# OpenNLPLab/ACR_WSSS

Hardware: AMD Instinct MI355X
Metric: img/s ACR-ViT-hybrid-base 448x448 train step (higher is better)
Workload: dtype f32_split; 1 GPU; BASELINE configs[1]: ViT-hybrid-base (DPT) 448x448, batch 16 per GPU, ACR train step (2 views, fwd+bwd+SGD); global_batch=16, classes=20, alpha=125, parallelism=dp1

## Files before the change

### acr_wsss_amd/csrc/attn_f32.h

```cpp
#pragma once
#include <hip/hip_runtime.h>
#include <stdint.h>

struct AttnGeom {
    int B, H, T;
    float scale;
    int64_t sb, st, sh;
    int64_t osb, ost, osh;
};

void acr_attn_fwd_f32_dma(const AttnGeom& g, const float* q, const float* k, const float* v, float* o, float* lse2, float* pmean,
                          int64_t pmean_sb, int64_t pmean_st, hipStream_t st);
void acr_attn_bwd_f32_dma(const AttnGeom& g, const float* q, const float* k, const float* v, const float* o, const float* d_o,
                          const float* lse2, const float* gm, int64_t gm_sb, int64_t gm_st, float* dq, float* dk, float* dv,
                          float* delta, hipStream_t st);

void acr_attn_fwd_f32_sres(const AttnGeom& g, const float* q, const float* k, const float* v, float* o, float* lse2, float* scores,
                           float* pmean, int64_t pmean_sb, int64_t pmean_st, hipStream_t st);
void acr_attn_bwd_f32_sres(const AttnGeom& g, const float* q, const float* k, const float* v, const float* o, const float* d_o,
                           const float* lse2, const float* scores, const float* gm, int64_t gm_sb, int64_t gm_st, float* dq,
                           float* dk, float* dv, float* delta, hipStream_t st);
void acr_attn_pmean_sres(const AttnGeom& g, const float* scores, const float* lse2, float* pmean, int64_t pmean_sb, int64_t pmean_st,
                         hipStream_t st);
void acr_attn_delta_sres(const AttnGeom& g, const float* scores, const float* o, const float* d_o, const float* lse2, const float* gm,
                         int64_t gm_sb, int64_t gm_st, float* delta, hipStream_t st);

int64_t acr_attn_x3_scores_floats(const AttnGeom& g);
int64_t acr_attn_x3_bwd_ws_floats(const AttnGeom& g);
bool acr_attn_x3_fwd_uses_split_tail(int T);
void acr_attn_fwd_f32_x3(const AttnGeom& g, const float* q, const float* k, const float* v, float* o, float* lse2, float* scores,
                         float* pmean, int64_t pmean_sb, int64_t pmean_st, hipStream_t st, char* oimg = nullptr);
void acr_attn_bwd_f32_x3(const AttnGeom& g, const float* q, const float* k, const float* v, const float* o, const float* d_o,
                         const float* lse2, const float* scores, const float* gm, int64_t gm_sb, int64_t gm_st, float* dq, float* dk,
                         float* dv, float* delta_ws, hipStream_t st);
```

### acr_wsss_amd/csrc/attn_f32.hip

```cpp
#include "acr_common.h"
#include "attn_f32.h"
#include "attn_f32_scores.h"

#define LDP 68
#define TILE_FLOATS (32 * LDP)

template <typename T, int NTHREADS>
__device__ __forceinline__ void stage_tile(float* lds, const T* g, int64_t st, int row0, int Tn, int tid, float mul) {
#pragma unroll
    for (int i = 0; i < 512 / NTHREADS; ++i) {
        const int slot = tid + i * NTHREADS;
        const int row = slot >> 4, c4 = slot & 15;
        f32x4 v = acr_load4<T>(g + (int64_t)min(row0 + row, Tn - 1) * st + c4 * 4) * mul;
        const f32x4 z = {0.f, 0.f, 0.f, 0.f};
        *reinterpret_cast<f32x4*>(lds + row * LDP + c4 * 4) = (row0 + row < Tn) ? v : z;
    }
}

template <typename T>
__device__ __forceinline__ void load_rows(float (&reg)[32], const T* g, int64_t st, int row0, int Tn, int lane, float mul) {
    const int r = lane & 31, h = lane >> 5;
    const float okm = (row0 + r < Tn) ? mul : 0.f;
    const T* p = g + (int64_t)min(row0 + r, Tn - 1) * st + 32 * h;
#pragma unroll
// ... 323 lines not shown
    const int r = lane & 31, hh = lane >> 5;
    const int key0 = ktile * 64 + wave * 32;
    const int64_t base = (int64_t)b * g.sb + (int64_t)h * g.sh;
    const int64_t obase = (int64_t)b * g.osb + (int64_t)h * g.osh;
    float kreg[32], vreg[32];
    load_rows<T>(kreg, k + base, g.st, key0, g.T, lane, g.scale * ACR_LOG2E);
    load_rows<T>(vreg, v + base, g.st, key0, g.T, lane, 1.f);
    const int key = key0 + r;
    const bool kok = key < g.T;
    const float invH = 1.f / (float)g.H;
    const float* lrow = lse2 + ((int64_t)b * g.H + h) * g.T;
    const float* drow = delta + ((int64_t)b * g.H + h) * g.T;
    const float* gbase = gm ? gm + (int64_t)b * gm_sb + min(key, g.T - 1) : nullptr;
    f32x16 dk0 = {0}, dk1 = {0}, dv0 = {0}, dv1 = {0};
    for (int q0 = 0; q0 < g.T; q0 += 32) {
        __syncthreads();
        stage_tile<T, 128>(qtile, q + base, g.st, q0, g.T, tid, 1.f);
        stage_tile<T, 128>(dotile, d_o + obase, g.ost, q0, g.T, tid, 1.f);
        if (tid < 32) {
            const bool ok = q0 + tid < g.T;
            const int qc = min(q0 + tid, g.T - 1);
            const float lv = lrow[qc], dvv = drow[qc];
            l2s[tid] = ok ? lv : INFINITY;
            dls[tid] = ok ? dvv : 0.f;
        }
        __syncthreads();
        f32x16 s = {0}, dp = {0};
        mma_rowop(s, qtile, kreg, lane);
        mma_rowop(dp, dotile, vreg, lane);
        float gv[16];
#pragma unroll
        for (int reg = 0; reg < 16; ++reg) gv[reg] = 0.f;
        if (gbase) {
#pragma unroll
            for (int reg = 0; reg < 16; ++reg) gv[reg] = gbase[min(q0 + acr_krow(reg, hh), g.T - 1) * (int)gm_st] * invH;
        }
        f32x16 p, ds;
        const float kmask = kok ? 1.f : 0.f;
#pragma unroll
        for (int reg = 0; reg < 16; ++reg) {
            const int kr = acr_krow(reg, hh);
            const float pv = exp2f(s[reg] - l2s[kr]) * kmask;
            p[reg] = pv;
            ds[reg] = pv * (dp[reg] + gv[reg] - dls[kr]);
        }
        mma_accop_a(dv0, p, dotile, 0, lane);
        mma_accop_a(dv1, p, dotile, 1, lane);
        mma_accop_a(dk0, ds, qtile, 0, lane);
        mma_accop_a(dk1, ds, qtile, 1, lane);
    }
#pragma unroll
    for (int reg = 0; reg < 16; ++reg) {
        const int kk = key0 + acr_krow(reg, hh);
        if (kk < g.T) {
            T* pk = dk + base + (int64_t)kk * g.st;
            T* pv = dv + base + (int64_t)kk * g.st;
            acr_store1<T>(pk + r, dk0[reg] * g.scale);
            acr_store1<T>(pk + 32 + r, dk1[reg] * g.scale);
            acr_store1<T>(pv + r, dv0[reg]);
            acr_store1<T>(pv + 32 + r, dv1[reg]);
        }
    }
}

template <typename T>
__global__ __launch_bounds__(64) void getam_row_kernel(AttnGeom g, const T* __restrict__ q, const T* __restrict__ k,
                                                       const T* __restrict__ v, const T* __restrict__ d_o,
                                                       const float* __restrict__ lse2, int batch, int func,
                                                       float* __restrict__ cam_row, int64_t row_stride) {
    __shared__ float q0s[64], do0s[64];
    const int j = blockIdx.x * 64 + threadIdx.x;
    batch += blockIdx.y;
    cam_row += (int64_t)blockIdx.y * row_stride;
    float sum_g = 0.f, sum_cg = 0.f;
    for (int h = 0; h < g.H; ++h) {
        const int64_t base = (int64_t)batch * g.sb + (int64_t)h * g.sh;
        __syncthreads();
        q0s[threadIdx.x] = acr_load1<T>(q + base + threadIdx.x) * (g.scale * ACR_LOG2E);
        do0s[threadIdx.x] = acr_load1<T>(d_o + (int64_t)batch * g.osb + (int64_t)h * g.osh + threadIdx.x);
        __syncthreads();
        if (j < g.T) {
            const T* kr = k + base + (int64_t)j * g.st;
            const T* vr = v + base + (int64_t)j * g.st;
            float s = 0.f, dp = 0.f;
#pragma unroll
            for (int d4 = 0; d4 < 16; ++d4) {
                f32x4 kv = acr_load4<T>(kr + 4 * d4), vv = acr_load4<T>(vr + 4 * d4);
#pragma unroll
                for (int e = 0; e < 4; ++e) {
                    s = fmaf(kv[e], q0s[4 * d4 + e], s);
                    dp = fmaf(vv[e], do0s[4 * d4 + e], dp);
                }
            }
            const float p = exp2f(s - lse2[((int64_t)batch * g.H + h) * g.T]);
            sum_g += fmaxf(dp, 0.f);
            sum_cg += fmaxf(dp * p, 0.f);
        }
    }
    if (j < g.T) {
        const float invH = 1.f / (float)g.H;
        const float mg = sum_g * invH, mcg = sum_cg * invH;
        float val;
        switch (func) {
            case ACR_GETAM_GRAD: val = mg; break;
            case ACR_GETAM_CAM_GRAD: val = mcg; break;
            case ACR_GETAM_GRAD_S: val = mg * mg; break;
            default: val = mcg * mg; break;
        }
        cam_row[j] += val;
    }
}

bool acr_bf16_mfma_ok(const acr_attn_desc* d, const void* const* ptrs, int n);
void acr_attn_fwd_bf16(const acr_attn_desc* d, const void* q, const void* k, const void* v, void* o, float* lse2,
                       float* pmean, int64_t pmean_sb, int64_t pmean_st, hipStream_t st);
void acr_attn_bwd_bf16(const acr_attn_desc* d, const void* q, const void* k, const void* v, const void* o,
                       const void* d_o, const float* lse2, const float* gm, int64_t gm_sb, int64_t gm_st, void* dq, void* dk,
                       void* dv, float* delta, hipStream_t st);
void acr_attn_probs_bf16(const acr_attn_desc* d, const void* q, const void* k, const float* lse2, float* probs,
                         hipStream_t st);
void acr_attn_dprobs_bf16(const acr_attn_desc* d, const void* d_o, const void* v, float* dprobs, hipStream_t st);

static int check_desc(const acr_attn_desc* d, const char* who) {
    ACR_CHECK_ARG(d != nullptr, "%s: null desc", who);
    ACR_CHECK_ARG(d->B > 0 && d->H > 0 && d->T > 0, "%s: bad geometry B=%d H=%d T=%d", who, d->B, d->H, d->T);
    ACR_CHECK_ARG(d->head_dim == 64, "%s: head_dim %d unsupported (library is built for 64)", who, d->head_dim);
    ACR_CHECK_ARG(d->dtype == ACR_F32 || d->dtype == ACR_BF16 || d->dtype == ACR_BF16_F32MATH || d->dtype == ACR_F32_BF16X3,
                  "%s: unknown dtype %d", who, d->dtype);
    ACR_CHECK_ARG((d->qkv_sb % 4) == 0 && (d->qkv_st % 4) == 0 && (d->qkv_sh % 4) == 0 && (d->o_sb % 4) == 0 &&
                      (d->o_st % 4) == 0 && (d->o_sh % 4) == 0,
                  "%s: strides must be multiples of 4 elements (vector loads)", who);
    ACR_CHECK_ARG((int64_t)d->B * d->H * ((d->T + 63) / 64) < (1ll << 31), "%s: grid too large", who);
    return ACR_OK;
}
static AttnGeom geom(const acr_attn_desc* d) {
    AttnGeom g;
    g.B = d->B; g.H = d->H; g.T = d->T; g.scale = d->scale;
    g.sb = d->qkv_sb; g.st = d->qkv_st; g.sh = d->qkv_sh;
    g.osb = d->o_sb; g.ost = d->o_st; g.osh = d->o_sh;
    return g;
}
static bool aligned16(const void* p) { return (reinterpret_cast<uintptr_t>(p) & 15) == 0; }
static bool aligned8(const void* p) { return (reinterpret_cast<uintptr_t>(p) & 7) == 0; }

template <typename T>
static int attn_fwd_t(const acr_attn_desc* d, const void* q, const void* k, const void* v, void* o, float* lse2,
                      float* pmean, int64_t pmean_sb, int64_t pmean_st, hipStream_t st) {
    AttnGeom g = geom(d);
    const int nqt = (d->T + 63) / 64;
    hipLaunchKernelGGL((attn_fwd_kernel<T>), dim3(d->B * d->H * nqt), dim3(128), 0, st, g, (const T*)q, (const T*)k,
                       (const T*)v, (T*)o, lse2);
    if (pmean)
        hipLaunchKernelGGL((attn_tile_qk_kernel<T, TQK_PMEAN>), dim3(d->B * nqt * nqt), dim3(256), 0, st, g,
                           (const T*)q, (const T*)k, (const float*)lse2, pmean, pmean_sb, pmean_st);
    return acr_check_launch("acr_attn_fwd");
}

extern "C" int acr_attn_fwd(const acr_attn_desc* d, const void* q, const void* k, const void* v, void* o,
                            float* lse2, float* pmean, int64_t pmean_sb, int64_t pmean_st, void* stream) {
    int rc = check_desc(d, "acr_attn_fwd");
    if (rc) return rc;
    ACR_CHECK_ARG(q && k && v && o && lse2, "acr_attn_fwd: null pointer");
    const bool f32 = d->dtype == ACR_F32;
    ACR_CHECK_ARG(f32 ? (aligned16(q) && aligned16(k) && aligned16(v) && aligned16(o))
                      : (aligned8(q) && aligned8(k) && aligned8(v) && aligned8(o)),
                  "acr_attn_fwd: q/k/v/o must be 16-byte (fp32) / 8-byte (bf16) aligned");
    ACR_CHECK_ARG(!pmean || (pmean_st >= d->T && pmean_sb >= (int64_t)d->T * pmean_st),
                  "acr_attn_fwd: pmean row pitch < T or batch stride < T*pitch");
    if (f32) {
        acr_attn_fwd_f32_dma(geom(d), (const float*)q, (const float*)k, (const float*)v, (float*)o, lse2, pmean, pmean_sb, pmean_st,
                             (hipStream_t)stream);
        return acr_check_launch("acr_attn_fwd");
    }
    const void* ptrs[4] = {q, k, v, o};
    if (d->dtype == ACR_BF16 && acr_bf16_mfma_ok(d, ptrs, 4)) {
        acr_attn_fwd_bf16(d, q, k, v, o, lse2, pmean, pmean_sb, pmean_st, (hipStream_t)stream);
        return acr_check_launch("acr_attn_fwd");
    }
    return attn_fwd_t<__bf16>(d, q, k, v, o, lse2, pmean, pmean_sb, pmean_st, (hipStream_t)stream);
}

static int check_gmean(const acr_attn_desc* d, const char* who, const float* gmean, int64_t gmean_sb, int64_t gmean_st) {
    ACR_CHECK_ARG(!gmean || (gmean_st >= d->T && gmean_sb >= (int64_t)d->T * gmean_st), "%s: gmean row pitch < T or batch stride < T*pitch", who);
    return ACR_OK;
}

template <typename T>
static int attn_bwd_t(const acr_attn_desc* d, const void* q, const void* k, const void* v, const void* o,
                      const void* d_o, const float* lse2, const float* gm, int64_t gm_sb, int64_t gm_st, void* dq,
                      void* dk, void* dv, float* delta, hipStream_t st) {
    AttnGeom g = geom(d);
    const int nqt = (d->T + 63) / 64;
    const dim3 grid(d->B * d->H * nqt);
    hipLaunchKernelGGL((attn_delta_kernel<T>), grid, dim3(128), 0, st, g, (const T*)q, (const T*)k, (const T*)o,
                       (const T*)d_o, lse2, gm, gm_sb, gm_st, delta);
    hipLaunchKernelGGL((attn_dkdv_kernel<T>), grid, dim3(128), 0, st, g, (const T*)q, (const T*)k, (const T*)v,
                       (const T*)d_o, lse2, (const float*)delta, gm, gm_sb, gm_st, (T*)dk, (T*)dv);
    hipLaunchKernelGGL((attn_dq_kernel<T>), grid, dim3(128), 0, st, g, (const T*)q, (const T*)k, (const T*)v,
                       (const T*)d_o, lse2, (const float*)delta, gm, gm_sb, gm_st, (T*)dq);
    return acr_check_launch("acr_attn_bwd");
}

extern "C" int acr_attn_bwd(const acr_attn_desc* d, const void* q, const void* k, const void* v, const void* o,
                            const void* d_o, const float* lse2, const float* gmean, int64_t gmean_sb, int64_t gmean_st,
                            void* dq, void* dk, void* dv, float* delta_ws, void* stream) {
    int rc = check_desc(d, "acr_attn_bwd");
    if (rc) return rc;
    ACR_CHECK_ARG(q && k && v && o && d_o && lse2 && dq && dk && dv && delta_ws, "acr_attn_bwd: null pointer");
    rc = check_gmean(d, "acr_attn_bwd", gmean, gmean_sb, gmean_st);
    if (rc) return rc;
    const bool f32 = d->dtype == ACR_F32;
    ACR_CHECK_ARG(f32 ? (aligned16(q) && aligned16(k) && aligned16(v) && aligned16(o) && aligned16(d_o))
                      : (aligned8(q) && aligned8(k) && aligned8(v) && aligned8(o) && aligned8(d_o)),
                  "acr_attn_bwd: inputs must be 16-byte (fp32) / 8-byte (bf16) aligned");
    if (f32) {
        acr_attn_bwd_f32_dma(geom(d), (const float*)q, (const float*)k, (const float*)v, (const float*)o, (const float*)d_o, lse2,
                             gmean, gmean_sb, gmean_st, (float*)dq, (float*)dk, (float*)dv, delta_ws, (hipStream_t)stream);
        return acr_check_launch("acr_attn_bwd");
    }
    const void* ptrs[8] = {q, k, v, o, d_o, dq, dk, dv};
    const bool g_ok = !gmean || ((gmean_st & 3) == 0 && gmean_st >= ((d->T + 3) & ~3) && (gmean_sb & 3) == 0 &&
                                 (reinterpret_cast<uintptr_t>(gmean) & 15) == 0);
    if (d->dtype == ACR_BF16 && g_ok && acr_bf16_mfma_ok(d, ptrs, 8)) {
        acr_attn_bwd_bf16(d, q, k, v, o, d_o, lse2, gmean, gmean_sb, gmean_st, dq, dk, dv, delta_ws, (hipStream_t)stream);
        return acr_check_launch("acr_attn_bwd");
    }
    return attn_bwd_t<__bf16>(d, q, k, v, o, d_o, lse2, gmean, gmean_sb, gmean_st, dq, dk, dv, delta_ws, (hipStream_t)stream);
}

extern "C" int64_t acr_attn_scores_floats(const acr_attn_desc* d) {
    if (d == nullptr || d->B <= 0 || d->H <= 0 || d->T <= 0) return 0;
    if (d->dtype == ACR_F32_BF16X3) return acr_attn_x3_scores_floats(geom(d));
    return attn_score_floats(d->B, d->H, d->T);
}

extern "C" int64_t acr_attn_bwd_ws_floats(const acr_attn_desc* d) {
    if (d == nullptr || d->B <= 0 || d->H <= 0 || d->T <= 0) return 0;
    if (d->dtype == ACR_F32_BF16X3) return acr_attn_x3_bwd_ws_floats(geom(d));
    return (int64_t)d->B * d->H * d->T;
}

static int check_x3(const acr_attn_desc* d, const char* who) {
    ACR_CHECK_ARG(d->qkv_sh >= 64 && d->o_sh >= 64, "%s: ACR_F32_BF16X3 needs head strides >= 64", who);
    ACR_CHECK_ARG((int64_t)32 * d->H * 64 < (1ll << 30), "%s: too many heads", who);
    return ACR_OK;
}

static int check_fwd_scores(const acr_attn_desc* d, const char* who, const void* q, const void* k, const void* v, const void* o,
                            const float* lse2, const float* scores, const float* pmean, int64_t pmean_sb, int64_t pmean_st,
                            bool has_image, const float* o_image) {
    ACR_CHECK_ARG(q && k && v && o && lse2 && scores && (!has_image || o_image), "%s: null pointer", who);
    ACR_CHECK_ARG(aligned16(q) && aligned16(k) && aligned16(v) && aligned16(o) && aligned16(scores) && aligned16(o_image),
                  "%s: q/k/v/o/scores%s must be 16-byte aligned", who, has_image ? "/o_image" : "");
    ACR_CHECK_ARG(!pmean || (pmean_st >= d->T && pmean_sb >= (int64_t)d->T * pmean_st), "%s: pmean row pitch < T or batch stride < T*pitch", who);
    return ACR_OK;
}

extern "C" int acr_attn_fwd_scores(const acr_attn_desc* d, const void* q, const void* k, const void* v, void* o, float* lse2,
                                   float* scores, float* pmean, int64_t pmean_sb, int64_t pmean_st, void* stream) {
    int rc = check_desc(d, "acr_attn_fwd_scores");
    if (rc) return rc;
    if (d->dtype != ACR_F32 && d->dtype != ACR_F32_BF16X3) {
        acr_set_error("acr_attn_fwd_scores: fp32 tensors only (the bf16 kernels recompute the logits)");
        return ACR_ERR_UNSUPPORTED;
    }
    rc = check_fwd_scores(d, "acr_attn_fwd_scores", q, k, v, o, lse2, scores, pmean, pmean_sb, pmean_st, false, nullptr);
    if (rc) return rc;
    if (d->dtype == ACR_F32_BF16X3) {
        rc = check_x3(d, "acr_attn_fwd_scores");
        if (rc) return rc;
        acr_attn_fwd_f32_x3(geom(d), (const float*)q, (const float*)k, (const float*)v, (float*)o, lse2, scores, pmean, pmean_sb, pmean_st,
                            (hipStream_t)stream);
        return acr_check_launch("acr_attn_fwd_scores");
    }
    acr_attn_fwd_f32_sres(geom(d), (const float*)q, (const float*)k, (const float*)v, (float*)o, lse2, scores, pmean, pmean_sb,
                          pmean_st, (hipStream_t)stream);
    return acr_check_launch("acr_attn_fwd_scores");
}

extern "C" int acr_attn_fwd_scores_oimg(const acr_attn_desc* d, const void* q, const void* k, const void* v, void* o, float* lse2,
                                        float* scores, float* pmean, int64_t pmean_sb, int64_t pmean_st, float* o_image, void* stream) {
    int rc = check_desc(d, "acr_attn_fwd_scores_oimg");
    if (rc) return rc;
    if (d->dtype != ACR_F32_BF16X3) {
        acr_set_error("acr_attn_fwd_scores_oimg: ACR_F32_BF16X3 only (the image is the split-product operand form)");
        return ACR_ERR_UNSUPPORTED;
    }
    rc = check_fwd_scores(d, "acr_attn_fwd_scores_oimg", q, k, v, o, lse2, scores, pmean, pmean_sb, pmean_st, true, o_image);
    if (rc) return rc;
    ACR_CHECK_ARG(d->o_sh == 64 && d->o_st == (int64_t)d->H * 64 && d->o_sb == (int64_t)d->T * d->o_st,
                  "acr_attn_fwd_scores_oimg: o must be the dense (B, T, H*64) activation (its image is that of the (B*T) x (H*64) matrix)");
    rc = check_x3(d, "acr_attn_fwd_scores_oimg");
    if (rc) return rc;
    acr_attn_fwd_f32_x3(geom(d), (const float*)q, (const float*)k, (const float*)v, (float*)o, lse2, scores, pmean, pmean_sb, pmean_st,
                        (hipStream_t)stream, reinterpret_cast<char*>(o_image));
    return acr_check_launch("acr_attn_fwd_scores_oimg");
}

extern "C" int acr_attn_fwd_oimg_offered(const acr_attn_desc* d) {
    if (!d || d->dtype != ACR_F32_BF16X3 || d->T <= 0) return 0;
    return acr_attn_x3_fwd_uses_split_tail(d->T) ? 0 : 1;
}

extern "C" int acr_attn_bwd_scores(const acr_attn_desc* d, const void* q, const void* k, const void* v, const void* o,
                                   const void* d_o, const float* lse2, const float* scores, const float* gmean, int64_t gmean_sb,
                                   int64_t gmean_st, void* dq, void* dk, void* dv, float* delta_ws, void* stream) {
    int rc = check_desc(d, "acr_attn_bwd_scores");
    if (rc) return rc;
    if (d->dtype != ACR_F32 && d->dtype != ACR_F32_BF16X3) {
        acr_set_error("acr_attn_bwd_scores: fp32 tensors only (the bf16 kernels recompute the logits)");
        return ACR_ERR_UNSUPPORTED;
    }
    ACR_CHECK_ARG(q && k && v && o && d_o && lse2 && scores && dq && dk && dv && delta_ws, "acr_attn_bwd_scores: null pointer");
    ACR_CHECK_ARG(aligned16(q) && aligned16(k) && aligned16(v) && aligned16(o) && aligned16(d_o) && aligned16(scores),
                  "acr_attn_bwd_scores: inputs must be 16-byte aligned");
    rc = check_gmean(d, "acr_attn_bwd_scores", gmean, gmean_sb, gmean_st);
    if (rc) return rc;
    ACR_CHECK_ARG(!gmean || ((gmean_st & 3) == 0 && (gmean_sb & 3) == 0 && aligned16(gmean)),
                  "acr_attn_bwd_scores: gmean must be 16-byte aligned with pitch and batch stride multiples of 4 floats");
    if (d->dtype == ACR_F32_BF16X3) {
        rc = check_x3(d, "acr_attn_bwd_scores");
        if (rc) return rc;
        ACR_CHECK_ARG(aligned16(delta_ws) && aligned16(dq) && aligned16(dk) && aligned16(dv), "acr_attn_bwd_scores: delta_ws / dq / dk / dv must be 16-byte aligned");
        acr_attn_bwd_f32_x3(geom(d), (const float*)q, (const float*)k, (const float*)v, (const float*)o, (const float*)d_o, lse2, scores,
                            gmean, gmean_sb, gmean_st, (float*)dq, (float*)dk, (float*)dv, delta_ws, (hipStream_t)stream);
        return acr_check_launch("acr_attn_bwd_scores");
    }
    acr_attn_bwd_f32_sres(geom(d), (const float*)q, (const float*)k, (const float*)v, (const float*)o, (const float*)d_o, lse2,
                          scores, gmean, gmean_sb, gmean_st, (float*)dq, (float*)dk, (float*)dv, delta_ws, (hipStream_t)stream);
    return acr_check_launch("acr_attn_bwd_scores");
}

extern "C" int acr_attn_probs(const acr_attn_desc* d, const void* q, const void* k, const float* lse2, float* probs,
                              void* stream) {
    int rc = check_desc(d, "acr_attn_probs");
    if (rc) return rc;
    ACR_CHECK_ARG(q && k && lse2 && probs, "acr_attn_probs: null pointer");
    AttnGeom g = geom(d);
    const int nt = (d->T + 63) / 64;
    ACR_CHECK_ARG((int64_t)d->B * d->H * nt * nt < (1ll << 31), "acr_attn_probs: grid too large");
    const dim3 grid(d->B * d->H * nt * nt);
    const void* pp[2] = {q, k};
    if (d->dtype == ACR_F32)
        hipLaunchKernelGGL((attn_tile_qk_kernel<float, TQK_PROBS>), grid, dim3(256), 0, (hipStream_t)stream, g,
                           (const float*)q, (const float*)k, lse2, probs, (int64_t)0, (int64_t)0);
    else if (d->dtype == ACR_BF16 && acr_bf16_mfma_ok(d, pp, 2))
        acr_attn_probs_bf16(d, q, k, lse2, probs, (hipStream_t)stream);
    else
        hipLaunchKernelGGL((attn_tile_qk_kernel<__bf16, TQK_PROBS>), grid, dim3(256), 0, (hipStream_t)stream, g,
                           (const __bf16*)q, (const __bf16*)k, lse2, probs, (int64_t)0, (int64_t)0);
    return acr_check_launch("acr_attn_probs");
}

extern "C" int acr_attn_dprobs(const acr_attn_desc* d, const void* d_o, const void* v, float* dprobs, void* stream) {
    int rc = check_desc(d, "acr_attn_dprobs");
    if (rc) return rc;
    ACR_CHECK_ARG(d_o && v && dprobs, "acr_attn_dprobs: null pointer");
    AttnGeom g = geom(d);
    const int nt = (d->T + 63) / 64;
    ACR_CHECK_ARG((int64_t)d->B * d->H * nt * nt < (1ll << 31), "acr_attn_dprobs: grid too large");
    const dim3 grid(d->B * d->H * nt * nt);
    const void* pp[2] = {d_o, v};
    if (d->dtype == ACR_F32)
        hipLaunchKernelGGL((attn_tile_qk_kernel<float, TQK_DPROBS>), grid, dim3(256), 0, (hipStream_t)stream, g,
                           (const float*)d_o, (const float*)v, (const float*)nullptr, dprobs, (int64_t)0, (int64_t)0);
    else if (d->dtype == ACR_BF16 && acr_bf16_mfma_ok(d, pp, 2))
        acr_attn_dprobs_bf16(d, d_o, v, dprobs, (hipStream_t)stream);
    else
        hipLaunchKernelGGL((attn_tile_qk_kernel<__bf16, TQK_DPROBS>), grid, dim3(256), 0, (hipStream_t)stream, g,
                           (const __bf16*)d_o, (const __bf16*)v, (const float*)nullptr, dprobs, (int64_t)0, (int64_t)0);
    return acr_check_launch("acr_attn_dprobs");
}

extern "C" int acr_getam_row_accum(const acr_attn_desc* d, const void* q, const void* k, const void* v,
                                   const void* d_o, const float* lse2, int32_t batch, int32_t func, float* cam_row,
                                   void* stream) {
    int rc = check_desc(d, "acr_getam_row_accum");
    if (rc) return rc;
    ACR_CHECK_ARG(q && k && v && d_o && lse2 && cam_row, "acr_getam_row_accum: null pointer");
    ACR_CHECK_ARG(batch >= 0 && batch < d->B, "acr_getam_row_accum: batch %d out of range", batch);
    ACR_CHECK_ARG(func >= 0 && func <= 3, "acr_getam_row_accum: unknown func %d", func);
    AttnGeom g = geom(d);
    const dim3 grid((d->T + 63) / 64);
    if (d->dtype == ACR_F32)
        hipLaunchKernelGGL((getam_row_kernel<float>), grid, dim3(64), 0, (hipStream_t)stream, g, (const float*)q,
                           (const float*)k, (const float*)v, (const float*)d_o, lse2, batch, func, cam_row, (int64_t)0);
    else
        hipLaunchKernelGGL((getam_row_kernel<__bf16>), grid, dim3(64), 0, (hipStream_t)stream, g, (const __bf16*)q,
                           (const __bf16*)k, (const __bf16*)v, (const __bf16*)d_o, lse2, batch, func, cam_row, (int64_t)0);
    return acr_check_launch("acr_getam_row_accum");
}

extern "C" int acr_getam_rows_accum(const acr_attn_desc* d, const void* q, const void* k, const void* v, const void* d_o,
                                    const float* lse2, int32_t func, float* cam_rows, int64_t row_stride, void* stream) {
    int rc = check_desc(d, "acr_getam_rows_accum");
    if (rc) return rc;
    ACR_CHECK_ARG(q && k && v && d_o && lse2 && cam_rows, "acr_getam_rows_accum: null pointer");
    ACR_CHECK_ARG(func >= 0 && func <= 3, "acr_getam_rows_accum: unknown func %d", func);
    ACR_CHECK_ARG(row_stride >= d->T && d->B < 65536, "acr_getam_rows_accum: row pitch < T or batch too large");
    ACR_CHECK_ARG(d->dtype != ACR_F32_BF16X3, "acr_getam_rows_accum: exact kernels only (pass ACR_F32)");
    AttnGeom g = geom(d);
    const dim3 grid((d->T + 63) / 64, d->B);
    if (d->dtype == ACR_F32)
        hipLaunchKernelGGL((getam_row_kernel<float>), grid, dim3(64), 0, (hipStream_t)stream, g, (const float*)q,
                           (const float*)k, (const float*)v, (const float*)d_o, lse2, 0, func, cam_rows, row_stride);
    else
        hipLaunchKernelGGL((getam_row_kernel<__bf16>), grid, dim3(64), 0, (hipStream_t)stream, g, (const __bf16*)q,
                           (const __bf16*)k, (const __bf16*)v, (const __bf16*)d_o, lse2, 0, func, cam_rows, row_stride);
    return acr_check_launch("acr_getam_rows_accum");
}
```

### acr_wsss_amd/csrc/attn_f32_scores.h

```cpp
#pragma once
#include "acr_common.h"
#include "attn_f32.h"
#include "attn_f32_tiles.h"

#define SB_FLOATS 1024
__device__ __forceinline__ int64_t attn_score_block(int H, int NB, int b, int hd, int qb, int kb) {
    return ((((int64_t)b * H + hd) * NB + qb) * NB + kb) * SB_FLOATS;
}
static inline int64_t attn_score_floats(int B, int H, int T) {
    const int64_t nb = (T + 31) / 32;
    return (int64_t)B * H * nb * nb * SB_FLOATS;
}
static inline bool attn_split_tail(int NB, int nw) { return (NB % nw) == 1 && NB > nw; }

#define SRES_LOAD_NT(p) __builtin_nontemporal_load(reinterpret_cast<const f32x4*>(p))
#define SRES_LOAD(p) (*reinterpret_cast<const f32x4*>(p))
#define SRES_STORE(p, v) __builtin_nontemporal_store(v, reinterpret_cast<f32x4*>(p))
#define SRES_LOAD_DQ(p) SRES_LOAD_NT(p)
#define SRES_DMA_AUX 0

template <bool TEXT, int N>
__device__ __forceinline__ void attn_vmcnt() {
    if constexpr (!TEXT) asm volatile("s_waitcnt vmcnt(%0)" ::"n"(N) : "memory");
    else if constexpr (N == 8) asm volatile("s_waitcnt vmcnt(8)" ::: "memory");
    else if constexpr (N == 4) asm volatile("s_waitcnt vmcnt(4)" ::: "memory");
    else { static_assert(N == 0, "add the count's text"); asm volatile("s_waitcnt vmcnt(0)" ::: "memory"); }
}
template <bool TEXT, int... Ns>
__device__ __forceinline__ void attn_wait_vm(int n) {
    if (!((n >= Ns ? (attn_vmcnt<TEXT, Ns>(), true) : false) || ...)) attn_vmcnt<TEXT, 0>();
}
#define ATTN_FENCE() asm volatile("" ::: "memory")

#define ATTN_MASK_ROWS(s, row0, T, h)                                   \
    if ((row0) + 32 > (T)) {  \
        _Pragma("unroll") for (int reg = 0; reg < 16; ++reg)            \
            if ((row0) + acr_krow(reg, h) >= (T)) s[reg] = -INFINITY;   \
    }

#define ATTN_QLANE_STREAMS(sres, H, NB, T, b, hd, q0, wave, lane, ssm, gsm, gm, gm_sb, gm_st)                                       \
    const float* srow = sres + attn_score_block(H, NB, b, hd, min(q0 >> 5, NB - 1), 0) + lane * 4;                                  \
    float* sw = ssm + wave * 2 * SB_FLOATS;                                                                                         \
    auto dma_scores = [&](int kblk, int slot) {                                                                                     \
        const float* src = srow + (int64_t)kblk * SB_FLOATS;                                                                        \
        _Pragma("unroll") for (int gq = 0; gq < 4; ++gq)                                                                            \
            __builtin_amdgcn_global_load_lds((glb_vp)(src + gq * 256), (lds_vp)(sw + slot * SB_FLOATS + gq * 256), 16, 0, SRES_DMA_AUX); \
    };                                                                                                                              \
    const float* gb0 = gm ? gm + (int64_t)b * gm_sb : nullptr;                                                                      \
    float* gw = gsm + wave * SB_FLOATS;                                                                                             \
    const float* grow[4];                                                                                                           \
    int gchunk[4];                                                                                                                  \
    _Pragma("unroll") for (int p = 0; p < 4; ++p) {                                                                                 \
        const int row = 8 * p + (lane >> 3);                                                                                        \
        grow[p] = gb0 ? gb0 + (int64_t)min(q0 + row, T - 1) * gm_st : nullptr;                                                      \
        gchunk[p] = 4 * ((lane & 7) ^ ((row >> 1) & 7));                                                                            \
    }                                                                                                                               \
    auto dma_g = [&](int k0) {                                                                                                      \
        if (gb0 == nullptr) return;                                                                                                 \
        _Pragma("unroll") for (int p = 0; p < 4; ++p)                                                                               \
            __builtin_amdgcn_global_load_lds((glb_vp)(grow[p] + min(k0 + gchunk[p], (int)gm_st - 4)), (lds_vp)(gw + p * 256), 16, 0, 0); \
    }
#define ATTN_QLANE_ADDRS(lane, r, h)                                                                                                \
    const uint32_t saddr = lds_addr_of(sw) + lane * 16;                                                                             \
    uint32_t gaddr[4];                                                                                                              \
    _Pragma("unroll") for (int gq = 0; gq < 4; ++gq) gaddr[gq] = lds_addr_of(gw) + r * 128 + (((2 * gq + h) ^ ((r >> 1) & 7)) << 4)
#define ATTN_QLANE_READ(SLOT, s4, g4, k0, T, h)                                                                                     \
    ACR_LDS_RD128(s4[0], saddr, SLOT * 4096); ACR_LDS_RD128(s4[1], saddr, SLOT * 4096 + 1024);                                      \
    ACR_LDS_RD128(s4[2], saddr, SLOT * 4096 + 2048); ACR_LDS_RD128(s4[3], saddr, SLOT * 4096 + 3072);                               \
    if (gb0 != nullptr) {                                                                                                           \
        ACR_LDS_RD128(g4[0], gaddr[0], 0); ACR_LDS_RD128(g4[1], gaddr[1], 0);                                                       \
        ACR_LDS_RD128(g4[2], gaddr[2], 0); ACR_LDS_RD128(g4[3], gaddr[3], 0);                                                       \
        ACR_LDS_WAIT4(0, g4[0], g4[1], g4[2], g4[3]);                                                                               \
        if (k0 + 32 > T) {                                                                                                          \
            _Pragma("unroll") for (int gq = 0; gq < 4; ++gq)                                                                        \
                _Pragma("unroll") for (int e = 0; e < 4; ++e)                                                                       \
                    if (k0 + 8 * gq + 4 * h + e >= T) g4[gq][e] = 0.f;                                                              \
        }                                                                                                                           \
    } else {                                                                                                                        \
        _Pragma("unroll") for (int gq = 0; gq < 4; ++gq) g4[gq] = f32x4{0.f, 0.f, 0.f, 0.f};                                        \
    }                                                                                                                               \
    ACR_LDS_WAIT4(0, s4[0], s4[1], s4[2], s4[3])
__device__ __forceinline__ void attn_ds_qlane(f32x16& ds, const f32x4 (&s4)[4], const f32x4 (&g4)[4], const f32x16& dp, float l2q, float dl,
                                              float invH) {
#pragma unroll
    for (int reg = 0; reg < 16; ++reg)
        ds[reg] = __builtin_amdgcn_exp2f(s4[reg >> 2][reg & 3] - l2q) * (dp[reg] + g4[reg >> 2][reg & 3] * invH - dl);
}

#define ATTN_KLANE_STREAMS(sres, H, NB, T, b, hd, key0, wave, lane, ssm, gsm, gm, gm_sb, gm_st)                                     \
    const float* scol = sres + attn_score_block(H, NB, b, hd, 0, min(key0 >> 5, NB - 1));                                           \
    const int64_t sstep = (int64_t)NB * SB_FLOATS;                                                                                  \
    int soff[4];                                                                                                                    \
    _Pragma("unroll") for (int gq = 0; gq < 4; ++gq) soff[gq] = gq * 256 + 4 * (lane ^ (2 * gq + (lane >> 5)));                     \
    float* sw = ssm + wave * 2 * SB_FLOATS;                                                                                         \
    auto dma_scores = [&](int qblk, int slot) {                                                                                     \
        const float* src = scol + (int64_t)qblk * sstep;                                                                            \
        _Pragma("unroll") for (int gq = 0; gq < 4; ++gq)                                                                            \
            __builtin_amdgcn_global_load_lds((glb_vp)(src + soff[gq]), (lds_vp)(sw + slot * SB_FLOATS + gq * 256), 16, 0, SRES_DMA_AUX); \
    };                                                                                                                              \
    const float* gb0 = gm ? gm + (int64_t)b * gm_sb : nullptr;                                                                      \
    float* gw = gsm + wave * SB_FLOATS;                                                                                             \
    const int gcol = min(key0 + 4 * (lane & 7), (int)gm_st - 4);                                                                    \
    auto dma_g = [&](int qrow0) {                                                                                                   \
        if (gb0 == nullptr) return;                                                                                                 \
        _Pragma("unroll") for (int p = 0; p < 4; ++p) {                                                                             \
            const float* src = gb0 + (int64_t)min(qrow0 + 8 * p + (lane >> 3), T - 1) * gm_st + gcol;                               \
            __builtin_amdgcn_global_load_lds((glb_vp)src, (lds_vp)(gw + p * 256), 16, 0, 0);                                        \
        }                                                                                                                           \
    }
#define ATTN_KLANE_ADDRS(ssm, gsm, wave, r, h)                                                                                      \
    uint32_t stb[4];                                                                                                                \
    {                                                                                                                               \
        const int gk = r >> 3, hk = (r >> 2) & 1, ek = r & 3, mm = 2 * gk + hk;                                                     \
        _Pragma("unroll") for (int j = 0; j < 4; ++j)                                                                               \
            stb[j] = lds_addr_of(ssm) + ((wave * 2 * SB_FLOATS) + gk * 256 + 128 * hk + ek + 4 * ((j + 4 * h) ^ mm)) * 4;           \
    }                                                                                                                               \
    const uint32_t gaddr = lds_addr_of(gsm) + (wave * SB_FLOATS + 4 * h * 32 + r) * 4
#define ATTN_16(M, ...) \
    M(0, __VA_ARGS__); M(1, __VA_ARGS__); M(2, __VA_ARGS__); M(3, __VA_ARGS__); M(4, __VA_ARGS__); M(5, __VA_ARGS__); M(6, __VA_ARGS__); M(7, __VA_ARGS__); \
    M(8, __VA_ARGS__); M(9, __VA_ARGS__); M(10, __VA_ARGS__); M(11, __VA_ARGS__); M(12, __VA_ARGS__); M(13, __VA_ARGS__); M(14, __VA_ARGS__); M(15, __VA_ARGS__)
#define ATTN_RDS(REG, s, SLOT) ACR_LDS_RD32(s[REG], stb[(REG) & 3], SLOT * SB_FLOATS * 4 + 128 * ((REG) >> 2))
#define ATTN_RDG(REG, gv) ACR_LDS_RD32(gv[REG], gaddr, 128 * (((REG) & 3) + 8 * ((REG) >> 2)))
#define ATTN_V16(x) \
    "+v"(x[0]), "+v"(x[1]), "+v"(x[2]), "+v"(x[3]), "+v"(x[4]), "+v"(x[5]), "+v"(x[6]), "+v"(x[7]), "+v"(x[8]), "+v"(x[9]), "+v"(x[10]), \
        "+v"(x[11]), "+v"(x[12]), "+v"(x[13]), "+v"(x[14]), "+v"(x[15])
#define ATTN_READ_G(gv)                                                     \
    if (gb0 != nullptr) {                                                   \
        ATTN_16(ATTN_RDG, gv);                                              \
        asm volatile("s_waitcnt lgkmcnt(0)" : ATTN_V16(gv));                \
    } else {                                                                \
        _Pragma("unroll") for (int reg = 0; reg < 16; ++reg) gv[reg] = 0.f; \
    }

__device__ __forceinline__ void attn_store_scores(float* sp, const f32x16& s) {
#pragma unroll
    for (int gq = 0; gq < 4; ++gq) {
        const f32x4 t = {s[4 * gq], s[4 * gq + 1], s[4 * gq + 2], s[4 * gq + 3]};
        SRES_STORE(sp + gq * 256, t);
    }
}
#define ATTN_SOFTMAX_STEP(s, m, l, o0, o1, p)                                                             \
    {                                                                                                     \
        float mx_ = s[0];                                                                                 \
        _Pragma("unroll") for (int reg = 1; reg < 16; ++reg) mx_ = fmaxf(mx_, s[reg]);                    \
        mx_ = fmaxf(mx_, __shfl_xor(mx_, 32));                                                            \
        if (__any(mx_ > m + 8.f)) {                                                                       \
            const float mn_ = fmaxf(m, mx_);                                                              \
            const float alpha_ = __builtin_amdgcn_exp2f(m - mn_);                                         \
            l *= alpha_;                                                                                  \
            o0 *= alpha_; o1 *= alpha_;                                                                   \
            m = mn_;                                                                                      \
        }                                                                                                 \
        float rs_ = 0.f;                                                                                  \
        _Pragma("unroll") for (int reg = 0; reg < 16; ++reg) { p[reg] = __builtin_amdgcn_exp2f(s[reg] - m); rs_ += p[reg]; } \
        rs_ += __shfl_xor(rs_, 32);                                                                       \
        l += rs_;                                                                                         \
    }
#define ATTN_FWD_FINISH(g, o, lse2, b, hd, q0, r, h, o0, o1, m, l, inv)                                                   \
    {                                                                                                                     \
        float* ob_ = o + (int64_t)b * g.osb + (int64_t)(q0 + r) * g.ost + (int64_t)hd * g.osh;                            \
        _Pragma("unroll") for (int grp = 0; grp < 4; ++grp) {                                                             \
            f32x4 a_ = {o0[4 * grp] * inv, o0[4 * grp + 1] * inv, o0[4 * grp + 2] * inv, o0[4 * grp + 3] * inv};          \
            f32x4 c_ = {o1[4 * grp] * inv, o1[4 * grp + 1] * inv, o1[4 * grp + 2] * inv, o1[4 * grp + 3] * inv};          \
            *reinterpret_cast<f32x4*>(ob_ + 8 * grp + 4 * h) = a_;                                                        \
            *reinterpret_cast<f32x4*>(ob_ + 32 + 8 * grp + 4 * h) = c_;                                                   \
        }                                                                                                                 \
        if (h == 0) lse2[((int64_t)b * g.H + hd) * g.T + q0 + r] = m + log2f(l);                                          \
    }
```

### acr_wsss_amd/csrc/attn_f32_sres.hip

```cpp
#include <type_traits>

#include "acr_common.h"
#include "attn_f32.h"
#include "attn_f32_tiles.h"
#include "attn_f32_scores.h"
#include "attn_f32_sres_tails.h"


template <int NW>
__global__ __launch_bounds__(64 * NW, NW == 4 ? 2 : 1) void attn_fwd_sres_kernel(AttnGeom g, const float* __restrict__ q, const float* __restrict__ k,
                                                               const float* __restrict__ v, float* __restrict__ o,
                                                               float* __restrict__ lse2, float* __restrict__ sres, int ntail) {
    __shared__ __attribute__((aligned(1024))) float smem[4 * DT_FLOATS];
    __shared__ float mlsh[4 * 64];
    const int nmain = (int)gridDim.x - ntail;
    if (NW == 4 && (int)blockIdx.x >= nmain) {
        attn_fwd_tail_body<4>(smem, mlsh, g, q, k, v, o, lse2, sres, acr_xcd_remap((int)blockIdx.x - nmain, ntail));
        return;
    }
    const int NB = (g.T + 31) >> 5, nqt = ntail ? NB / NW : (NB + NW - 1) / NW;
    int id = acr_xcd_remap(blockIdx.x, nmain);
    const int qt = id % nqt; id /= nqt;
    const int hd = id % g.H;
    const int b = id / g.H;
// ... 156 lines not shown
    f32x16 pm = {0};
    for (int h0 = 0; h0 < g.H; h0 += 4) {
        f32x4 sv[4][4];
        float lv[4];
#pragma unroll
        for (int hi = 0; hi < 4; ++hi) {
            const int hd = min(h0 + hi, g.H - 1);
#pragma unroll
            for (int gq = 0; gq < 4; ++gq) sv[hi][gq] = SRES_LOAD_NT(sp + hd * hstride + gq * 256);
            lv[hi] = lp[(int64_t)hd * g.T];
        }
#pragma unroll
        for (int hi = 0; hi < 4; ++hi) {
            if (h0 + hi < g.H) {
                const float l2 = qrow < g.T ? lv[hi] : INFINITY;
#pragma unroll
                for (int reg = 0; reg < 16; ++reg) pm[reg] += __builtin_amdgcn_exp2f(sv[hi][reg >> 2][reg & 3] - l2);
            }
        }
    }
    const float mul = 1.f / (float)g.H;
    float* tl = tile[wave];
#pragma unroll
    for (int reg = 0; reg < 16; ++reg) tl[theta * 33 + acr_krow(reg, hh)] = pm[reg] * mul;
    __syncthreads();
    if (act) {
        const int key = kb * 32 + theta;
        float* ob = out + (int64_t)b * out_sb;
        if (key < g.T) {
#pragma unroll
            for (int i = 0; i < 16; ++i) {
                const int row = 2 * i + hh;
                const int qq = qb * 32 + row;
                if (qq < g.T) ob[(int64_t)qq * out_st + key] = tl[row * 33 + theta];
            }
        }
    }
}

__global__ __launch_bounds__(256) void attn_delta_sres_kernel(AttnGeom g, int NB, const float* __restrict__ sres,
                                                              const float* __restrict__ o, const float* __restrict__ d_o,
                                                              const float* __restrict__ lse2, const float* __restrict__ gm,
                                                              int64_t gm_sb, int64_t gm_st, float* __restrict__ delta) {
    const int tid = threadIdx.x, lane = tid & 63, wave = tid >> 6;
    const int theta = lane & 31, hh = lane >> 5;
    int id = blockIdx.x * 4 + wave;
    if (id >= g.B * NB * g.H) return;
    const int hd = id % g.H;
    const int t = id / g.H;
    const int qb = t % NB, b = t / NB;
    const int qrow = qb * 32 + theta;
    const bool qok = qrow < g.T;
    const int qc = min(qrow, g.T - 1);
    float part = 0.f;
    {
        const int64_t off = (int64_t)b * g.osb + (int64_t)hd * g.osh + (int64_t)qc * g.ost + 32 * hh;
        const float* op = o + off;
        const float* dp = d_o + off;
#pragma unroll
        for (int i = 0; i < 8; ++i) {
            const f32x4 a = *reinterpret_cast<const f32x4*>(op + 4 * i), c = *reinterpret_cast<const f32x4*>(dp + 4 * i);
            part += a[0] * c[0] + a[1] * c[1] + a[2] * c[2] + a[3] * c[3];
        }
    }
    part += __shfl_xor(part, 32);
    float rho = 0.f;
    if (gm != nullptr) {
        const float l2q = qok ? lse2[((int64_t)b * g.H + hd) * g.T + qrow] : INFINITY;
        const float* sp = sres + attn_score_block(g.H, NB, b, hd, qb, 0) + lane * 4;
        const float* gr = gm + (int64_t)b * gm_sb + (int64_t)qc * gm_st;
        const int nfull = g.T >> 5;
#pragma unroll 4
        for (int kb = 0; kb < nfull; ++kb) {
            f32x4 sv[4], gv[4];
#pragma unroll
            for (int gq = 0; gq < 4; ++gq) {
                sv[gq] = SRES_LOAD(sp + (int64_t)kb * SB_FLOATS + gq * 256);
                gv[gq] = *reinterpret_cast<const f32x4*>(gr + kb * 32 + 8 * gq + 4 * hh);
            }
#pragma unroll
            for (int reg = 0; reg < 16; ++reg)
                rho = fmaf(__builtin_amdgcn_exp2f(sv[reg >> 2][reg & 3] - l2q), gv[reg >> 2][reg & 3], rho);
        }
        if (nfull < NB) {
            const int k0 = nfull * 32;
#pragma unroll
            for (int gq = 0; gq < 4; ++gq) {
                const f32x4 sv = *reinterpret_cast<const f32x4*>(sp + (int64_t)nfull * SB_FLOATS + gq * 256);
#pragma unroll
                for (int e = 0; e < 4; ++e) {
                    const float gv = gr[min(k0 + 8 * gq + 4 * hh + e, g.T - 1)];
                    rho = fmaf(__builtin_amdgcn_exp2f(sv[e] - l2q), gv, rho);
                }
            }
        }
        rho += __shfl_xor(rho, 32);
    }
    if (hh == 0 && qok) delta[((int64_t)b * g.H + hd) * g.T + qrow] = part + rho * (1.f / (float)g.H);
}

__device__ __forceinline__ void sres_wait_vm(int n) { attn_wait_vm<true, 8, 4>(n); }

__device__ __forceinline__ void attn_dq_sres_body(float* smem, float* ssm, float* gsm, int bid, int nblk, bool tails, const AttnGeom& g,
                                                  const float* __restrict__ k, const float* __restrict__ v,
                                                  const float* __restrict__ d_o, const float* __restrict__ lse2,
                                                  const float* __restrict__ delta, const float* __restrict__ sres,
                                                  const float* __restrict__ gm, int64_t gm_sb, int64_t gm_st, float* __restrict__ dq) {
    const int NB = (g.T + 31) >> 5, nqt = tails ? NB >> 2 : (NB + 3) >> 2;
    int id = acr_xcd_remap(bid, nblk);
    const int qt = id % nqt; id /= nqt;
    const int hd = id % g.H;
    const int b = id / g.H;
    const int tid = threadIdx.x, lane = tid & 63;
    const int wave = __builtin_amdgcn_readfirstlane(tid >> 6);
    const int r = lane & 31, h = lane >> 5;
    const int q0 = qt * 128 + wave * 32;
    const bool live = q0 < g.T;
    const int64_t base = (int64_t)b * g.sb + (int64_t)hd * g.sh;
    const int64_t obase = (int64_t)b * g.osb + (int64_t)hd * g.osh;
    const float* kb = k + base;
    const float* vb = v + base;
    ATTN_QLANE_STREAMS(sres, g.H, NB, g.T, b, hd, q0, wave, lane, ssm, gsm, gm, gm_sb, gm_st);
    dma_tile32(smem, kb, g.st, 0, g.T, wave, lane);
    dma_tile32(smem + DT_FLOATS, vb, g.st, 0, g.T, wave, lane);
    if (live) {
        dma_g(0);
        dma_scores(0, 0);
        if (32 < g.T) dma_scores(1, 1);
    }
    float doreg[32];
    rows_from_global(doreg, d_o + obase, g.ost, q0, g.T, r, h, 1.f);
    const bool qok = q0 + r < g.T;
    const float l2q = qok ? lse2[((int64_t)b * g.H + hd) * g.T + q0 + r] : INFINITY;
    const float dl = qok ? delta[((int64_t)b * g.H + hd) * g.T + q0 + r] : 0.f;
    const float invH = gb0 ? 1.f / (float)g.H : 0.f;
    f32x16 dq0 = {0}, dq1 = {0};
    const LaneBasesA lb = lane_bases_a(r, h, smem);
    int doff[2];
    dma_offsets32(doff, g.st, wave, lane);
    ATTN_QLANE_ADDRS(lane, r, h);
    auto step = [&](int k0, auto slot_tag) {
        constexpr int SLOT = decltype(slot_tag)::value;
        constexpr int KOFF = SLOT * 2 * DT_FLOATS * 4, VOFF = KOFF + DT_FLOATS * 4;
        sres_wait_vm((k0 > 0 && live) ? (gb0 ? 4 : 0) + (k0 + 32 < g.T ? 4 : 0) : 0);
        acr_barrier_nofence();
        if (k0 + 64 <= g.T) {
            dma_tile32_i(smem + (SLOT ^ 1) * 2 * DT_FLOATS, kb + (int64_t)(k0 + 32) * g.st, doff, wave);
            dma_tile32_i(smem + (SLOT ^ 1) * 2 * DT_FLOATS + DT_FLOATS, vb + (int64_t)(k0 + 32) * g.st, doff, wave);
        } else if (k0 + 32 < g.T) {
            dma_tile32(smem + (SLOT ^ 1) * 2 * DT_FLOATS, kb, g.st, k0 + 32, g.T, wave, lane);
            dma_tile32(smem + (SLOT ^ 1) * 2 * DT_FLOATS + DT_FLOATS, vb, g.st, k0 + 32, g.T, wave, lane);
        }
        ATTN_FENCE();
        if (!live) return;
        f32x16 dp = {0};
        rowop_x<VOFF>(dp, lb, doreg);
        if (k0 > 0) sres_wait_vm(k0 + 32 < g.T ? 8 : 0);
        f32x4 s4[4], g4[4];
        ATTN_QLANE_READ(SLOT, s4, g4, k0, g.T, h);
        f32x16 ds;
        __builtin_amdgcn_s_setprio(2);
        attn_ds_qlane(ds, s4, g4, dp, l2q, dl, invH);
        __builtin_amdgcn_s_setprio(0);
        if (k0 + 32 < g.T) dma_g(k0 + 32);
        if (k0 + 64 < g.T) dma_scores((k0 >> 5) + 2, SLOT);
        ATTN_FENCE();
        accop_x<KOFF, 0, true>(dq0, ds, lb);
        accop_x<KOFF, 1, true>(dq1, ds, lb);
    };
    for (int k0 = 0; k0 < g.T; k0 += 64) {
        step(k0, std::integral_constant<int, 0>{});
        if (k0 + 32 < g.T) step(k0 + 32, std::integral_constant<int, 1>{});
    }
    if (!live) return;
#pragma unroll
    for (int reg = 0; reg < 16; ++reg) {
        const int qq = q0 + acr_krow(reg, h);
        if (qq < g.T) {
            float* p = dq + base + (int64_t)qq * g.st;
            p[r] = dq0[reg] * g.scale;
            p[32 + r] = dq1[reg] * g.scale;
        }
    }
}

__device__ __forceinline__ void attn_dkdv_sres_body(float* smem, float* ssm, float* gsm, int bid, int nblk, bool tails, const AttnGeom& g,
                                                    const float* __restrict__ q, const float* __restrict__ v,
                                                    const float* __restrict__ d_o, const float* __restrict__ lse2,
                                                    const float* __restrict__ delta, const float* __restrict__ sres,
                                                    const float* __restrict__ gm, int64_t gm_sb, int64_t gm_st,
                                                    float* __restrict__ dk, float* __restrict__ dv) {
    const int NB = (g.T + 31) >> 5, nkt = tails ? NB >> 2 : (NB + 3) >> 2;
    int id = acr_xcd_remap(bid, nblk);
    const int ktile = id % nkt; id /= nkt;
    const int hd = id % g.H;
    const int b = id / g.H;
    const int tid = threadIdx.x, lane = tid & 63;
    const int wave = __builtin_amdgcn_readfirstlane(tid >> 6);
    const int r = lane & 31, h = lane >> 5;
    const int key0 = ktile * 128 + wave * 32;
    const bool live = key0 < g.T;
    const int64_t base = (int64_t)b * g.sb + (int64_t)hd * g.sh;
    const int64_t obase = (int64_t)b * g.osb + (int64_t)hd * g.osh;
    const float* qb = q + base;
    const float* dob = d_o + obase;
    const float* lrow = lse2 + ((int64_t)b * g.H + hd) * g.T;
    const float* drow = delta + ((int64_t)b * g.H + hd) * g.T;
    ATTN_KLANE_STREAMS(sres, g.H, NB, g.T, b, hd, key0, wave, lane, ssm, gsm, gm, gm_sb, gm_st);
    dma_tile32(smem, qb, g.st, 0, g.T, wave, lane);
    dma_tile32(smem + DT_FLOATS, dob, g.ost, 0, g.T, wave, lane);
    if (live) {
        dma_g(0);
        dma_scores(0, 0);
        if (32 < g.T) dma_scores(1, 1);
    }
    float vreg[32];
    rows_from_global(vreg, v + base, g.st, key0, g.T, r, h, 1.f);
    const float invH = gb0 ? 1.f / (float)g.H : 0.f;
    f32x16 dk0 = {0}, dk1 = {0}, dv0 = {0}, dv1 = {0};
    const LaneBasesA lb = lane_bases_a(r, h, smem);
    int qoff[2], dooff[2];
    dma_offsets32(qoff, g.st, wave, lane);
    dma_offsets32(dooff, g.ost, wave, lane);
    ATTN_KLANE_ADDRS(ssm, gsm, wave, r, h);
    auto step = [&](int q0, auto slot_tag) {
        constexpr int SLOT = decltype(slot_tag)::value;
        constexpr int QOFF = SLOT * 2 * DT_FLOATS * 4, DOOFF = QOFF + DT_FLOATS * 4;
        sres_wait_vm((q0 > 0 && live) ? (gb0 ? 4 : 0) + (q0 + 32 < g.T ? 4 : 0) : 0);
        acr_barrier_nofence();
        if (q0 + 64 <= g.T) {
            dma_tile32_i(smem + (SLOT ^ 1) * 2 * DT_FLOATS, qb + (int64_t)(q0 + 32) * g.st, qoff, wave);
            dma_tile32_i(smem + (SLOT ^ 1) * 2 * DT_FLOATS + DT_FLOATS, dob + (int64_t)(q0 + 32) * g.ost, dooff, wave);
        } else if (q0 + 32 < g.T) {
            dma_tile32(smem + (SLOT ^ 1) * 2 * DT_FLOATS, qb, g.st, q0 + 32, g.T, wave, lane);
            dma_tile32(smem + (SLOT ^ 1) * 2 * DT_FLOATS + DT_FLOATS, dob, g.ost, q0 + 32, g.T, wave, lane);
        }
        ATTN_FENCE();
        if (!live) return;
        const int qi = min(q0 + r, g.T - 1);
        const float lq_lane = lrow[qi], dq_lane = drow[qi];
        f32x16 dp = {0};
        rowop_x<DOOFF>(dp, lb, vreg);
        if (q0 > 0) sres_wait_vm(q0 + 32 < g.T ? 8 : 0);
        float s[16], gv[16];
        ATTN_16(ATTN_RDS, s, SLOT);
        ATTN_READ_G(gv)
        asm volatile("s_waitcnt lgkmcnt(0)" : ATTN_V16(s));
        ATTN_MASK_ROWS(s, q0, g.T, h);
        f32x16 p, ds;
        __builtin_amdgcn_s_setprio(2);
#pragma unroll
        for (int reg = 0; reg < 16; ++reg) {
            const int src = acr_krow(reg, h);
            const float lq = __shfl(lq_lane, src), dq_ = __shfl(dq_lane, src);
            const float pv = __builtin_amdgcn_exp2f(s[reg] - lq);
            p[reg] = pv;
            ds[reg] = pv * (dp[reg] + gv[reg] * invH - dq_);
        }
        __builtin_amdgcn_s_setprio(0);
        asm volatile("s_waitcnt lgkmcnt(0)" ::: "memory");
        if (q0 + 32 < g.T) dma_g(q0 + 32);
        if (q0 + 64 < g.T) dma_scores((q0 >> 5) + 2, SLOT);
        ATTN_FENCE();
        accop_x<DOOFF, 0, true>(dv0, p, lb);
        accop_x<DOOFF, 1, true>(dv1, p, lb);
        accop_x<QOFF, 0, true>(dk0, ds, lb);
        accop_x<QOFF, 1, true>(dk1, ds, lb);
    };
    for (int q0 = 0; q0 < g.T; q0 += 64) {
        step(q0, std::integral_constant<int, 0>{});
        if (q0 + 32 < g.T) step(q0 + 32, std::integral_constant<int, 1>{});
    }
    if (!live) return;
#pragma unroll
    for (int reg = 0; reg < 16; ++reg) {
        const int kk = key0 + acr_krow(reg, h);
        if (kk < g.T) {
            float* pk = dk + base + (int64_t)kk * g.st;
            float* pv = dv + base + (int64_t)kk * g.st;
            pk[r] = dk0[reg] * g.scale;
            pk[32 + r] = dk1[reg] * g.scale;
            pv[r] = dv0[reg];
            pv[32 + r] = dv1[reg];
        }
    }
}

__global__ __launch_bounds__(256, 2) void attn_bwd_sres_kernel(AttnGeom g, const float* __restrict__ q, const float* __restrict__ k,
                                                               const float* __restrict__ v, const float* __restrict__ d_o,
                                                               const float* __restrict__ lse2, const float* __restrict__ delta,
                                                               const float* __restrict__ sres, const float* __restrict__ gm,
                                                               int64_t gm_sb, int64_t gm_st, float* __restrict__ dq,
                                                               float* __restrict__ dk, float* __restrict__ dv, int ntail) {
    __shared__ __attribute__((aligned(1024))) float smem[4 * DT_FLOATS];
    __shared__ __attribute__((aligned(1024))) float ssm[4 * 2 * SB_FLOATS];
    __shared__ __attribute__((aligned(1024))) float gsm[4 * SB_FLOATS];
    const int half = ((int)gridDim.x - 2 * ntail) >> 1;
    const int bid = (int)blockIdx.x;
    if (bid < half)
        attn_dkdv_sres_body(smem, ssm, gsm, bid, half, ntail != 0, g, q, v, d_o, lse2, delta, sres, gm, gm_sb, gm_st, dk, dv);
    else if (bid < 2 * half)
        attn_dq_sres_body(smem, ssm, gsm, bid - half, half, ntail != 0, g, k, v, d_o, lse2, delta, sres, gm, gm_sb, gm_st, dq);
    else if (bid < 2 * half + ntail)
        attn_dkdv_tail_body<4>(smem, ssm, g, q, v, d_o, lse2, delta, sres, gm, gm_sb, gm_st, dk, dv, acr_xcd_remap(bid - 2 * half, ntail));
    else
        attn_dq_tail_body<4>(smem, g, k, v, d_o, lse2, delta, sres, gm, gm_sb, gm_st, dq, acr_xcd_remap(bid - 2 * half - ntail, ntail));
}

void acr_attn_fwd_f32_sres(const AttnGeom& g, const float* q, const float* k, const float* v, float* o, float* lse2, float* scores,
                           float* pmean, int64_t pmean_sb, int64_t pmean_st, hipStream_t st) {
    const int NB = (g.T + 31) / 32;
    const int ntail = attn_split_tail(NB, 4) ? g.B * g.H : 0;
    const int nmain = g.B * g.H * (ntail ? NB / 4 : (NB + 3) / 4);
    hipLaunchKernelGGL(attn_fwd_sres_kernel<4>, dim3(nmain + ntail), dim3(256), 0, st, g, q, k, v, o, lse2, scores, ntail);
    if (pmean) acr_attn_pmean_sres(g, scores, lse2, pmean, pmean_sb, pmean_st, st);
}

void acr_attn_pmean_sres(const AttnGeom& g, const float* scores, const float* lse2, float* pmean, int64_t pmean_sb, int64_t pmean_st,
                         hipStream_t st) {
    const int NB = (g.T + 31) / 32;
    hipLaunchKernelGGL(attn_pmean_sres_kernel, dim3((g.B * NB * NB + 3) / 4), dim3(256), 0, st, g, NB, scores, lse2, pmean, pmean_sb,
                       pmean_st);
}

void acr_attn_delta_sres(const AttnGeom& g, const float* scores, const float* o, const float* d_o, const float* lse2, const float* gm,
                         int64_t gm_sb, int64_t gm_st, float* delta, hipStream_t st) {
    const int NB = (g.T + 31) / 32;
#ifndef DELTA4_NW
#define DELTA4_NW 4
#endif
    if (gm != nullptr && (g.H % DELTA4_NW) == 0 && acr_opt(ACR_OPT_ATTN_DELTA_1HEAD) == 0)
        hipLaunchKernelGGL(attn_delta_sres4_kernel<DELTA4_NW>, dim3(g.B * NB * (g.H / DELTA4_NW)), dim3(64 * DELTA4_NW), 0, st, g, NB, scores, o, d_o,
                           lse2, gm, gm_sb, gm_st, delta);
    else
        hipLaunchKernelGGL(attn_delta_sres_kernel, dim3((g.B * NB * g.H + 3) / 4), dim3(256), 0, st, g, NB, scores, o, d_o, lse2, gm, gm_sb,
                           gm_st, delta);
}

void acr_attn_bwd_f32_sres(const AttnGeom& g, const float* q, const float* k, const float* v, const float* o, const float* d_o,
                           const float* lse2, const float* scores, const float* gm, int64_t gm_sb, int64_t gm_st, float* dq,
                           float* dk, float* dv, float* delta, hipStream_t st) {
    const int nt = (g.T + 127) / 128, NB = (g.T + 31) / 32;
    acr_attn_delta_sres(g, scores, o, d_o, lse2, gm, gm_sb, gm_st, delta, st);
    const int ntail = attn_split_tail(NB, 4) ? g.B * g.H : 0;
    const int nmain = g.B * g.H * (ntail ? NB / 4 : nt);
    hipLaunchKernelGGL(attn_bwd_sres_kernel, dim3(2 * nmain + 2 * ntail), dim3(256), 0, st, g, q, k, v, d_o, lse2, (const float*)delta,
                       scores, gm, gm_sb, gm_st, dq, dk, dv, ntail);
}
```

### acr_wsss_amd/csrc/attn_f32_sres_tails.h

```cpp
#pragma once
#include "acr_common.h"
#include "attn_f32.h"
#include "attn_f32_tiles.h"
#include "attn_f32_scores.h"


__device__ __forceinline__ void wave_wait_dma() { asm volatile("s_waitcnt vmcnt(0)" ::: "memory"); }
__device__ __forceinline__ void wave_wait_lds() { asm volatile("s_waitcnt lgkmcnt(0)" ::: "memory"); }

template <int NW>
__device__ __forceinline__ void attn_fwd_tail_body(float* smem, float* mlsh, const AttnGeom& g, const float* __restrict__ q,
                                                   const float* __restrict__ k, const float* __restrict__ v, float* __restrict__ o,
                                                   float* __restrict__ lse2, float* __restrict__ sres, int id) {
    const int NB = (g.T + 31) >> 5;
    const int hd = id % g.H, b = id / g.H;
    const int tid = threadIdx.x, lane = tid & 63;
    const int wave = __builtin_amdgcn_readfirstlane(tid >> 6);
    const int r = lane & 31, h = lane >> 5;
    const int q0 = (NB - 1) * 32;
    const int64_t base = (int64_t)b * g.sb + (int64_t)hd * g.sh;
    const float* kb = k + base;
    const float* vb = v + base;
    float* tl = smem + wave * DT_FLOATS;
    float qreg[32];
    rows_from_global(qreg, q + base, g.st, q0, g.T, r, h, g.scale * ACR_LOG2E);
    float m = -INFINITY, l = 0.f;
    f32x16 o0 = {0}, o1 = {0};
    const LaneBases lb = lane_bases_at(r, h, wave * DT_FLOATS * 4);
    const char* sm = reinterpret_cast<const char*>(smem);
    float* sblk = sres + attn_score_block(g.H, NB, b, hd, NB - 1, 0) + lane * 4;
    for (int kt = wave; kt < NB; kt += NW) {
        const int k0 = kt * 32;
        dma_tile32_one(tl, kb, g.st, k0, g.T, lane);
        wave_wait_dma();
        f32x16 s = {0};
        rowop_i<0>(s, sm, lb, qreg);
        ATTN_MASK_ROWS(s, k0, g.T, h);
        wave_wait_lds();
        dma_tile32_one(tl, vb, g.st, k0, g.T, lane);
        attn_store_scores(sblk + (int64_t)kt * SB_FLOATS, s);
        f32x16 p;
        ATTN_SOFTMAX_STEP(s, m, l, o0, o1, p);
        wave_wait_dma();
        accop_b_i<0, 0>(o0, p, sm, lb);
        accop_b_i<0, 1>(o1, p, sm, lb);
        wave_wait_lds();
    }
    __syncthreads();
#pragma unroll
    for (int e = 0; e < 16; ++e) { tl[e * 64 + lane] = o0[e]; tl[(16 + e) * 64 + lane] = o1[e]; }
    if (h == 0) { mlsh[wave * 64 + r] = m; mlsh[wave * 64 + 32 + r] = l; }
    __syncthreads();
    if (wave != 0) return;
    float M = m;
#pragma unroll
    for (int w = 1; w < NW; ++w) M = fmaxf(M, mlsh[w * 64 + r]);
    float L = 0.f;
    f32x16 a0 = {0}, a1 = {0};
#pragma unroll
    for (int w = 0; w < NW; ++w) {
        const float f = __builtin_amdgcn_exp2f(mlsh[w * 64 + r] - M);
        L += mlsh[w * 64 + 32 + r] * f;
        const float* pw = smem + w * DT_FLOATS;
#pragma unroll
        for (int e = 0; e < 16; ++e) { a0[e] += pw[e * 64 + lane] * f; a1[e] += pw[(16 + e) * 64 + lane] * f; }
    }
    if (q0 + r < g.T) {
        const float inv = 1.f / L;
        ATTN_FWD_FINISH(g, o, lse2, b, hd, q0, r, h, a0, a1, M, L, inv);
    }
}

template <int NW>
__device__ __forceinline__ void attn_dq_tail_body(float* smem, const AttnGeom& g, const float* __restrict__ k,
                                                  const float* __restrict__ v, const float* __restrict__ d_o,
                                                  const float* __restrict__ lse2, const float* __restrict__ delta,
                                                  const float* __restrict__ sres, const float* __restrict__ gm, int64_t gm_sb,
                                                  int64_t gm_st, float* __restrict__ dq, int id) {
    const int NB = (g.T + 31) >> 5;
    const int hd = id % g.H, b = id / g.H;
    const int tid = threadIdx.x, lane = tid & 63;
    const int wave = __builtin_amdgcn_readfirstlane(tid >> 6);
    const int r = lane & 31, h = lane >> 5;
    const int q0 = (NB - 1) * 32;
    const int64_t base = (int64_t)b * g.sb + (int64_t)hd * g.sh;
    const int64_t obase = (int64_t)b * g.osb + (int64_t)hd * g.osh;
    const float* kb = k + base;
    const float* vb = v + base;
    float* tl = smem + wave * DT_FLOATS;
    float doreg[32];
    rows_from_global(doreg, d_o + obase, g.ost, q0, g.T, r, h, 1.f);
    const bool qok = q0 + r < g.T;
    const float l2q = qok ? lse2[((int64_t)b * g.H + hd) * g.T + q0 + r] : INFINITY;
    const float dl = qok ? delta[((int64_t)b * g.H + hd) * g.T + q0 + r] : 0.f;
    const float invH = 1.f / (float)g.H;
    const float* grow = gm ? gm + (int64_t)b * gm_sb + (int64_t)min(q0 + r, g.T - 1) * gm_st : nullptr;
    const float* sblk = sres + attn_score_block(g.H, NB, b, hd, NB - 1, 0) + lane * 4;
    f32x16 dq0 = {0}, dq1 = {0};
    const LaneBases lb = lane_bases_at(r, h, wave * DT_FLOATS * 4);
    const char* sm = reinterpret_cast<const char*>(smem);
    for (int kt = wave; kt < NB; kt += NW) {
        const int k0 = kt * 32;
        dma_tile32_one(tl, vb, g.st, k0, g.T, lane);
        f32x4 s4[4], g4[4];
        const float* sp = sblk + (int64_t)kt * SB_FLOATS;
#pragma unroll
        for (int gq = 0; gq < 4; ++gq) s4[gq] = SRES_LOAD_DQ(sp + gq * 256);
        if (grow == nullptr) {
#pragma unroll
            for (int gq = 0; gq < 4; ++gq) g4[gq] = f32x4{0.f, 0.f, 0.f, 0.f};
        } else if (k0 + 32 <= g.T) {
#pragma unroll
            for (int gq = 0; gq < 4; ++gq) g4[gq] = *reinterpret_cast<const f32x4*>(grow + k0 + 8 * gq + 4 * h);
        } else {
#pragma unroll
            for (int gq = 0; gq < 4; ++gq)
#pragma unroll
                for (int e = 0; e < 4; ++e) g4[gq][e] = grow[min(k0 + 8 * gq + 4 * h + e, g.T - 1)];
        }
        wave_wait_dma();
        f32x16 dp = {0};
        rowop_i<0>(dp, sm, lb, doreg);
        wave_wait_lds();
        dma_tile32_one(tl, kb, g.st, k0, g.T, lane);
        f32x16 ds;
#pragma unroll
        for (int reg = 0; reg < 16; ++reg) {
            const float gv = g4[reg >> 2][reg & 3] * invH;
            ds[reg] = __builtin_amdgcn_exp2f(s4[reg >> 2][reg & 3] - l2q) * (dp[reg] + gv - dl);
        }
        wave_wait_dma();
        accop_a_i<0, 0>(dq0, ds, sm, lb);
        accop_a_i<0, 1>(dq1, ds, sm, lb);
        wave_wait_lds();
    }
    __syncthreads();
#pragma unroll
    for (int e = 0; e < 16; ++e) { tl[e * 64 + lane] = dq0[e]; tl[(16 + e) * 64 + lane] = dq1[e]; }
    __syncthreads();
    if (wave != 0) return;
#pragma unroll 1
    for (int w = 1; w < NW; ++w) {
        const float* pw = smem + w * DT_FLOATS;
#pragma unroll
        for (int e = 0; e < 16; ++e) { dq0[e] += pw[e * 64 + lane]; dq1[e] += pw[(16 + e) * 64 + lane]; }
    }
#pragma unroll
    for (int reg = 0; reg < 16; ++reg) {
        const int qq = q0 + acr_krow(reg, h);
        if (qq < g.T) {
            float* p = dq + base + (int64_t)qq * g.st;
            p[r] = dq0[reg] * g.scale;
            p[32 + r] = dq1[reg] * g.scale;
        }
    }
}

template <int NW>
__device__ __forceinline__ void attn_dkdv_tail_body(float* smem, float* ssm, const AttnGeom& g, const float* __restrict__ q,
                                                    const float* __restrict__ v, const float* __restrict__ d_o,
                                                    const float* __restrict__ lse2, const float* __restrict__ delta,
                                                    const float* __restrict__ sres, const float* __restrict__ gm, int64_t gm_sb,
                                                    int64_t gm_st, float* __restrict__ dk, float* __restrict__ dv, int id) {
    const int NB = (g.T + 31) >> 5;
    const int hd = id % g.H, b = id / g.H;
    const int tid = threadIdx.x, lane = tid & 63;
    const int wave = __builtin_amdgcn_readfirstlane(tid >> 6);
    const int r = lane & 31, h = lane >> 5;
    const int key0 = (NB - 1) * 32;
    const int64_t base = (int64_t)b * g.sb + (int64_t)hd * g.sh;
    const int64_t obase = (int64_t)b * g.osb + (int64_t)hd * g.osh;
    const float* qb = q + base;
    const float* dob = d_o + obase;
    const float* lrow = lse2 + ((int64_t)b * g.H + hd) * g.T;
    const float* drow = delta + ((int64_t)b * g.H + hd) * g.T;
    const float* scol = sres + attn_score_block(g.H, NB, b, hd, 0, NB - 1);
    const int64_t sstep = (int64_t)NB * SB_FLOATS;
    float* tl = smem + wave * DT_FLOATS;
    float* sw = ssm + wave * 2 * SB_FLOATS;
    float* rcw = sw + SB_FLOATS;
    float vreg[32];
    rows_from_global(vreg, v + base, g.st, key0, g.T, r, h, 1.f);
    const int key = key0 + r;
    const int gcl = min(key, g.T - 1);
    const float invH = 1.f / (float)g.H;
    const float* gb0 = gm ? gm + (int64_t)b * gm_sb : nullptr;
    f32x16 dk0 = {0}, dk1 = {0}, dv0 = {0}, dv1 = {0};
    const LaneBases lb = lane_bases_at(r, h, wave * DT_FLOATS * 4);
    const char* sm = reinterpret_cast<const char*>(smem);
    const char* ssb = reinterpret_cast<const char*>(ssm);
    int tb[4];
    {
        const int gk = r >> 3, hk = (r >> 2) & 1, ek = r & 3, mm = 2 * gk + hk;
#pragma unroll
        for (int j = 0; j < 4; ++j) tb[j] = ((wave * 2 * SB_FLOATS) + gk * 256 + 128 * hk + ek + 4 * ((j + 4 * h) ^ mm)) * 4;
    }
    for (int qt = wave; qt < NB; qt += NW) {
        const int q0 = qt * 32;
        dma_tile32_one(tl, dob, g.ost, q0, g.T, lane);
        {
            const float* src = scol + (int64_t)qt * sstep;
#pragma unroll
            for (int gq = 0; gq < 4; ++gq)
                __builtin_amdgcn_global_load_lds((glb_vp)(src + gq * 256 + 4 * (lane ^ (2 * gq + (lane >> 5)))),
                                                 (lds_vp)(sw + gq * 256), 16, 0, 0);
        }
        dma_rowconst(rcw, lrow, drow, q0, g.T, lane);
        float gv[16];
#pragma unroll
        for (int reg = 0; reg < 16; ++reg)
            gv[reg] = gb0 ? gb0[(int64_t)min(q0 + acr_krow(reg, h), g.T - 1) * gm_st + gcl] * invH : 0.f;
        wave_wait_dma();
        f32x16 dp = {0};
        rowop_i<0>(dp, sm, lb, vreg);
        f32x16 s;
#pragma unroll
        for (int reg = 0; reg < 16; ++reg) s[reg] = *reinterpret_cast<const float*>(ssb + tb[reg & 3] + 128 * (reg >> 2));
        ATTN_MASK_ROWS(s, q0, g.T, h);
        f32x16 p, ds;
#pragma unroll
        for (int gq = 0; gq < 4; ++gq) {
            const f32x4 l4 = *reinterpret_cast<const f32x4*>(rcw + 8 * gq + 4 * h);
            const f32x4 d4 = *reinterpret_cast<const f32x4*>(rcw + 32 + 8 * gq + 4 * h);
#pragma unroll
            for (int e = 0; e < 4; ++e) {
                const int reg = 4 * gq + e;
                const float pv = __builtin_amdgcn_exp2f(s[reg] - l4[e]);
                p[reg] = pv;
                ds[reg] = pv * (dp[reg] + gv[reg] - d4[e]);
            }
        }
        accop_a_i<0, 0>(dv0, p, sm, lb);
        accop_a_i<0, 1>(dv1, p, sm, lb);
        wave_wait_lds();
        dma_tile32_one(tl, qb, g.st, q0, g.T, lane);
        wave_wait_dma();
        accop_a_i<0, 0>(dk0, ds, sm, lb);
        accop_a_i<0, 1>(dk1, ds, sm, lb);
        wave_wait_lds();
    }
    __syncthreads();
#pragma unroll
    for (int e = 0; e < 16; ++e) {
        tl[e * 64 + lane] = dk0[e]; tl[(16 + e) * 64 + lane] = dk1[e];
        sw[e * 64 + lane] = dv0[e]; sw[(16 + e) * 64 + lane] = dv1[e];
    }
    __syncthreads();
    if (wave != 0) return;
#pragma unroll 1
    for (int w = 1; w < NW; ++w) {
        const float* pk = smem + w * DT_FLOATS;
        const float* pv = ssm + w * 2 * SB_FLOATS;
#pragma unroll
        for (int e = 0; e < 16; ++e) {
            dk0[e] += pk[e * 64 + lane]; dk1[e] += pk[(16 + e) * 64 + lane];
            dv0[e] += pv[e * 64 + lane]; dv1[e] += pv[(16 + e) * 64 + lane];
        }
    }
#pragma unroll
    for (int reg = 0; reg < 16; ++reg) {
        const int kk = key0 + acr_krow(reg, h);
        if (kk < g.T) {
            float* pk = dk + base + (int64_t)kk * g.st;
            float* pv = dv + base + (int64_t)kk * g.st;
            pk[r] = dk0[reg] * g.scale;
            pk[32 + r] = dk1[reg] * g.scale;
            pv[r] = dv0[reg];
            pv[32 + r] = dv1[reg];
        }
    }
}
```

### acr_wsss_amd/csrc/attn_f32_x3.hip

```cpp
#include <type_traits>

#include "acr_split.h"
#include "attn_f32.h"
#include "attn_f32_scores.h"
#include "attn_f32_sres_tails.h"

typedef __bf16 bf16_t;

#define X3_PLANE_B (32 * 64 * 2)
#define X3_TILE_B (3 * X3_PLANE_B)
#define X3_SLOT_B (2 * X3_TILE_B)


__device__ __forceinline__ void x3_wait_vm(int n) { attn_wait_vm<false, 9, 8, 7, 5, 4, 1>(n); }
__device__ __forceinline__ void x3_barrier(int n_younger) {
    x3_wait_vm(n_younger);
    acr_barrier_nofence();
}

struct X3Geom {
    int B, H, T, D;
    float scale;
    int64_t plane;
    int64_t osb, ost, osh;
    int64_t sb, st, sh;
};

__device__ __forceinline__ int x3_swz(int row) {
    const int x = (row >> 1) & 7;
    return x ^ ((x & 1) << 2);
}

struct X3SplitArgs {
    const float* src[3];
    int64_t sb, st, sh;
    bf16_t* dst;
    int64_t plane;
    int B, T, H;
};
__global__ __launch_bounds__(256) void x3_split_kernel(const X3SplitArgs a) {
    const int64_t n8 = (int64_t)a.B * a.T * a.H * 8;
    const int64_t i = (int64_t)blockIdx.x * 256 + threadIdx.x;
    if (i >= n8) return;
    const int w = blockIdx.y;
    const int c8 = (int)(i & 7);
    int64_t t = i >> 3;
    const int h = (int)(t % a.H); t /= a.H;
    const int tok = (int)(t % a.T);
    const int b = (int)(t / a.T);
    const float* s = a.src[w] + (int64_t)b * a.sb + (int64_t)tok * a.st + (int64_t)h * a.sh + c8 * 8;
    const f32x4 lo = *reinterpret_cast<const f32x4*>(s), hi = *reinterpret_cast<const f32x4*>(s + 4);
    bf16x8 p0, p1, p2;
    split3_bf16(lo, hi, p0, p1, p2);
    bf16_t* d = a.dst + (int64_t)(3 * w) * a.plane + i * 8;
    *reinterpret_cast<bf16x8*>(d) = p0;
    *reinterpret_cast<bf16x8*>(d + a.plane) = p1;
    *reinterpret_cast<bf16x8*>(d + 2 * a.plane) = p2;
}

__global__ __launch_bounds__(256) void x3_split2d_kernel(const float* __restrict__ x, int64_t rows, int64_t cols, int64_t ld,
                                                        bf16_t* __restrict__ dst, int64_t plane) {
    const int64_t c8n = cols >> 3;
    const int64_t i = (int64_t)blockIdx.x * 256 + threadIdx.x;
    if (i >= rows * c8n) return;
    const int64_t row = i / c8n, c8 = i - row * c8n;
    const float* s = x + row * ld + c8 * 8;
    const f32x4 lo = *reinterpret_cast<const f32x4*>(s), hi = *reinterpret_cast<const f32x4*>(s + 4);
    bf16x8 p0, p1, p2;
    split3_bf16(lo, hi, p0, p1, p2);
    bf16_t* d = dst + row * cols + c8 * 8;
    *reinterpret_cast<bf16x8*>(d) = p0;
    *reinterpret_cast<bf16x8*>(d + plane) = p1;
    *reinterpret_cast<bf16x8*>(d + 2 * plane) = p2;
}

__device__ __forceinline__ int x3_dma_off(int D, int wave, int lane) {
    const int row = 8 * wave + (lane >> 3);
    return row * D + (((lane & 7) ^ x3_swz(row)) << 3);
}
__device__ __forceinline__ void x3_dma_tile_i(char* lds, const bf16_t* __restrict__ row0ptr, int64_t plane, int off, int wave) {
#pragma unroll
    for (int p = 0; p < 3; ++p)
        __builtin_amdgcn_global_load_lds((glb_vp)(row0ptr + p * plane + off), (lds_vp)(lds + p * X3_PLANE_B + wave * 1024), 16, 0, 0);
}
__device__ __forceinline__ void x3_dma_tile(char* lds, const bf16_t* __restrict__ base, int64_t plane, int D, int row0, int Tn, int wave,
                                            int lane) {
    const int row = 8 * wave + (lane >> 3);
    const bf16_t* src = base + (int64_t)min(row0 + row, Tn - 1) * D + (((lane & 7) ^ x3_swz(row)) << 3);
#pragma unroll
    for (int p = 0; p < 3; ++p)
        __builtin_amdgcn_global_load_lds((glb_vp)(src + p * plane), (lds_vp)(lds + p * X3_PLANE_B + wave * 1024), 16, 0, 0);
}

struct X3Lane { uint32_t rowb[4]; uint32_t trb[2][2]; };
__device__ __forceinline__ X3Lane x3_lane(int lane, const char* smem) {
    X3Lane lb;
    const uint32_t lds0 = lds_addr_of(smem);
    const int r = lane & 31, h = lane >> 5;
    const int fr = x3_swz(r);
#pragma unroll
    for (int s = 0; s < 4; ++s) lb.rowb[s] = lds0 + r * 128 + (((2 * s + h) ^ fr) << 4);
    const int i = lane & 15, g1 = (lane >> 4) & 1, q = i >> 2, p = i & 3;
#pragma unroll
    for (int hi = 0; hi < 2; ++hi) {
        const int row = 8 * hi + 4 * h + q;
        const int f = x3_swz(row);
#pragma unroll
        for (int blk = 0; blk < 2; ++blk) lb.trb[hi][blk] = lds0 + row * 128 + (((4 * blk + 2 * g1 + (p >> 1)) ^ f) << 4) + 8 * (p & 1);
    }
    return lb;
}
#define X3_RDTR(lo, hi, alo, ahi, OFF)                                                                  \
    asm volatile("ds_read_b64_tr_b16 %0, %2 offset:%4\n\tds_read_b64_tr_b16 %1, %3 offset:%4"          \
                 : "=&v"(lo), "=&v"(hi) : "v"(alo), "v"(ahi), "i"(OFF))
#define X3_WAIT3(cnt, x) asm volatile("s_waitcnt lgkmcnt(" #cnt ")" : "+v"(x[0]), "+v"(x[1]), "+v"(x[2]))
#define X3_WAIT6(cnt, l, h_) \
    asm volatile("s_waitcnt lgkmcnt(" #cnt ")" : "+v"(l[0]), "+v"(l[1]), "+v"(l[2]), "+v"(h_[0]), "+v"(h_[1]), "+v"(h_[2]))
#define X3_ROWFRAG(a, lb, TOFF, S) \
    { ACR_LDS_RD128(a[0], lb.rowb[S], TOFF); ACR_LDS_RD128(a[1], lb.rowb[S], (TOFF) + X3_PLANE_B); ACR_LDS_RD128(a[2], lb.rowb[S], (TOFF) + 2 * X3_PLANE_B); }
#define X3_TRFRAG(l, h_, lb, TOFF, S, BLK)                                                      \
    { X3_RDTR(l[0], h_[0], lb.trb[0][BLK], lb.trb[1][BLK], (TOFF) + (S) * 2048);                 \
      X3_RDTR(l[1], h_[1], lb.trb[0][BLK], lb.trb[1][BLK], (TOFF) + X3_PLANE_B + (S) * 2048);    \
      X3_RDTR(l[2], h_[2], lb.trb[0][BLK], lb.trb[1][BLK], (TOFF) + 2 * X3_PLANE_B + (S) * 2048); }
#define X3_JOIN(a, l, h_)                                                                       \
    const bf16x8 a[3] = {__builtin_shufflevector(l[0], h_[0], 0, 1, 2, 3, 4, 5, 6, 7),           \
                         __builtin_shufflevector(l[1], h_[1], 0, 1, 2, 3, 4, 5, 6, 7),           \
                         __builtin_shufflevector(l[2], h_[2], 0, 1, 2, 3, 4, 5, 6, 7)}

struct X3Nop { __device__ __forceinline__ void operator()() const {} };

template <int TILE_OFF, class F0 = X3Nop, class F1 = X3Nop, class F2 = X3Nop>
__device__ __forceinline__ void x3_rowop(f32x16& acc, const X3Lane& lb, const bf16x8 (&y)[3][4], F0&& f0 = F0(), F1&& f1 = F1(),
                                         F2&& f2 = F2()) {
    bf16x8 a0[3], a1[3];
    X3_ROWFRAG(a0, lb, TILE_OFF, 0);
    X3_ROWFRAG(a1, lb, TILE_OFF, 1);
    X3_WAIT3(3, a0);
    { const bf16x8 b_[3] = {y[0][0], y[1][0], y[2][0]}; ACR_MFMA6(acc, a0, b_); }
    f0();
    X3_ROWFRAG(a0, lb, TILE_OFF, 2);
    X3_WAIT3(3, a1);
    { const bf16x8 b_[3] = {y[0][1], y[1][1], y[2][1]}; ACR_MFMA6(acc, a1, b_); }
    f1();
    X3_ROWFRAG(a1, lb, TILE_OFF, 3);
    X3_WAIT3(3, a0);
    { const bf16x8 b_[3] = {y[0][2], y[1][2], y[2][2]}; ACR_MFMA6(acc, a0, b_); }
    f2();
    X3_WAIT3(0, a1);
    { const bf16x8 b_[3] = {y[0][3], y[1][3], y[2][3]}; ACR_MFMA6(acc, a1, b_); }
}
template <int TILE_OFF, bool ZA, class F0 = X3Nop, class F1 = X3Nop, class F2 = X3Nop>
__device__ __forceinline__ void x3_accop(f32x16& acc0, f32x16& acc1, const bf16x8 (&z0)[3], const bf16x8 (&z1)[3], const X3Lane& lb,
                                         F0&& f0 = F0(), F1&& f1 = F1(), F2&& f2 = F2()) {
    bf16x4 l0[3], h0[3], l1[3], h1[3];
    X3_TRFRAG(l0, h0, lb, TILE_OFF, 0, 0);
    X3_TRFRAG(l1, h1, lb, TILE_OFF, 0, 1);
    X3_WAIT6(6, l0, h0);
    { X3_JOIN(t, l0, h0); if (ZA) { ACR_MFMA6(acc0, z0, t); } else { ACR_MFMA6(acc0, t, z0); } }
    f0();
    X3_TRFRAG(l0, h0, lb, TILE_OFF, 1, 0);
    X3_WAIT6(6, l1, h1);
    { X3_JOIN(t, l1, h1); if (ZA) { ACR_MFMA6(acc1, z0, t); } else { ACR_MFMA6(acc1, t, z0); } }
    f1();
    X3_TRFRAG(l1, h1, lb, TILE_OFF, 1, 1);
    X3_WAIT6(6, l0, h0);
    { X3_JOIN(t, l0, h0); if (ZA) { ACR_MFMA6(acc0, z1, t); } else { ACR_MFMA6(acc0, t, z1); } }
    f2();
    X3_WAIT6(0, l1, h1);
    { X3_JOIN(t, l1, h1); if (ZA) { ACR_MFMA6(acc1, z1, t); } else { ACR_MFMA6(acc1, t, z1); } }
}
template <int TILE_OFF, bool ZA, class F0 = X3Nop, class F1 = X3Nop, class F2 = X3Nop>
__device__ __forceinline__ void x3_accop1(f32x16& acc0, f32x16& acc1, const bf16x8 (&z0)[3], const bf16x8 (&z1)[3], const X3Lane& lb,
                                          F0&& f0 = F0(), F1&& f1 = F1(), F2&& f2 = F2()) {
    bf16x4 l0[3], h0[3];
    X3_TRFRAG(l0, h0, lb, TILE_OFF, 0, 0);
    X3_WAIT6(0, l0, h0);
    { X3_JOIN(t, l0, h0); if (ZA) { ACR_MFMA6(acc0, z0, t); } else { ACR_MFMA6(acc0, t, z0); } }
    X3_TRFRAG(l0, h0, lb, TILE_OFF, 0, 1);
    f0();
    X3_WAIT6(0, l0, h0);
    { X3_JOIN(t, l0, h0); if (ZA) { ACR_MFMA6(acc1, z0, t); } else { ACR_MFMA6(acc1, t, z0); } }
    X3_TRFRAG(l0, h0, lb, TILE_OFF, 1, 0);
    f1();
    X3_WAIT6(0, l0, h0);
    { X3_JOIN(t, l0, h0); if (ZA) { ACR_MFMA6(acc0, z1, t); } else { ACR_MFMA6(acc0, t, z1); } }
    X3_TRFRAG(l0, h0, lb, TILE_OFF, 1, 1);
    f2();
    X3_WAIT6(0, l0, h0);
    { X3_JOIN(t, l0, h0); if (ZA) { ACR_MFMA6(acc1, z1, t); } else { ACR_MFMA6(acc1, t, z1); } }
}
__device__ __forceinline__ void x3_rows_from_global(bf16x8 (&y)[3][4], const bf16_t* __restrict__ base, int64_t plane, int D, int row0,
                                                    int Tn, int r, int h) {
    const bf16_t* p0 = base + (int64_t)min(row0 + r, Tn - 1) * D + 8 * h;
#pragma unroll
    for (int p = 0; p < 3; ++p)
#pragma unroll
        for (int s = 0; s < 4; ++s) y[p][s] = *reinterpret_cast<const bf16x8*>(p0 + p * plane + 16 * s);
}

__global__ __launch_bounds__(256, 2) void attn_fwd_x3_kernel(X3Geom g, const bf16_t* __restrict__ qp, const bf16_t* __restrict__ kp,
                                                             const bf16_t* __restrict__ vp, float* __restrict__ o, float* __restrict__ lse2,
                                                             float* __restrict__ sres, const float* __restrict__ q32,
                                                             const float* __restrict__ k32, const float* __restrict__ v32,
                                                             AttnGeom g32, int ntail, char* __restrict__ oimg) {
    __shared__ __attribute__((aligned(1024))) char smem[2 * X3_SLOT_B];
    __shared__ float mlsh[4 * 64];
    const int nmain = (int)gridDim.x - ntail;
    if ((int)blockIdx.x >= nmain) {
        attn_fwd_tail_body<4>(reinterpret_cast<float*>(smem), mlsh, g32, q32, k32, v32, o, lse2, sres, acr_xcd_remap((int)blockIdx.x - nmain, ntail));
        return;
    }
    const int NB = (g.T + 31) >> 5, nqt = ntail ? NB >> 2 : (NB + 3) >> 2;
    int id = acr_xcd_remap(blockIdx.x, nmain);
    const int qt = id % nqt; id /= nqt;
    const int hd = id % g.H;
    const int b = id / g.H;
    const int tid = threadIdx.x, lane = tid & 63;
    const int wave = __builtin_amdgcn_readfirstlane(tid >> 6);
    const int r = lane & 31, h = lane >> 5;
    const int q0 = (qt * 4 + wave) * 32;
    const bool live = q0 < g.T;
    const int64_t pbase = (int64_t)b * g.T * g.D + (int64_t)hd * 64;
    const bf16_t* kb = kp + pbase;
    const bf16_t* vb = vp + pbase;
    x3_dma_tile(smem, kb, g.plane, g.D, 0, g.T, wave, lane);
    x3_dma_tile(smem + X3_TILE_B, vb, g.plane, g.D, 0, g.T, wave, lane);
    bf16x8 qf[3][4];
    x3_rows_from_global(qf, qp + pbase, g.plane, g.D, q0, g.T, r, h);
    float m = -INFINITY, l = 0.f;
    f32x16 o0 = {0}, o1 = {0};
    const X3Lane lb = x3_lane(lane, smem);
    const int doff = x3_dma_off(g.D, wave, lane);
    const float c2 = g.scale * ACR_LOG2E;
    float* sblk = sres + attn_score_block(g.H, NB, b, hd, min(q0 >> 5, NB - 1), 0) + lane * 4;
    auto step = [&](int k0, auto slot_tag) {
        constexpr int SLOT = decltype(slot_tag)::value;
        constexpr int KOFF = SLOT * X3_SLOT_B, VOFF = KOFF + X3_TILE_B;
        x3_barrier((k0 > 0 && live) ? 4 : 0);
        auto dma_next = [&](const bf16_t* base, int toff) {
            if (k0 + 64 <= g.T) x3_dma_tile_i(smem + (SLOT ^ 1) * X3_SLOT_B + toff, base + (int64_t)(k0 + 32) * g.D, g.plane, doff, wave);
            else if (k0 + 32 < g.T) x3_dma_tile(smem + (SLOT ^ 1) * X3_SLOT_B + toff, base, g.plane, g.D, k0 + 32, g.T, wave, lane);
            ATTN_FENCE();
        };
        if (!live) {
            dma_next(kb, 0);
            dma_next(vb, X3_TILE_B);
            return;
        }
        f32x16 s = {0};
        x3_rowop<KOFF>(s, lb, qf, [&] { dma_next(kb, 0); }, [&] { dma_next(vb, X3_TILE_B); });
#pragma unroll
        for (int reg = 0; reg < 16; ++reg) s[reg] *= c2;
        ATTN_MASK_ROWS(s, k0, g.T, h);
        attn_store_scores(sblk + (int64_t)(k0 >> 5) * SB_FLOATS, s);
        f32x16 p;
        ATTN_SOFTMAX_STEP(s, m, l, o0, o1, p);
        bf16x8 p0[3], p1[3];
        split3_bf16_acc<0>(p, p0);
        x3_accop<VOFF, false>(o0, o1, p0, p1, lb, [&] { split3_bf16_acc<1>(p, p1); });
    };
    for (int k0 = 0; k0 < g.T; k0 += 64) {
        step(k0, std::integral_constant<int, 0>{});
        if (k0 + 32 < g.T) step(k0 + 32, std::integral_constant<int, 1>{});
    }
    if (live && q0 + r < g.T) {
        const float inv = 1.f / l;
        ATTN_FWD_FINISH(g, o, lse2, b, hd, q0, r, h, o0, o1, m, l, inv);
        if (oimg != nullptr) {
            const int64_t row = (int64_t)b * g.T + q0 + r;
            const int nkb = g.D >> 4;
            char* ib = oimg + IMG_STAGE_OFF(row >> 7, nkb, hd * 4, 3) + (int)(row & 127) * IMG_ROW_B;
            const int sw = (int)IMG_ROW_SWZ(row);
#pragma unroll
            for (int half = 0; half < 2; ++half)
#pragma unroll
                for (int j = 0; j < 2; ++j) {
                    float own[4], snd[4], rcv[4];
#pragma unroll
                    for (int e = 0; e < 4; ++e) {
                        const float lo = (half ? o1 : o0)[4 * (2 * j) + e] * inv, hi = (half ? o1 : o0)[4 * (2 * j + 1) + e] * inv;
                        own[e] = h ? hi : lo;
                        snd[e] = h ? lo : hi;
                    }
#pragma unroll
                    for (int e = 0; e < 4; ++e) rcv[e] = __shfl_xor(snd[e], 32);
                    const float v8[8] = {h ? rcv[0] : own[0], h ? rcv[1] : own[1], h ? rcv[2] : own[2], h ? rcv[3] : own[3],
                                         h ? own[0] : rcv[0], h ? own[1] : rcv[1], h ? own[2] : rcv[2], h ? own[3] : rcv[3]};
                    bf16x8 p0, p1, p2;
                    split3_bf16(v8, p0, p1, p2);
                    const int c8 = half * 4 + 2 * j + h;
                    char* dst = ib + (c8 >> 1) * (3 * IMG_PLANE_B) + (((c8 & 1) ^ sw) << 4);
                    *reinterpret_cast<bf16x8*>(dst) = p0;
                    *reinterpret_cast<bf16x8*>(dst + IMG_PLANE_B) = p1;
                    *reinterpret_cast<bf16x8*>(dst + 2 * IMG_PLANE_B) = p2;
                }
        }
    }
    if (oimg != nullptr && live && b == g.B - 1 && q0 + 32 >= g.T) {
        const int64_t rows = (int64_t)g.B * g.T, rend = (rows + 127) & ~(int64_t)127;
        const int nkb = g.D >> 4;
        const bf16x8 z = {0};
        for (int i = lane; i < (int)(rend - rows) * 24; i += 64) {
            const int64_t row = rows + i / 24;
            const int rem = i % 24, stage = rem / 6, pl = (rem % 6) >> 1, half = rem & 1;
            char* dst = oimg + IMG_STAGE_OFF(row >> 7, nkb, (int64_t)(hd * 4) + stage, 3) + pl * IMG_PLANE_B + (int)(row & 127) * IMG_ROW_B + half * 16;
            *reinterpret_cast<bf16x8*>(dst) = z;
        }
    }
}

#define X3_BW 8

__device__ __forceinline__ void attn_dq_x3_body(char* smem, float* ssm, float* gsm, int bid, int nblk, bool tails, const X3Geom& g,
                                                const bf16_t* __restrict__ kp, const bf16_t* __restrict__ vp,
                                                const bf16_t* __restrict__ dop, const float* __restrict__ lse2,
                                                const float* __restrict__ delta, const float* __restrict__ sres,
                                                const float* __restrict__ gm, int64_t gm_sb, int64_t gm_st, float* __restrict__ dq) {
    const int NB = (g.T + 31) >> 5, nqt = tails ? NB / X3_BW : (NB + X3_BW - 1) / X3_BW;
    int id = acr_xcd_remap(bid, nblk);
    const int qt = id % nqt; id /= nqt;
    const int hd = id % g.H;
    const int b = id / g.H;
    const int tid = threadIdx.x, lane = tid & 63;
    const int wave = __builtin_amdgcn_readfirstlane(tid >> 6);
    const int r = lane & 31, h = lane >> 5;
    const int q0 = (qt * X3_BW + wave) * 32;
    const bool live = q0 < g.T;
    const int64_t pbase = (int64_t)b * g.T * g.D + (int64_t)hd * 64;
    const int op = wave >> 2, pc = wave & 3;
    const bf16_t* tb = (op ? vp : kp) + pbase;
    char* tdst = smem + op * X3_TILE_B;
    ATTN_QLANE_STREAMS(sres, g.H, NB, g.T, b, hd, q0, wave, lane, ssm, gsm, gm, gm_sb, gm_st);
    x3_dma_tile(tdst, tb, g.plane, g.D, 0, g.T, pc, lane);
    if (live) {
        dma_g(0);
        dma_scores(0, 0);
        if (32 < g.T) dma_scores(1, 1);
    }
    bf16x8 dof[3][4];
    x3_rows_from_global(dof, dop + pbase, g.plane, g.D, q0, g.T, r, h);
    const bool qok = q0 + r < g.T;
    const float l2q = qok ? lse2[((int64_t)b * g.H + hd) * g.T + q0 + r] : INFINITY;
    const float dl = qok ? delta[((int64_t)b * g.H + hd) * g.T + q0 + r] : 0.f;
    const float invH = gb0 ? 1.f / (float)g.H : 0.f;
    f32x16 dq0 = {0}, dq1 = {0};
    const X3Lane lb = x3_lane(lane, smem);
    const int doff = x3_dma_off(g.D, pc, lane);
    ATTN_QLANE_ADDRS(lane, r, h);
    auto step = [&](int k0, auto slot_tag) {
        constexpr int SLOT = decltype(slot_tag)::value;
        constexpr int KOFF = SLOT * X3_SLOT_B, VOFF = KOFF + X3_TILE_B;
        x3_barrier((k0 > 0 && live) ? (gb0 ? 4 : 0) + (k0 + 32 < g.T ? 4 : 0) : 0);
        auto dma_next = [&] {
            if (k0 + 64 <= g.T) x3_dma_tile_i(tdst + (SLOT ^ 1) * X3_SLOT_B, tb + (int64_t)(k0 + 32) * g.D, g.plane, doff, pc);
            else if (k0 + 32 < g.T) x3_dma_tile(tdst + (SLOT ^ 1) * X3_SLOT_B, tb, g.plane, g.D, k0 + 32, g.T, pc, lane);
            ATTN_FENCE();
        };
        if (!live) { dma_next(); return; }
        f32x16 dp = {0};
        x3_rowop<VOFF>(dp, lb, dof, dma_next);
        if (k0 > 0) x3_wait_vm(k0 + 32 < g.T ? 7 : 0);
        f32x4 s4[4], g4[4];
        ATTN_QLANE_READ(SLOT, s4, g4, k0, g.T, h);
        f32x16 ds;
        attn_ds_qlane(ds, s4, g4, dp, l2q, dl, invH);
        bf16x8 z0[3], z1[3];
        split3_bf16_acc<0>(ds, z0);
        x3_accop<KOFF, true>(dq0, dq1, z0, z1, lb,
                             [&] { split3_bf16_acc<1>(ds, z1); },
                             [&] { if (k0 + 32 < g.T) dma_g(k0 + 32); ATTN_FENCE(); },
                             [&] { if (k0 + 64 < g.T) dma_scores((k0 >> 5) + 2, SLOT); ATTN_FENCE(); });
    };
    for (int k0 = 0; k0 < g.T; k0 += 64) {
        step(k0, std::integral_constant<int, 0>{});
        if (k0 + 32 < g.T) step(k0 + 32, std::integral_constant<int, 1>{});
    }
    if (!live) return;
    const int64_t base = (int64_t)b * g.sb + (int64_t)hd * g.sh;
#pragma unroll
    for (int reg = 0; reg < 16; ++reg) {
        const int qq = q0 + acr_krow(reg, h);
        if (qq < g.T) {
            float* p = dq + base + (int64_t)qq * g.st;
            p[r] = dq0[reg] * g.scale;
            p[32 + r] = dq1[reg] * g.scale;
        }
    }
}

__device__ __forceinline__ void attn_dkdv_x3_body(char* smem, float* ssm, float* gsm, float* rcm, int bid, int nblk, bool tails,
                                                  const X3Geom& g,
                                                  const bf16_t* __restrict__ qp, const bf16_t* __restrict__ vp,
                                                  const bf16_t* __restrict__ dop, const float* __restrict__ lse2,
                                                  const float* __restrict__ delta, const float* __restrict__ sres,
                                                  const float* __restrict__ gm, int64_t gm_sb, int64_t gm_st, float* __restrict__ dk,
                                                  float* __restrict__ dv) {
    const int NB = (g.T + 31) >> 5, nkt = tails ? NB / X3_BW : (NB + X3_BW - 1) / X3_BW;
    int id = acr_xcd_remap(bid, nblk);
    const int ktile = id % nkt; id /= nkt;
    const int hd = id % g.H;
    const int b = id / g.H;
    const int tid = threadIdx.x, lane = tid & 63;
    const int wave = __builtin_amdgcn_readfirstlane(tid >> 6);
    const int r = lane & 31, h = lane >> 5;
    const int key0 = (ktile * X3_BW + wave) * 32;
    const bool live = key0 < g.T;
    const int64_t pbase = (int64_t)b * g.T * g.D + (int64_t)hd * 64;
    const int op = wave >> 2, pc = wave & 3;
    const bf16_t* tb = (op ? dop : qp) + pbase;
    char* tdst = smem + op * X3_TILE_B;
    const float* lrow = lse2 + ((int64_t)b * g.H + hd) * g.T;
    const float* drow = delta + ((int64_t)b * g.H + hd) * g.T;
    ATTN_KLANE_STREAMS(sres, g.H, NB, g.T, b, hd, key0, wave, lane, ssm, gsm, gm, gm_sb, gm_st);
    float* rcw = rcm + wave * 64;
    auto dma_rc = [&](int q0) {
        const float* src = (lane < 32 ? lrow : drow) + min(q0 + (lane & 31), g.T - 1);
        __builtin_amdgcn_global_load_lds((glb_vp)src, (lds_vp)rcw, 4, 0, 0);
    };
    x3_dma_tile(tdst, tb, g.plane, g.D, 0, g.T, pc, lane);
    if (live) {
        dma_rc(0);
        dma_g(0);
        dma_scores(0, 0);
        if (32 < g.T) dma_scores(1, 1);
    }
    bf16x8 vf[3][4];
    x3_rows_from_global(vf, vp + pbase, g.plane, g.D, key0, g.T, r, h);
    const float invH = gb0 ? 1.f / (float)g.H : 0.f;
    f32x16 dk0 = {0}, dk1 = {0}, dv0 = {0}, dv1 = {0};
    const X3Lane lb = x3_lane(lane, smem);
    const int doff = x3_dma_off(g.D, pc, lane);
    ATTN_KLANE_ADDRS(ssm, gsm, wave, r, h);
    const uint32_t rcaddr = lds_addr_of(rcw) + 16 * h;
    auto step = [&](int q0, auto slot_tag) {
        constexpr int SLOT = decltype(slot_tag)::value;
        constexpr int QOFF = SLOT * X3_SLOT_B, DOOFF = QOFF + X3_TILE_B;
        x3_barrier((q0 > 0 && live) ? 1 + (gb0 ? 4 : 0) + (q0 + 32 < g.T ? 4 : 0) : 0);
        auto dma_next = [&] {
            if (q0 + 64 <= g.T) x3_dma_tile_i(tdst + (SLOT ^ 1) * X3_SLOT_B, tb + (int64_t)(q0 + 32) * g.D, g.plane, doff, pc);
            else if (q0 + 32 < g.T) x3_dma_tile(tdst + (SLOT ^ 1) * X3_SLOT_B, tb, g.plane, g.D, q0 + 32, g.T, pc, lane);
            ATTN_FENCE();
        };
        if (!live) { dma_next(); return; }
        f32x16 dp = {0};
        x3_rowop<DOOFF>(dp, lb, vf, dma_next);
        if (q0 > 0) x3_wait_vm(q0 + 32 < g.T ? 7 : 0);
        float s[16], gv[16];
        f32x4 l4[4], d4[4];
        ATTN_16(ATTN_RDS, s, SLOT);
        ACR_LDS_RD128(l4[0], rcaddr, 0); ACR_LDS_RD128(l4[1], rcaddr, 32); ACR_LDS_RD128(l4[2], rcaddr, 64); ACR_LDS_RD128(l4[3], rcaddr, 96);
        ACR_LDS_RD128(d4[0], rcaddr, 128); ACR_LDS_RD128(d4[1], rcaddr, 160); ACR_LDS_RD128(d4[2], rcaddr, 192); ACR_LDS_RD128(d4[3], rcaddr, 224);
        ATTN_READ_G(gv)
        asm volatile("s_waitcnt lgkmcnt(0)" : ATTN_V16(s), "+v"(l4[0]), "+v"(l4[1]), "+v"(l4[2]), "+v"(l4[3]), "+v"(d4[0]), "+v"(d4[1]), "+v"(d4[2]), "+v"(d4[3]));
        ATTN_MASK_ROWS(s, q0, g.T, h);
        f32x16 p, ds;
#pragma unroll
        for (int gq = 0; gq < 4; ++gq) {
#pragma unroll
            for (int e = 0; e < 4; ++e) {
                const int reg = 4 * gq + e;
                const float pv = __builtin_amdgcn_exp2f(s[reg] - l4[gq][e]);
                p[reg] = pv;
                ds[reg] = pv * (dp[reg] + gv[reg] * invH - d4[gq][e]);
            }
        }
        asm volatile("s_waitcnt lgkmcnt(0)" ::: "memory");
        bf16x8 z0[3], z1[3];
        split3_bf16_acc<0>(p, z0);
        x3_accop<DOOFF, true>(dv0, dv1, z0, z1, lb,
                              [&] { split3_bf16_acc<1>(p, z1); },
                              [&] { if (q0 + 32 < g.T) dma_rc(q0 + 32); ATTN_FENCE(); },
                              [&] { if (q0 + 32 < g.T) dma_g(q0 + 32); ATTN_FENCE(); });
        split3_bf16_acc<0>(ds, z0);
        x3_accop<QOFF, true>(dk0, dk1, z0, z1, lb,
                             [&] { split3_bf16_acc<1>(ds, z1); },
                             [&] { if (q0 + 64 < g.T) dma_scores((q0 >> 5) + 2, SLOT); ATTN_FENCE(); });
    };
    for (int q0 = 0; q0 < g.T; q0 += 64) {
        step(q0, std::integral_constant<int, 0>{});
        if (q0 + 32 < g.T) step(q0 + 32, std::integral_constant<int, 1>{});
    }
    if (!live) return;
    const int64_t base = (int64_t)b * g.sb + (int64_t)hd * g.sh;
#pragma unroll
    for (int reg = 0; reg < 16; ++reg) {
        const int kk = key0 + acr_krow(reg, h);
        if (kk < g.T) {
            float* pk = dk + base + (int64_t)kk * g.st;
            float* pv = dv + base + (int64_t)kk * g.st;
            pk[r] = dk0[reg] * g.scale;
            pk[32 + r] = dk1[reg] * g.scale;
            pv[r] = dv0[reg];
            pv[32 + r] = dv1[reg];
        }
    }
}

__global__ __launch_bounds__(64 * X3_BW, 2) void attn_bwd_x3_kernel(X3Geom g, const bf16_t* __restrict__ qp, const bf16_t* __restrict__ kp,
                                                                   const bf16_t* __restrict__ vp, const bf16_t* __restrict__ dop,
                                                                   const float* __restrict__ lse2, const float* __restrict__ delta,
                                                                   const float* __restrict__ sres, const float* __restrict__ gm,
                                                                   int64_t gm_sb, int64_t gm_st, float* __restrict__ dq,
                                                                   float* __restrict__ dk, float* __restrict__ dv,
                                                                   const float* __restrict__ q32, const float* __restrict__ k32,
                                                                   const float* __restrict__ v32, const float* __restrict__ do32,
                                                                   AttnGeom g32, int ntail) {
    __shared__ __attribute__((aligned(1024))) char lds[2 * X3_SLOT_B + X3_BW * 3 * SB_FLOATS * 4 + X3_BW * 256];
    char* smem = lds;
    float* ssm = reinterpret_cast<float*>(lds + 2 * X3_SLOT_B);
    float* gsm = ssm + X3_BW * 2 * SB_FLOATS;
    float* rcm = gsm + X3_BW * SB_FLOATS;
    const int half = ((int)gridDim.x - 2 * ntail) >> 1;
    const int bid = (int)blockIdx.x;
    if (bid < half)
        attn_dkdv_x3_body(smem, ssm, gsm, rcm, bid, half, ntail != 0, g, qp, vp, dop, lse2, delta, sres, gm, gm_sb, gm_st, dk, dv);
    else if (bid < 2 * half)
        attn_dq_x3_body(smem, ssm, gsm, bid - half, half, ntail != 0, g, kp, vp, dop, lse2, delta, sres, gm, gm_sb, gm_st, dq);
    else if (bid < 2 * half + ntail)
        attn_dkdv_tail_body<X3_BW>(reinterpret_cast<float*>(lds), reinterpret_cast<float*>(lds) + X3_BW * DT_FLOATS, g32, q32, v32, do32, lse2,
                                   delta, sres, gm, gm_sb, gm_st, dk, dv, acr_xcd_remap(bid - 2 * half, ntail));
    else
        attn_dq_tail_body<X3_BW>(reinterpret_cast<float*>(lds), g32, k32, v32, do32, lse2, delta, sres, gm, gm_sb, gm_st, dq,
                                 acr_xcd_remap(bid - 2 * half - ntail, ntail));
}

int64_t acr_attn_x3_scores_floats(const AttnGeom& g) {
    return attn_score_floats(g.B, g.H, g.T) + 9 * ((int64_t)g.B * g.T * g.H * 64) / 2;
}
int64_t acr_attn_x3_bwd_ws_floats(const AttnGeom& g) {
    return (((int64_t)g.B * g.H * g.T + 3) & ~(int64_t)3) + 3 * ((int64_t)g.B * g.T * g.H * 64) / 2;
}
static X3Geom x3_geom(const AttnGeom& g) {
    X3Geom x;
    x.B = g.B; x.H = g.H; x.T = g.T; x.D = g.H * 64; x.scale = g.scale;
    x.plane = (int64_t)g.B * g.T * x.D;
    x.osb = g.osb; x.ost = g.ost; x.osh = g.osh;
    x.sb = g.sb; x.st = g.st; x.sh = g.sh;
    return x;
}

bool acr_attn_x3_fwd_uses_split_tail(int T) {
    const int NB = (T + 31) / 32;
    return attn_split_tail(NB, 4) && NB >= 33;
}

void acr_attn_fwd_f32_x3(const AttnGeom& g, const float* q, const float* k, const float* v, float* o, float* lse2, float* scores,
                         float* pmean, int64_t pmean_sb, int64_t pmean_st, hipStream_t st, char* oimg) {
    const X3Geom x = x3_geom(g);
    bf16_t* planes = reinterpret_cast<bf16_t*>(scores + attn_score_floats(g.B, g.H, g.T));
    X3SplitArgs a;
    a.src[0] = q; a.src[1] = k; a.src[2] = v;
    a.sb = g.sb; a.st = g.st; a.sh = g.sh; a.dst = planes; a.plane = x.plane; a.B = g.B; a.T = g.T; a.H = g.H;
    const int64_t n8 = (int64_t)g.B * g.T * g.H * 8;
    hipLaunchKernelGGL(x3_split_kernel, dim3((unsigned)((n8 + 255) / 256), 3), dim3(256), 0, st, a);
    const int NB = (g.T + 31) / 32;
    const int ntail = (acr_attn_x3_fwd_uses_split_tail(g.T) && oimg == nullptr) ? g.B * g.H : 0;
    hipLaunchKernelGGL(attn_fwd_x3_kernel, dim3(g.B * g.H * (ntail ? NB / 4 : (NB + 3) / 4) + ntail), dim3(256), 0, st, x, (const bf16_t*)planes,
                       (const bf16_t*)(planes + 3 * x.plane), (const bf16_t*)(planes + 6 * x.plane), o, lse2, scores, q, k, v, g, ntail, oimg);
    if (pmean) acr_attn_pmean_sres(g, scores, lse2, pmean, pmean_sb, pmean_st, st);
}

void acr_attn_bwd_f32_x3(const AttnGeom& g, const float* q, const float* k, const float* v, const float* o, const float* d_o,
                         const float* lse2, const float* scores, const float* gm, int64_t gm_sb, int64_t gm_st, float* dq, float* dk,
                         float* dv, float* delta_ws, hipStream_t st) {
    const X3Geom x = x3_geom(g);
    const bf16_t* planes = reinterpret_cast<const bf16_t*>(scores + attn_score_floats(g.B, g.H, g.T));
    bf16_t* dop = reinterpret_cast<bf16_t*>(delta_ws + (((int64_t)g.B * g.H * g.T + 3) & ~(int64_t)3));
    X3SplitArgs a;
    a.src[0] = d_o; a.src[1] = a.src[2] = nullptr;
    a.sb = g.osb; a.st = g.ost; a.sh = g.osh; a.dst = dop; a.plane = x.plane; a.B = g.B; a.T = g.T; a.H = g.H;
    const int64_t n8 = (int64_t)g.B * g.T * g.H * 8;
    hipLaunchKernelGGL(x3_split_kernel, dim3((unsigned)((n8 + 255) / 256), 1), dim3(256), 0, st, a);
    acr_attn_delta_sres(g, scores, o, d_o, lse2, gm, gm_sb, gm_st, delta_ws, st);
    const int NB = (g.T + 31) / 32;
    const int ntail = attn_split_tail(NB, X3_BW) ? g.B * g.H : 0;
    const int nmain = g.B * g.H * (ntail ? NB / X3_BW : (NB + X3_BW - 1) / X3_BW);
    hipLaunchKernelGGL(attn_bwd_x3_kernel, dim3(2 * nmain + 2 * ntail), dim3(64 * X3_BW), 0, st, x, planes, planes + 3 * x.plane,
                       planes + 6 * x.plane, (const bf16_t*)dop, lse2, (const float*)delta_ws, scores, gm, gm_sb, gm_st, dq, dk, dv, q, k, v, d_o, g,
                       ntail);
}

extern "C" int acr_split3_bf16(const float* x, int64_t rows, int64_t cols, int64_t ld, void* planes, int64_t plane_stride, void* stream) {
    ACR_CHECK_ARG(x && planes, "acr_split3_bf16: null pointer");
    ACR_CHECK_ARG(rows > 0 && cols > 0 && (cols % 8) == 0 && (ld % 4) == 0 && ld >= cols, "acr_split3_bf16: need cols %% 8 == 0, ld %% 4 == 0, ld >= cols");
    ACR_CHECK_ARG(plane_stride >= rows * cols && (plane_stride % 8) == 0, "acr_split3_bf16: plane stride must cover rows * cols and be a multiple of 8");
    ACR_CHECK_ARG(((uintptr_t)x & 15) == 0 && ((uintptr_t)planes & 15) == 0, "acr_split3_bf16: 16-byte alignment");
    const int64_t n = rows * (cols >> 3);
    ACR_CHECK_ARG((n + 255) / 256 < (1ll << 31), "acr_split3_bf16: too large");
    hipLaunchKernelGGL(x3_split2d_kernel, dim3((unsigned)((n + 255) / 256)), dim3(256), 0, (hipStream_t)stream, x, rows, cols, ld,
                       (bf16_t*)planes, plane_stride);
    return acr_check_launch("acr_split3_bf16");
}
```

### acr_wsss_amd/ops.py

```python
import os
import numpy as np
import torch
from torch.autograd import Function

from . import _abi
from . import _derived
from . import _lib as L

HEAD_DIM = 64
ATTN_F32_SCORES = True


def pad4(n):
    return (n + 3) & ~3


def _desc(B, H, T, dtype, packed_qkv=True, math=0):
    D = H * HEAD_DIM
    d = L.AttnDesc()
    d.B, d.H, d.T, d.head_dim = B, H, T, HEAD_DIM
    d.dtype = L.ACR_F32_BF16X3 if (math == 1 and dtype == torch.float32) else L.dtype_code(dtype)
    d.scale = HEAD_DIM ** -0.5
    d.qkv_sb, d.qkv_st, d.qkv_sh = T * 3 * D, 3 * D, HEAD_DIM
    d.o_sb, d.o_st, d.o_sh = T * D, D, HEAD_DIM
    return d


def _qkv_ptrs(qkv, H):
    esz = qkv.element_size()
    base = qkv.data_ptr()
    D = H * HEAD_DIM
    return (L.c_void_p(base), L.c_void_p(base + D * esz), L.c_void_p(base + 2 * D * esz))


class MeanStack:

    def __init__(self, B, Lyr, T, device):
        self.buf = torch.empty((B, Lyr, T, T), dtype=torch.float32, device=device)
        self.n_layers = Lyr



class KernelTimer:

    def __init__(self):
        self.samples, self._seen, self._open = {}, set(), []

    def next_step(self):
        self._seen.clear()

    def begin(self, key):
        if key in self._seen:
            return None
        self._seen.add(key)
        e0, e1 = torch.cuda.Event(enable_timing=True), torch.cuda.Event(enable_timing=True)
        e0.record()
        return key, e0, e1

    def end(self, tok):
        tok[2].record()
        self._open.append(tok)

    def collect(self):
        torch.cuda.synchronize()
        for key, e0, e1 in self._open:
            self.samples.setdefault(key, []).append(e0.elapsed_time(e1))
        self._open = []
        return self.samples


KERNEL_TIMER = None


def _t0(name, *dims):
    return KERNEL_TIMER.begin("%s %s" % (name, "x".join(str(int(d)) for d in dims))) if KERNEL_TIMER is not None else None


def _t1(tok):
    if tok is not None:
        KERNEL_TIMER.end(tok)

class AttnCoreFn(Function):

    @staticmethod
    def forward(ctx, qkv, heads, stack, layer, owner, math=0, want_oimg=False):
        L.require_gpu(qkv)
        ctx.set_materialize_grads(False)
        if not qkv.is_contiguous():
            qkv = qkv.contiguous()
        B, T, D3 = qkv.shape
        D = heads * HEAD_DIM
        assert D3 == 3 * D, "qkv last dim %d != 3*heads*64" % D3
        lib = L.load()
        keep_scores = ctx.needs_input_grad[0]
        ctx.math = math = int(math == 1 and ATTN_F32_SCORES and qkv.dtype == torch.float32 and (keep_scores or stack is not None))
        d = _desc(B, heads, T, qkv.dtype, math=math)
        o = torch.empty((B, T, D), dtype=qkv.dtype, device=qkv.device)
        lse2 = torch.empty((B, heads, T), dtype=torch.float32, device=qkv.device)
        pm = None
        if stack is not None:
            pm = stack.buf[:, layer]
        qp, kp, vp = _qkv_ptrs(qkv, heads)
        scores = None
        if ATTN_F32_SCORES and qkv.dtype == torch.float32 and (keep_scores or pm is not None):
            scores = torch.empty(lib.acr_attn_scores_floats(d), dtype=torch.float32, device=qkv.device)
        tok = _t0("attn_fwd" if pm is not None else "attn_fwd_nomean", B, heads, T)
        pm_sb, pm_st = (pm.stride(0), pm.stride(1)) if pm is not None else (0, 0)
        oimg = None
        if want_oimg and scores is not None and math == 1 and lib.acr_attn_fwd_oimg_offered(d):
            oimg = x3_image_empty(B * T, D, qkv.device)
        if oimg is not None:
            L.check(lib.acr_attn_fwd_scores_oimg(d, qp, kp, vp, L.ptr(o), L.ptr(lse2), L.ptr(scores), L.ptr(pm), pm_sb, pm_st, L.ptr(oimg),
                                                 L.stream_ptr()), "acr_attn_fwd_scores_oimg")
        elif scores is not None:
            L.check(lib.acr_attn_fwd_scores(d, qp, kp, vp, L.ptr(o), L.ptr(lse2), L.ptr(scores), L.ptr(pm), pm_sb, pm_st,
                                            L.stream_ptr()), "acr_attn_fwd_scores")
        else:
            L.check(lib.acr_attn_fwd(d, qp, kp, vp, L.ptr(o), L.ptr(lse2), L.ptr(pm), pm_sb, pm_st, L.stream_ptr()),
                    "acr_attn_fwd")
        _t1(tok)
        if scores is not None and keep_scores:
            ctx.save_for_backward(qkv, o, lse2, scores)
        else:
            ctx.save_for_backward(qkv, o, lse2)
        ctx.heads = heads
        keep = owner is not None and (not owner.training or getattr(owner, "keep_state_in_training", False))
        ctx.owner = owner if keep else None
        if owner is not None:
            owner._saved = (qkv, lse2, heads) if keep else None
            owner._saved_do = None
            owner._saved_gpm = None
        if want_oimg:
            if oimg is not None:
                ctx.mark_non_differentiable(oimg)
            return o, pm, oimg
        if pm is None:
            return o, None
        return o, pm

    @staticmethod
    def backward(ctx, d_o, g_pm, *unused):
        saved = ctx.saved_tensors
        qkv, o, lse2 = saved[:3]
        scores = saved[3] if len(saved) > 3 else None
        heads = ctx.heads
        B, T, _ = qkv.shape
        lib = L.load()
        if d_o is None:
            d_o = torch.zeros_like(o)
        if not d_o.is_contiguous():
            d_o = d_o.contiguous()
        if d_o.dtype != qkv.dtype:
            d_o = d_o.to(qkv.dtype)
        gm_sb = gm_st = 0
        if g_pm is not None:
            ok = (g_pm.dtype == torch.float32 and g_pm.stride(2) == 1 and g_pm.stride(1) % 4 == 0
                  and g_pm.stride(1) >= pad4(T) and g_pm.stride(0) % 4 == 0 and g_pm.data_ptr() % 16 == 0)
            if not ok:
                buf = torch.zeros((B, T, pad4(T)), dtype=torch.float32, device=qkv.device)
                buf[:, :, :T].copy_(g_pm)
                g_pm = buf[:, :, :T]
            gm_sb, gm_st = g_pm.stride(0), g_pm.stride(1)
        d = _desc(B, heads, T, qkv.dtype, math=ctx.math if scores is not None else 0)
        dqkv = torch.empty_like(qkv)
        delta = torch.empty(lib.acr_attn_bwd_ws_floats(d) if scores is not None else B * heads * T, dtype=torch.float32, device=qkv.device)
        qp, kp, vp = _qkv_ptrs(qkv, heads)
        dqp, dkp, dvp = _qkv_ptrs(dqkv, heads)
        tok = _t0("attn_bwd" if g_pm is not None else "attn_bwd_nomean", B, heads, T)
        if scores is not None:
            L.check(lib.acr_attn_bwd_scores(d, qp, kp, vp, L.ptr(o), L.ptr(d_o), L.ptr(lse2), L.ptr(scores), L.ptr(g_pm), gm_sb,
                                            gm_st, dqp, dkp, dvp, L.ptr(delta), L.stream_ptr()), "acr_attn_bwd_scores")
        else:
            L.check(lib.acr_attn_bwd(d, qp, kp, vp, L.ptr(o), L.ptr(d_o), L.ptr(lse2), L.ptr(g_pm), gm_sb, gm_st,
                                     dqp, dkp, dvp, L.ptr(delta), L.stream_ptr()), "acr_attn_bwd")
        _t1(tok)
        if ctx.owner is not None:
            ctx.owner._saved_do = d_o
            ctx.owner._saved_gpm = g_pm
        return dqkv, None, None, None, None, None, None


class StackAliasFn(Function):

    @staticmethod
    def forward(ctx, stack, *pms):
        ctx.n = len(pms)
        return stack.buf

    @staticmethod
    def backward(ctx, g):
        return (None,) + tuple(g[:, l] for l in range(ctx.n))


def attention_core(qkv, heads, stack=None, layer=0, owner=None, math=0):
    return AttnCoreFn.apply(qkv, heads, stack, layer, owner, math)


def attention_core_oimg(qkv, heads, stack=None, layer=0, owner=None, math=0):
    return AttnCoreFn.apply(qkv, heads, stack, layer, owner, math, True)


def attn_probs(qkv, lse2, heads):
    B, T, _ = qkv.shape
    lib = L.load()
    out = torch.empty((B, heads, T, T), dtype=torch.float32, device=qkv.device)
    qp, kp, _ = _qkv_ptrs(qkv, heads)
    L.check(lib.acr_attn_probs(_desc(B, heads, T, qkv.dtype), qp, kp, L.ptr(lse2), L.ptr(out), L.stream_ptr()),
            "acr_attn_probs")
    return out


def attn_dprobs(qkv, d_o, heads):
    B, T, _ = qkv.shape
    lib = L.load()
    out = torch.empty((B, heads, T, T), dtype=torch.float32, device=qkv.device)
    _, _, vp = _qkv_ptrs(qkv, heads)
    L.check(lib.acr_attn_dprobs(_desc(B, heads, T, qkv.dtype), L.ptr(d_o), vp, L.ptr(out), L.stream_ptr()),
            "acr_attn_dprobs")
    return out


def getam_row_accum(qkv, d_o, lse2, heads, batch, func, cam_row):
    B, T, _ = qkv.shape
    lib = L.load()
    qp, kp, vp = _qkv_ptrs(qkv, heads)
    L.check(lib.acr_getam_row_accum(_desc(B, heads, T, qkv.dtype), qp, kp, vp, L.ptr(d_o), L.ptr(lse2), batch,
                                    L.GETAM_FUNCS[func], L.ptr(cam_row), L.stream_ptr()), "acr_getam_row_accum")


def getam_rows_accum(qkv, d_o, lse2, heads, func, cam_rows):
    B, T, _ = qkv.shape
    lib = L.load()
    qp, kp, vp = _qkv_ptrs(qkv, heads)
    assert cam_rows.shape == (B, T) and cam_rows.stride(1) == 1
    L.check(lib.acr_getam_rows_accum(_desc(B, heads, T, qkv.dtype), qp, kp, vp, L.ptr(d_o), L.ptr(lse2), L.GETAM_FUNCS[func],
                                     L.ptr(cam_rows), cam_rows.stride(0), L.stream_ptr()), "acr_getam_rows_accum")


def linear_bf16(x, weight, bias=None, resid=None, out=None):
    L.require_gpu(x, weight)
    M, K = x.shape
    N = weight.shape[0]
    assert x.dtype == torch.bfloat16 and weight.dtype == torch.bfloat16 and x.stride(1) == 1 and weight.stride(1) == 1
    if out is None:
        out = torch.empty((M, N), dtype=torch.bfloat16, device=x.device)
    tok = _t0("linear_bf16", M, N, K)
    L.check(L.load().acr_linear_bf16(L.ptr(x), x.stride(0), L.ptr(weight), weight.stride(0), L.ptr(bias),
                                     L.ptr(resid), resid.stride(0) if resid is not None else 0, L.ptr(out),
                                     out.stride(0), M, N, K, L.stream_ptr()), "acr_linear_bf16")
    _t1(tok)
    return out


def colsum_bf16(dy2):
    M, N = dy2.shape
    lib = L.load()
    if N % 8 or dy2.stride(1) != 1 or dy2.stride(0) % 8 or dy2.data_ptr() % 16:
        return dy2.sum(dim=0)
    ws = torch.empty(lib.acr_colsum_ws_floats(M, N), dtype=torch.float32, device=dy2.device)
    out = torch.empty(N, dtype=torch.bfloat16, device=dy2.device)
    L.check(lib.acr_colsum_bf16(L.ptr(dy2), dy2.stride(0), M, N, L.ptr(ws), L.ptr(out), L.stream_ptr()), "acr_colsum_bf16")
    return out


def wgrad_bf16(dy2, x2):
    M, N = dy2.shape
    K = x2.shape[1]
    lib = L.load()
    nws = lib.acr_wgrad_ws_floats(M, N, K)
    if (nws == 0 or dy2.stride(1) != 1 or x2.stride(1) != 1 or dy2.stride(0) % 8 or x2.stride(0) % 8
            or dy2.data_ptr() % 16 or x2.data_ptr() % 16):
        return torch.mm(dy2.t(), x2)
    ws = torch.empty(nws, dtype=torch.float32, device=dy2.device)
    dw = torch.empty((N, K), dtype=torch.bfloat16, device=dy2.device)
    tok = _t0("wgrad_bf16", M, N, K)
    L.check(lib.acr_wgrad_bf16(L.ptr(dy2), dy2.stride(0), L.ptr(x2), x2.stride(0), M, N, K, L.ptr(ws), L.ptr(dw),
                               L.stream_ptr()), "acr_wgrad_bf16")
    _t1(tok)
    return dw


def wgrad_bias_bf16(dy2, x2):
    M, N = dy2.shape
    K = x2.shape[1]
    lib = L.load()
    nws = lib.acr_wgrad_bias_ws_floats(M, N, K)
    if (nws == 0 or N % 8 or dy2.stride(1) != 1 or x2.stride(1) != 1 or dy2.stride(0) % 8 or x2.stride(0) % 8
            or dy2.data_ptr() % 16 or x2.data_ptr() % 16):
        return wgrad_bf16(dy2, x2), colsum_bf16(dy2)
    ws = torch.empty(nws, dtype=torch.float32, device=dy2.device)
    dw = torch.empty((N, K), dtype=torch.bfloat16, device=dy2.device)
    db = torch.empty(N, dtype=torch.bfloat16, device=dy2.device)
    tok = _t0("wgrad_bf16", M, N, K)
    L.check(lib.acr_wgrad_bias_bf16(L.ptr(dy2), dy2.stride(0), L.ptr(x2), x2.stride(0), M, N, K, L.ptr(ws), L.ptr(dw), L.ptr(db),
                                    L.stream_ptr()), "acr_wgrad_bias_bf16")
    _t1(tok)
    return dw, db


def transpose_records(srcs, dsts, shapes):
    rec = np.zeros(len(shapes), _abi.record_dtype("acr_tr_tensor"))
    bt, t0 = [], 0
    for i, (src, dst, (rows, cols)) in enumerate(zip(srcs, dsts, shapes)):
        tr, tc = (rows + 63) // 64, (cols + 63) // 64
        rec[i] = (src, dst, rows, cols, t0, tc)
        bt.append(np.full(tr * tc, i, dtype=np.int32))
        t0 += tr * tc
    return rec, np.concatenate(bt), t0


class WeightTransposes:

    def __init__(self, modules, dtype=torch.bfloat16):
        mult = 8 if dtype == torch.bfloat16 else 4
        self.dtype = dtype
        self.lins = [m for m in modules if isinstance(m, torch.nn.Linear) and m.weight.is_cuda and m.weight.dtype == dtype
                     and m.weight.is_contiguous() and m.weight.shape[0] % mult == 0 and m.weight.shape[1] % mult == 0
                     and m.weight.shape[0] >= 64 and m.weight.requires_grad]
        self.ok = bool(self.lins)
        if not self.ok:
            return
        dev = self.lins[0].weight.device
        self.bufs = [torch.empty(tuple(m.weight.shape)[::-1], dtype=dtype, device=dev) for m in self.lins]
        self._ptrs = [m.weight.data_ptr() for m in self.lins]
        rec, blk, self.nblocks = transpose_records(self._ptrs, [wt.data_ptr() for wt in self.bufs], [tuple(m.weight.shape) for m in self.lins])
        self.table = torch.from_numpy(rec.view(np.uint8).copy()).to(dev)
        self.blk = torch.from_numpy(blk).to(dev)

    @torch.no_grad()
    def refresh(self):
        if not self.ok:
            return
        if any(m.weight.data_ptr() != p for m, p in zip(self.lins, self._ptrs)):
            self.ok = False
            for m in self.lins:
                _derived.entries(m).pop("t", None)
            return
        fn = L.load().acr_transpose_many_bf16 if self.dtype == torch.bfloat16 else L.load().acr_transpose_many_f32
        L.check(fn(L.ptr(self.table), L.ptr(self.blk), self.nblocks, L.stream_ptr()), "acr_transpose_many")
        for m, wt in zip(self.lins, self.bufs):
            _derived.put(m, "t", m.weight, wt)


def weight_t(weight, owner=None, make=True):
    wt = _derived.get(owner, "t", weight)
    return weight.t().contiguous() if wt is None and make else wt


F32_WT = True


def _dx_f32(dy2, weight, owner, out, aux=None, act=0, math=0):
    wt = weight_t(weight, owner, make=False) if F32_WT else None
    if wt is not None:
        return gemm_f32_raw("nt", dy2, wt, out, aux=aux, act=act, math=math)
    return gemm_f32_raw("nn", dy2, weight, out, aux=aux, act=act, math=math)


class LinearBf16Fn(Function):

    @staticmethod
    def forward(ctx, x, weight, bias, resid, owner=None):
        ctx.owner = owner
        shp = x.shape
        x2 = x.reshape(-1, shp[-1])
        r2 = resid.reshape(-1, weight.shape[0]) if resid is not None else None
        y = linear_bf16(x2, weight, bias, r2)
        ctx.save_for_backward(x2, weight)
        ctx.has_bias, ctx.has_resid = bias is not None, resid is not None
        return y.reshape(*shp[:-1], weight.shape[0])

    @staticmethod
    def backward(ctx, dy):
        x2, weight = ctx.saved_tensors
        dy2 = dy.reshape(-1, dy.shape[-1])
        if not dy2.is_contiguous():
            dy2 = dy2.contiguous()
        dx = dw = db = None
        if ctx.needs_input_grad[0]:
            if weight.shape[0] % 64 == 0:
                dx = linear_bf16(dy2, weight_t(weight, ctx.owner))
            else:
                dx = torch.mm(dy2, weight)
            dx = dx.reshape(*dy.shape[:-1], weight.shape[1])
        want_db = ctx.has_bias and ctx.needs_input_grad[2]
        if ctx.needs_input_grad[1] and want_db:
            dw, db = wgrad_bias_bf16(dy2, x2)
        else:
            if ctx.needs_input_grad[1]:
                dw = wgrad_bf16(dy2, x2)
            if want_db:
                db = colsum_bf16(dy2)
        return dx, dw, db, (dy if ctx.has_resid else None), None


def _al16(*ts):
    return all(t is None or t.data_ptr() % 16 == 0 for t in ts)


def mlp_fusable(x, fc1, fc2):
    return (x.is_cuda and x.dtype == torch.bfloat16 and x.is_contiguous() and fc1.weight.dtype == torch.bfloat16
            and fc1.bias is not None and fc2.bias is not None and fc1.weight.shape[1] % 64 == 0
            and fc1.weight.shape[0] % 64 == 0 and fc2.weight.shape[0] % 64 == 0
            and _al16(x, fc1.weight, fc1.bias, fc2.weight, fc2.bias))


class MlpFn(Function):

    @staticmethod
    def forward(ctx, x, w1, b1, w2, b2, resid, fc1=None, fc2=None):
        ctx.fc1, ctx.fc2 = fc1, fc2
        shp = x.shape
        x2 = x.reshape(-1, shp[-1])
        M, K = x2.shape
        Hd = w1.shape[0]
        lib = L.load()
        h = torch.empty((M, Hd), dtype=torch.bfloat16, device=x.device)
        a = torch.empty((M, Hd), dtype=torch.bfloat16, device=x.device)
        tok = _t0("linear_bf16", M, Hd, K)
        L.check(lib.acr_linear_gelu_bf16(L.ptr(x2), x2.stride(0), L.ptr(w1), w1.stride(0), L.ptr(b1), L.ptr(h), L.ptr(a), Hd,
                                         M, Hd, K, L.stream_ptr()), "acr_linear_gelu_bf16")
        _t1(tok)
        r2 = resid.reshape(-1, w2.shape[0]) if resid is not None else None
        y = linear_bf16(a, w2, b2, r2)
        ctx.save_for_backward(x2, h, a, w1, w2)
        ctx.has_resid = resid is not None
        return y.reshape(*shp[:-1], w2.shape[0])

    @staticmethod
    def backward(ctx, dy):
        x2, h, a, w1, w2 = ctx.saved_tensors
        dy2 = dy.reshape(-1, dy.shape[-1])
        if not dy2.is_contiguous():
            dy2 = dy2.contiguous()
        M, Hd = h.shape
        lib = L.load()
        need = ctx.needs_input_grad
        dw1 = db1 = dw2 = db2 = None
        if need[3] and need[4]:
            dw2, db2 = wgrad_bias_bf16(dy2, a)
        elif need[3]:
            dw2 = wgrad_bf16(dy2, a)
        elif need[4]:
            db2 = colsum_bf16(dy2)
        w2t = weight_t(w2, ctx.fc2)
        dh = torch.empty_like(h)
        L.check(lib.acr_linear_dgelu_bf16(L.ptr(dy2), dy2.stride(0), L.ptr(w2t), w2t.stride(0), L.ptr(h), h.stride(0), L.ptr(dh),
                                          dh.stride(0), M, Hd, dy2.shape[1], L.stream_ptr()), "acr_linear_dgelu_bf16")
        if need[1] and need[2]:
            dw1, db1 = wgrad_bias_bf16(dh, x2)
        elif need[1]:
            dw1 = wgrad_bf16(dh, x2)
        elif need[2]:
            db1 = colsum_bf16(dh)
        dx = None
        if need[0]:
            dx = linear_bf16(dh, weight_t(w1, ctx.fc1)).reshape(*dy.shape[:-1], w1.shape[1])
        return dx, dw1, db1, dw2, db2, (dy if ctx.has_resid else None), None, None


def mlp(x, fc1, fc2, resid=None):
    return MlpFn.apply(x, fc1.weight, fc1.bias, fc2.weight, fc2.bias, resid, fc1, fc2)


GEMM_MODES = {m: _abi.constants["ACR_GEMM_" + m.upper()] for m in ("nt", "nn", "tn")}


def gemm_f32_raw(mode, a, b, c, bias=None, aux=None, act=0, c2=None, colsum=None, math=0):
    lib = L.load()
    md = GEMM_MODES[mode]
    M, N = c.shape
    K = a.shape[0] if md == 2 else a.shape[1]
# ... 1031 lines not shown
```

### include/acr_hip.h

```cpp
#ifndef ACR_HIP_H
#define ACR_HIP_H

#include <stddef.h>
#include <stdint.h>

#ifdef __cplusplus
extern "C" {
#endif

#define ACR_ABI_VERSION 2

typedef enum acr_status {
    ACR_OK = 0,
    ACR_ERR_INVALID = -1,
    ACR_ERR_LAUNCH = -2,
    ACR_ERR_UNSUPPORTED = -3
} acr_status;

typedef enum acr_dtype { ACR_F32 = 0, ACR_BF16 = 1, ACR_BF16_F32MATH = 2, ACR_F32_BF16X3 = 3 } acr_dtype;

typedef enum acr_math { ACR_MATH_F32 = 0, ACR_MATH_BF16X3 = 1, ACR_MATH_FP16X2 = 2 } acr_math;
#define ACR_FP16X2_REL 2.384185791015625e-07
#define ACR_FP16X2_FLOOR 1.8189894035458565e-12

typedef enum acr_getam_func {
    ACR_GETAM_GRAD = 0, ACR_GETAM_CAM_GRAD = 1, ACR_GETAM_GRAD_S = 2, ACR_GETAM_CAM_GRAD_S = 3
} acr_getam_func;

typedef struct acr_attn_desc {
    int32_t B, H, T, head_dim;
    int32_t dtype;
    float   scale;
    int64_t qkv_sb, qkv_st, qkv_sh;
    int64_t o_sb, o_st, o_sh;
} acr_attn_desc;

int         acr_version(void);
const char* acr_last_error(void);

typedef enum acr_option {
    ACR_OPT_ATTN_DELTA_1HEAD = 7,
} acr_option;
int     acr_set_option(int32_t option, int32_t value);
int32_t acr_get_option(int32_t option);

int acr_attn_fwd(const acr_attn_desc* desc, const void* q, const void* k, const void* v,
                 void* o, float* lse2, float* pmean, int64_t pmean_sb, int64_t pmean_st, void* stream);

int acr_attn_bwd(const acr_attn_desc* desc, const void* q, const void* k, const void* v,
                 const void* o, const void* d_o, const float* lse2,
                 const float* gmean, int64_t gmean_sb, int64_t gmean_st,
                 void* dq, void* dk, void* dv, float* delta_ws, void* stream);

int64_t acr_attn_scores_floats(const acr_attn_desc* desc);
int64_t acr_attn_bwd_ws_floats(const acr_attn_desc* desc);
int acr_split3_bf16(const float* x, int64_t rows, int64_t cols, int64_t ld, void* planes, int64_t plane_stride, void* stream);
int acr_attn_fwd_scores(const acr_attn_desc* desc, const void* q, const void* k, const void* v,
                        void* o, float* lse2, float* scores, float* pmean, int64_t pmean_sb, int64_t pmean_st, void* stream);
int acr_attn_fwd_scores_oimg(const acr_attn_desc* desc, const void* q, const void* k, const void* v,
                             void* o, float* lse2, float* scores, float* pmean, int64_t pmean_sb, int64_t pmean_st, float* o_image,
                             void* stream);
int acr_attn_fwd_oimg_offered(const acr_attn_desc* desc);
int acr_attn_bwd_scores(const acr_attn_desc* desc, const void* q, const void* k, const void* v,
                        const void* o, const void* d_o, const float* lse2, const float* scores,
                        const float* gmean, int64_t gmean_sb, int64_t gmean_st,
                        void* dq, void* dk, void* dv, float* delta_ws, void* stream);

int acr_attn_probs(const acr_attn_desc* desc, const void* q, const void* k, const float* lse2,
                   float* probs, void* stream);
int acr_attn_dprobs(const acr_attn_desc* desc, const void* d_o, const void* v,
                    float* dprobs, void* stream);

int acr_linear_bf16(const void* a, int64_t lda, const void* b, int64_t ldb, const void* bias,
                    const void* resid, int64_t ldr, void* y, int64_t ldy, int32_t M, int32_t N, int32_t K,
                    void* stream);
int acr_linear_gelu_bf16(const void* a, int64_t lda, const void* w, int64_t ldw, const void* bias, void* h, void* act,
                         int64_t ldy, int32_t M, int32_t N, int32_t K, void* stream);
int acr_linear_dgelu_bf16(const void* a, int64_t lda, const void* w, int64_t ldw, const void* h, int64_t ldh, void* y,
                          int64_t ldy, int32_t M, int32_t N, int32_t K, void* stream);


typedef enum acr_gemm_mode { ACR_GEMM_NT = 0, ACR_GEMM_NN = 1, ACR_GEMM_TN = 2 } acr_gemm_mode;
size_t acr_gemm_f32_ws_floats(int32_t mode, int32_t math, int32_t M, int32_t N, int32_t K);
int acr_gemm_f32(int32_t mode, int32_t math, int32_t act, const float* a, int64_t lda, const float* b, int64_t ldb, const float* bias,
                 const float* aux, int64_t ldaux, float* c, int64_t ldc, float* c2, float* colsum, int32_t M, int32_t N,
                 int32_t K, float* ws, void* stream);

size_t acr_wgrad_ws_floats(int32_t M, int32_t N, int32_t K);
int acr_wgrad_bf16(const void* dy, int64_t ldy, const void* x, int64_t ldx, int32_t M, int32_t N, int32_t K,
                   float* ws, void* dw, void* stream);
size_t acr_wgrad_bias_ws_floats(int32_t M, int32_t N, int32_t K);
int acr_wgrad_bias_bf16(const void* dy, int64_t ldy, const void* x, int64_t ldx, int32_t M, int32_t N, int32_t K, float* ws,
                        void* dw, void* dbias, void* stream);


size_t acr_colsum_ws_floats(int32_t M, int32_t N);
int acr_colsum_bf16(const void* dy, int64_t ld, int32_t M, int32_t N, float* ws, void* out, void* stream);

int acr_conv1x1_bf16(const void* w, int64_t ldw, const void* x, const void* addend, void* y, int32_t nsamp, int32_t cout,
                     int32_t cin, int32_t hw, void* stream);
size_t acr_conv1x1_wgrad_ws_floats(int32_t nsamp, int32_t cout, int32_t cin, int32_t hw);
int acr_conv1x1_wgrad_bf16(const void* dy, const void* x, int32_t nsamp, int32_t cout, int32_t cin, int32_t hw,
                           float* ws, void* dw, void* stream);

size_t acr_conv1x1_ws_floats(int32_t math, int32_t nsamp, int32_t cout, int32_t cin, int32_t hw);
int acr_conv1x1_f32(int32_t math, const float* w, int32_t w_transposed, const float* x, const float* addend, float* y, int32_t nsamp,
                    int32_t cout, int32_t cin, int32_t hw, float* ws, void* stream);
int acr_conv1x1_x3(const float* w_img, const float* x, const float* addend, float* y, int32_t nsamp, int32_t cout, int32_t cin, int32_t hw,
                   float* ws, void* stream);
size_t acr_conv1x1_wgrad_f32_ws_floats(int32_t nsamp, int32_t cout, int32_t cin, int32_t hw);
int acr_conv1x1_wgrad_f32(int32_t math, const float* dy, const float* x, int32_t nsamp, int32_t cout, int32_t cin, int32_t hw, float* ws,
                          float* dw, void* stream);

size_t acr_x3_image_floats(int32_t rows, int32_t cols);
size_t acr_x3_colsum_ws_floats(int32_t rows, int32_t cols);
int acr_x3_image(const float* x, int64_t ld, int32_t rows, int32_t cols, float* image, float* colsum, float* colsum_ws, void* stream);
int acr_x3_image_t(const float* x, int64_t ld, int32_t rows, int32_t cols, float* image, void* stream);
size_t acr_gemm_x3_ws_floats(int32_t mode, int32_t act, int32_t M, int32_t N, int32_t K);
typedef struct acr_x3_many_desc {
    const float* src;
    void* dst;
    int32_t rows, K, sr, kin, sko, ski, wg0, nkb;
} acr_x3_many_desc;
int acr_x3_image_many(const void* descs, const int32_t* blk, int32_t nwg, void* stream);
int acr_gemm_x3(int32_t mode, int32_t act, const float* a_img, const float* b_img, const float* bias, const float* aux, int64_t ldaux, float* c,
                int64_t ldc, float* c2, float* colsum, int32_t M, int32_t N, int32_t K, float* ws, void* stream);

typedef enum acr_h2_dir { ACR_H2_ROWS = 0, ACR_H2_COLS = 1 } acr_h2_dir;
size_t acr_h2_image_floats(int32_t rows, int32_t cols);
size_t acr_h2_ws_floats(int32_t rows, int32_t cols);
int acr_h2_image(const float* x, int64_t ld, int32_t rows, int32_t cols, float* image, float* colsum, float* ws, void* stream);
int acr_h2_image_cols(const float* x, int64_t ld, int32_t rows, int32_t cols, float* image, float* colsum, float* ws, void* stream);
int acr_h2_image_t(const float* x, int64_t ld, int32_t rows, int32_t cols, float* image, float* ws, void* stream);
size_t acr_gemm_h2_ws_floats(int32_t mode, int32_t act, int32_t M, int32_t N, int32_t K);
int acr_gemm_h2(int32_t mode, int32_t act, const float* a_img, const float* b_img, const float* bias, const float* aux, int64_t ldaux, float* c,
                int64_t ldc, float* c2, int32_t M, int32_t N, int32_t K, float* ws, void* stream);

size_t acr_conv3x3_ws_floats(int32_t nsamp, int32_t cout, int32_t cin, int32_t H, int32_t W);
int acr_conv3x3_f32(int32_t math, const float* w_packed, const float* x, float* y, int32_t nsamp, int32_t cout, int32_t cin,
                    int32_t H, int32_t W, float* ws, void* stream);
int acr_conv3x3_x3(const float* w_img, const float* x, float* y, int32_t nsamp, int32_t cout, int32_t cin, int32_t H, int32_t W, float* ws,
                   void* stream);
size_t acr_conv3x3_wgrad_ws_floats(int32_t nsamp, int32_t cout, int32_t cin, int32_t H, int32_t W);
int acr_conv3x3_wgrad_f32(int32_t math, const float* dy, const float* x, int32_t nsamp, int32_t cout, int32_t cin, int32_t H, int32_t W,
                          float* ws, float* dw_packed, void* stream);

int acr_space_to_depth2_f32(const float* x, float* xs, int32_t nsamp, int32_t C, int32_t H, int32_t W, int32_t xrows, void* stream);
int acr_depth_to_space2_f32(const float* xs, float* x, int32_t nsamp, int32_t C, int32_t H, int32_t W, void* stream);
size_t acr_conv_taps_ws_floats(int32_t nsamp, int32_t cout, int32_t cin, int32_t H, int32_t W, int32_t ntap);
int acr_conv_taps_x3(const float* w_img, const float* x, float* y, int32_t nsamp, int32_t cout, int32_t cin, int32_t H, int32_t W, int32_t ntap,
                     const int32_t* tdy, const int32_t* tdx, const int32_t* tcb, int32_t xrows, int32_t yrows, float* ws, void* stream);
size_t acr_conv_taps_wgrad_ws_floats(int32_t nsamp, int32_t cout, int32_t cin, int32_t H, int32_t W, int32_t ntap);
int acr_conv_taps_wgrad_f32(int32_t math, const float* dy, const float* x, int32_t nsamp, int32_t cout, int32_t cin, int32_t H, int32_t W,
                            int32_t ntap, const int32_t* tdy, const int32_t* tdx, const int32_t* tcb, int32_t xrows, float* ws, float* dw_packed,
                            void* stream);

int acr_maxpool3x3s2_fwd_bf16(const void* x, void* y, uint8_t* amax, int64_t nc, int32_t h, int32_t w, int32_t ho,
                              int32_t wo, int32_t pad_top, int32_t pad_left, void* stream);
int acr_maxpool3x3s2_bwd_bf16(const void* dy, const uint8_t* amax, void* dx, int64_t nc, int32_t h, int32_t w,
                              int32_t ho, int32_t wo, int32_t pad_top, int32_t pad_left, void* stream);
int acr_maxpool3x3s2_fwd_f32(const void* x, void* y, uint8_t* amax, int64_t nc, int32_t h, int32_t w, int32_t ho,
                             int32_t wo, int32_t pad_top, int32_t pad_left, void* stream);
int acr_maxpool3x3s2_bwd_f32(const void* dy, const uint8_t* amax, void* dx, int64_t nc, int32_t h, int32_t w,
                             int32_t ho, int32_t wo, int32_t pad_top, int32_t pad_left, void* stream);
int acr_subsample2_fwd_f32(const float* x, float* y, int64_t nc, int32_t h, int32_t w, void* stream);
int acr_subsample2_bwd_f32(const float* dy, float* dx, int64_t nc, int32_t h, int32_t w, void* stream);

typedef struct acr_sgd_tensor {
    const void* grad;
    float* master;
    float* mom;
    void* param;
    int64_t n;
} acr_sgd_tensor;
int32_t acr_sgd_chunk_elems(void);
int acr_sgd_step_bf16(const void* table, const int32_t* blk_tensor, const int32_t* blk_chunk, int32_t nblocks, float lr,
                      float momentum, void* stream);
int acr_sgd_step_f32(const void* table, const int32_t* blk_tensor, const int32_t* blk_chunk, int32_t nblocks, float lr,
                     float momentum, void* stream);

typedef struct acr_tr_tensor {
    const void* src;
    void* dst;
    int32_t rows, cols;
    int32_t tile0;
    int32_t tiles_c;
} acr_tr_tensor;
int acr_transpose_many_bf16(const void* table, const int32_t* blk_tensor, int32_t nblocks, void* stream);
int acr_transpose_many_f32(const void* table, const int32_t* blk_tensor, int32_t nblocks, void* stream);

size_t acr_layernorm_ws_floats(int32_t M, int32_t C);
int acr_layernorm_fwd_bf16(const void* x, const void* gamma, const void* beta, void* y, float* stats, int32_t M,
                           int32_t C, float eps, void* stream);
int acr_layernorm_bwd_bf16(const void* dy, const void* x, const void* gamma, const float* stats, const void* dskip,
                           void* dx, float* ws, void* dgamma, void* dbeta, int32_t M, int32_t C, void* stream);

int acr_layernorm_fwd_f32(const float* x, const float* gamma, const float* beta, float* y, float* stats, int32_t M, int32_t C,
                          float eps, void* stream);
int acr_layernorm_bwd_f32(const float* dy, const float* x, const float* gamma, const float* stats, const float* dskip, float* dx,
                          float* ws, float* dgamma, float* dbeta, int32_t M, int32_t C, void* stream);
int acr_layernorm_image_f32(const float* x, const float* gamma, const float* beta, float* image, float* stats, int32_t M, int32_t C, float eps,
                            void* stream);

int acr_tokens_fwd_f32(const float* y, const float* bias, const float* prefix, const float* pos, float* tok, int32_t B, int32_t D, int32_t T,
                       int32_t P, void* stream);
int acr_tokens_bwd_f32(const float* dtok, float* dy, float* dpos, int32_t B, int32_t D, int32_t T, int32_t P, void* stream);

int acr_groupnorm_fwd_bf16(const void* x, const void* resid, const void* gamma, const void* beta, void* y,
                           float* stats, int32_t N, int32_t C, int32_t HW, float eps, int32_t act, void* stream);
int acr_groupnorm_bwd_bf16(const void* dy, const void* x, const void* resid, const void* gamma, const void* beta,
                           const float* stats, void* dx, void* dresid, float* dgamma_part, float* dbeta_part,
                           void* dgamma, void* dbeta, int32_t N, int32_t C, int32_t HW, int32_t act, void* stream);

size_t acr_groupnorm_fwd_ws_floats(int32_t N, int32_t C, int32_t HW);
int acr_groupnorm_fwd_f32(const float* x, const float* resid, const float* gamma, const float* beta, float* y, float* stats,
                          int32_t N, int32_t C, int32_t HW, float eps, int32_t act, float* ws, void* stream);
int acr_groupnorm_bwd_f32(const float* dy, const float* x, const float* resid, const float* gamma, const float* beta,
                          const float* stats, float* dx, float* dresid, float* dgamma_part, float* dbeta_part, float* dgamma,
                          float* dbeta, int32_t N, int32_t C, int32_t HW, int32_t act, void* stream);
int acr_groupnorm_fwd_mask_f32(const float* x, const float* resid, const float* gamma, const float* beta, float* y, float* stats,
                               int32_t N, int32_t C, int32_t HW, float eps, uint8_t* relu_mask, void* stream);
int acr_groupnorm_bwd_mask_f32(const float* dy, const float* x, const uint8_t* relu_mask, const float* gamma, const float* beta,
                               const float* stats, float* dx, float* dresid, float* dgamma_part, float* dbeta_part, float* dgamma,
                               float* dbeta, int32_t N, int32_t C, int32_t HW, void* stream);

typedef struct acr_wstd_desc {
    uint64_t p0, p1, p2, p3;
    int32_t cout, n, ch_start, pad;
} acr_wstd_desc;
int acr_weight_std_bf16(const void* desc_dev, int32_t n_conv, int32_t total_channels, float eps, int32_t backward,
                        void* stream);
int acr_weight_std_f32(const void* desc_dev, int32_t n_conv, int32_t total_channels, float eps, int32_t backward,
                       void* stream);

int acr_mlsm_fwd_f32(const float* x, int64_t ldx, const float* y, int64_t ldy, int32_t N, int32_t C, float* loss, void* stream);
int acr_mlsm_bwd_f32(const float* x, int64_t ldx, const float* y, int64_t ldy, const float* g, int32_t N, int32_t C, float* dx, void* stream);

size_t acr_consistency_ws_floats(int32_t B, int32_t L, int32_t T);
int acr_consistency_fwd(const float* a1, const float* a2, int64_t a_sb, int32_t B, int32_t L,
                        int32_t T, int32_t p, float* partial_ws, float* out2, void* stream);
int acr_consistency_bwd(const float* a1, const float* a2, int64_t a_sb, int32_t B, int32_t L,
                        int32_t T, int32_t p, const float* gout2, float* g1, float* g2,
                        int64_t g_sb, int64_t g_st, void* stream);

int acr_getam_row_accum(const acr_attn_desc* desc, const void* q, const void* k, const void* v,
                        const void* d_o, const float* lse2, int32_t batch, int32_t func,
                        float* cam_row, void* stream);
int acr_getam_rows_accum(const acr_attn_desc* desc, const void* q, const void* k, const void* v, const void* d_o,
                         const float* lse2, int32_t func, float* cam_rows, int64_t row_stride, void* stream);

int acr_aff_refine(const float* a, int32_t L, int32_t T, const float* cam, int32_t n_cam,
                   float* out, void* stream);
int acr_aff_refine_batch(const float* a, int64_t a_sb, int32_t L, int32_t T, const float* cam, int32_t n_cam,
                         int32_t nbatch, float* out, void* stream);

typedef struct acr_pre_image {
    int64_t offset;
    int32_t h, w;
    int32_t rh, rw;
    int32_t flip;
    int32_t cont_top, cont_left, img_top, img_left, ch, cw;
} acr_pre_image;
int acr_preprocess_batch(const void* packed_u8, const void* table, int32_t batch, int32_t S, const float* mean3,
                         const float* std3, int32_t out_dtype, void* out, void* stream);

int acr_preprocess_seg_batch(const void* packed_u8, const void* table, const int64_t* map_offsets, int32_t batch, int32_t S,
                             const float* mean3, const float* std3, int32_t out_dtype, int32_t map_fill, void* images,
                             void* ori_u8, void* croppings, void* map_u8, void* stream);

int64_t acr_lattice_ws_bytes(int32_t n_pixels, int32_t d);
int acr_lattice_build(const void* rgb, int32_t H, int32_t W, float sxy, float srgb, void* ws, int64_t ws_bytes, void* stream);
int acr_lattice_info(const void* ws, int32_t* n_points, int32_t* key_overflow, void* stream);
int acr_lattice_tables(void* ws, int32_t n_pixels, int32_t d, void** offsets, void** weights, void** point_keys);
int acr_lattice_filter(const void* ws, int32_t n_pixels, int32_t d, int32_t n_points, const void* in, const void* pre, void* out,
                       const void* post, float post_scale, int32_t apply_scale, int32_t K, void* vals, void* stream);
int acr_crf_unary(const void* probs, void* unary, int64_t n, float clip, void* stream);
int acr_crf_norm(void* norm, int32_t n_pixels, void* stream);
int acr_crf_update(const void* unary, const void* msg0, const void* msg1, void* q, int32_t n_pixels, int32_t K, void* stream);
int acr_crf_alpha_unary(const void* cams, int32_t n_cls, int32_t n_pixels, const void* alphas, int32_t n_alpha, float clip, void* scores,
                        void* unary, void* q, void* stream);
int acr_crf_update_groups(const void* unary, const void* msg0, const void* msg1, void* q, int32_t n_pixels, int32_t K, int32_t G, void* stream);
int acr_crf_label_unary(const uint8_t* labels_u8, int32_t n_pixels, int32_t n_labels, float e_label, float e_other, float e_unsure, void* unary,
                        void* q, void* stream);
int acr_crf_update_argmax(const void* unary, const void* msg0, const void* msg1, int32_t n_pixels, int32_t K, uint8_t* label_u8, void* stream);

int acr_patch_cam(const void* x, int64_t x_st, const void* w, const void* bias, int32_t N, int32_t D,
                  int32_t C, int32_t dtype, float* out, void* stream);
int acr_bilinear_resize(const float* src, int64_t src_sc, int64_t src_sp, int32_t C, int32_t ih,
                        int32_t iw, float* dst, int32_t oh, int32_t ow, int32_t align_corners,
                        const float* chan_mul, int32_t hflip, int32_t accumulate, void* stream);

int acr_pamr_affinity(const float* x, int32_t B, int32_t K, int32_t H, int32_t W, const int32_t* dilations, int32_t n_dil,
                      float* w_out, void* stream);
int acr_pamr_propagate(const float* w, const float* mask_in, float* mask_out, int32_t B, int32_t C, int32_t H, int32_t W,
                       const int32_t* dilations, int32_t n_dil, void* stream);

#define ACR_EVAL_MAX_CLS 128
#define ACR_EVAL_MAX_NT 256
int acr_eval_sweep_f32(const float* cams, const int32_t* classes, int32_t n, const uint8_t* gt, int32_t h, int32_t w,
                       const float* thresholds, int32_t nt, int32_t num_cls, int64_t* raw, void* stream);
int acr_eval_sweep_finish(const int64_t* raw, int32_t nt, int32_t num_cls, int64_t* TP, int64_t* P, void* stream);
int acr_eval_confusion_u8(const uint8_t* pred, const uint8_t* gt, int64_t n_pixels, int32_t num_cls, int64_t* conf, void* stream);

#define ACR_PSEUDO_MAX_LABELS 128
int64_t acr_pseudo_ws_bytes(int32_t K, int32_t h, int32_t w);
int acr_pseudo_label_f32(const float* scores, const int32_t* classes, int32_t K, int32_t h, int32_t w, int32_t num_classes,
                         uint8_t* out, void* stream);
int acr_pseudo_compose(const float* cams, const int32_t* classes, int32_t K, const float* la, const float* ha, int32_t h, int32_t w,
                       int32_t num_classes, int32_t ignore_uncertain, double bg_alpha, float cam_floor, double fg_quantile,
                       float bg_sure, float crf_sure, void* ws, int64_t ws_bytes, uint8_t* out, void* stream);

#define ACR_SAL_PSEUDO_MAX_CLASSES 127
int64_t acr_sal_pseudo_ws_bytes(int32_t B, int32_t C, int32_t h, int32_t w);
int acr_sal_pseudo_compose(const float* cams, const uint8_t* present, int32_t B, int32_t C, int32_t h, int32_t w, const uint8_t* saliency,
                           double bg_alpha, double cut, int32_t open_size, void* ws, int64_t ws_bytes, uint8_t* label,
                           uint8_t* saliency_out, void* stream);
int acr_morph_open_u8(const uint8_t* src, int32_t B, int32_t h, int32_t w, int32_t k, uint8_t* dst, void* stream);

#define ACR_DENSE_ENERGY_WS_BYTES 2048
#define ACR_SEG_MAX_K 128
int64_t acr_segloss_ws_bytes(int32_t B, int32_t K, int32_t h, int32_t w, int32_t W, int32_t H);
int acr_segloss_fwd(const float* logits, const uint8_t* label, int32_t B, int32_t K, int32_t h, int32_t w, int32_t W, int32_t H,
                    int32_t batch_average, void* ws, int64_t ws_bytes, float* probs, float* rowstat, float* sums, int64_t* counts,
                    float* loss, void* stream);
int acr_segloss_bwd(const float* logits, const uint8_t* label, const float* rowstat, const int64_t* counts, const float* g,
                    const float* probs, const float* d_probs, int32_t B, int32_t K, int32_t h, int32_t w, int32_t W, int32_t H,
                    int32_t batch_average, void* ws, int64_t ws_bytes, float* d_logits, void* stream);
int acr_dense_energy_dot(const float* s, const float* as, int64_t count, float grad_scale, float* grad, void* ws, int64_t ws_bytes,
                         float* out, void* stream);

int64_t acr_bn2d_ws_bytes(int32_t N, int32_t C, int32_t HW);
int acr_bn2d_fwd(const float* x, const float* gamma, const float* beta, float* running_mean, float* running_var, const float* resid,
                 const float* resid2, int32_t N, int32_t C, int32_t HW, int32_t training, double eps, double momentum, int32_t relu,
                 void* ws, int64_t ws_bytes, double* stats, float* y, void* stream);
int acr_bn2d_bwd(const float* x, const float* y, const float* dy, const float* gamma, const double* stats, int32_t N, int32_t C,
                 int32_t HW, int32_t training, int32_t relu, void* ws, int64_t ws_bytes, float* dx, float* dgamma, float* dbeta,
                 float* dres, void* stream);
int acr_bn2d_moments(const float* x, int32_t N, int32_t C, int32_t HW, void* ws, int64_t ws_bytes, double* moments, void* stream);
int acr_bn2d_fwd_merged(const float* x, const float* gamma, const float* beta, float* running_mean, float* running_var,
                        const float* resid, const float* resid2, int32_t N, int32_t C, int32_t HW, const double* gathered, int32_t W,
                        double eps, double momentum, int32_t relu, void* ws, int64_t ws_bytes, double* stats, float* y, void* stream);
int acr_bn2d_bwd_sums(const float* x, const float* y, const float* dy, const double* stats, int32_t N, int32_t C, int32_t HW,
                      int32_t relu, void* ws, int64_t ws_bytes, double* sums, float* dgamma, float* dbeta, void* stream);
int acr_bn2d_bwd_merged(const float* x, const float* y, const float* dy, const float* gamma, const double* stats,
                        const double* gathered_sums, int32_t W, int32_t N, int32_t C, int32_t HW, int32_t relu, void* ws,
                        int64_t ws_bytes, float* dx, float* dres, void* stream);
int acr_relu_fwd_f32(const float* x, int64_t n, float* y, void* stream);
int acr_relu_bwd_f32(const float* y, const float* dy, int64_t n, float* dx, void* stream);
int acr_upsample2x_fwd(const float* x, int64_t planes, int32_t H, int32_t W, int32_t OH, int32_t OW, float* y, void* stream);
int acr_upsample2x_bwd(const float* dy, int64_t planes, int32_t H, int32_t W, int32_t OH, int32_t OW, float* dx, void* stream);

int acr_bn2d_fwd_bf16(const void* x, const void* gamma, const void* beta, float* running_mean, float* running_var, const void* resid,
                      const void* resid2, int32_t N, int32_t C, int32_t HW, int32_t training, double eps, double momentum, int32_t relu,
                      void* ws, int64_t ws_bytes, double* stats, void* y, void* stream);
int acr_bn2d_bwd_bf16(const void* x, const void* y, const void* dy, const void* gamma, const double* stats, int32_t N, int32_t C,
                      int32_t HW, int32_t training, int32_t relu, void* ws, int64_t ws_bytes, void* dx, float* dgamma, float* dbeta,
                      void* dres, void* stream);
int acr_bn2d_moments_bf16(const void* x, int32_t N, int32_t C, int32_t HW, void* ws, int64_t ws_bytes, double* moments, void* stream);
int acr_bn2d_fwd_merged_bf16(const void* x, const void* gamma, const void* beta, float* running_mean, float* running_var,
                             const void* resid, const void* resid2, int32_t N, int32_t C, int32_t HW, const double* gathered, int32_t W,
                             double eps, double momentum, int32_t relu, void* ws, int64_t ws_bytes, double* stats, void* y,
                             void* stream);
int acr_bn2d_bwd_sums_bf16(const void* x, const void* y, const void* dy, const double* stats, int32_t N, int32_t C, int32_t HW,
                           int32_t relu, void* ws, int64_t ws_bytes, double* sums, float* dgamma, float* dbeta, void* stream);
int acr_bn2d_bwd_merged_bf16(const void* x, const void* y, const void* dy, const void* gamma, const double* stats,
                             const double* gathered_sums, int32_t W, int32_t N, int32_t C, int32_t HW, int32_t relu, void* ws,
                             int64_t ws_bytes, void* dx, void* dres, void* stream);
int acr_relu_fwd_bf16(const void* x, int64_t n, void* y, void* stream);
int acr_relu_bwd_bf16(const void* y, const void* dy, int64_t n, void* dx, void* stream);
// ... 55 lines not shown
```

Baseline: 126.3 img/s.

## Split x3 attention backward into dK/dV kernel that stores dS and dQ kernel

For the bf16x3 fp32-emulation path, the attention backward no longer runs a fused kernel where the dQ sweep recomputes dS. The dK/dV kernel now writes dS to a new workspace, and a separate dQ kernel streams that dS and multiplies it by K. This removes the duplicated softmax-gradient computation in the dQ sweep. In exchange it adds a full score-sized fp32 buffer write and read, a per-call allocation and a second launch.

After: 127.4 img/s, median of 6. Within noise of the previous version (+0.8%).

```diff
diff --git a/acr_wsss_amd/csrc/attn_f32.h b/acr_wsss_amd/csrc/attn_f32.h
--- a/acr_wsss_amd/csrc/attn_f32.h
+++ b/acr_wsss_amd/csrc/attn_f32.h
@@ -27,9 +27,10 @@
 
 int64_t acr_attn_x3_scores_floats(const AttnGeom& g);
 int64_t acr_attn_x3_bwd_ws_floats(const AttnGeom& g);
+int64_t acr_attn_x3_bwd_ds_floats(const AttnGeom& g);
 bool acr_attn_x3_fwd_uses_split_tail(int T);
 void acr_attn_fwd_f32_x3(const AttnGeom& g, const float* q, const float* k, const float* v, float* o, float* lse2, float* scores,
                          float* pmean, int64_t pmean_sb, int64_t pmean_st, hipStream_t st, char* oimg = nullptr);
 void acr_attn_bwd_f32_x3(const AttnGeom& g, const float* q, const float* k, const float* v, const float* o, const float* d_o,
                          const float* lse2, const float* scores, const float* gm, int64_t gm_sb, int64_t gm_st, float* dq, float* dk,
-                         float* dv, float* delta_ws, hipStream_t st);
+                         float* dv, float* delta_ws, float* ds_ws, hipStream_t st);
diff --git a/acr_wsss_amd/csrc/attn_f32.hip b/acr_wsss_amd/csrc/attn_f32.hip
--- a/acr_wsss_amd/csrc/attn_f32.hip
+++ b/acr_wsss_amd/csrc/attn_f32.hip
@@ -649,33 +649,56 @@
     return acr_attn_x3_fwd_uses_split_tail(d->T) ? 0 : 1;
 }
 
+static int attn_bwd_scores(const char* who, bool with_ds, const acr_attn_desc* d, const void* q, const void* k, const void* v, const void* o,
+                           const void* d_o, const float* lse2, const float* scores, const float* gmean, int64_t gmean_sb,
+                           int64_t gmean_st, void* dq, void* dk, void* dv, float* delta_ws, float* ds_ws, void* stream) {
+    int rc = check_desc(d, who);
+    if (rc) return rc;
+    if (with_ds && d->dtype != ACR_F32_BF16X3) {
+        acr_set_error("%s: ACR_F32_BF16X3 only (the exact-fp32 sweeps keep no dS)", who);
+        return ACR_ERR_UNSUPPORTED;
+    }
+    if (d->dtype != ACR_F32 && d->dtype != ACR_F32_BF16X3) {
+        acr_set_error("%s: fp32 tensors only (the bf16 kernels recompute the logits)", who);
+        return ACR_ERR_UNSUPPORTED;
+    }
+    ACR_CHECK_ARG(q && k && v && o && d_o && lse2 && scores && dq && dk && dv && delta_ws, "%s: null pointer", who);
+    ACR_CHECK_ARG(aligned16(q) && aligned16(k) && aligned16(v) && aligned16(o) && aligned16(d_o) && aligned16(scores),
+                  "%s: inputs must be 16-byte aligned", who);
+    rc = check_gmean(d, who, gmean, gmean_sb, gmean_st);
+    if (rc) return rc;
+    ACR_CHECK_ARG(!gmean || ((gmean_st & 3) == 0 && (gmean_sb & 3) == 0 && aligned16(gmean)),
+                  "%s: gmean must be 16-byte aligned with pitch and batch stride multiples of 4 floats", who);
+    if (d->dtype == ACR_F32_BF16X3) {
+        rc = check_x3(d, who);
+        if (rc) return rc;
+        ACR_CHECK_ARG(!with_ds || (ds_ws != nullptr && aligned16(ds_ws)), "%s: ds_ws must be a 16-byte aligned workspace", who);
+        ACR_CHECK_ARG(aligned16(delta_ws) && aligned16(dq) && aligned16(dk) && aligned16(dv), "%s: delta_ws / dq / dk / dv must be 16-byte aligned", who);
+        acr_attn_bwd_f32_x3(geom(d), (const float*)q, (const float*)k, (const float*)v, (const float*)o, (const float*)d_o, lse2, scores,
+                            gmean, gmean_sb, gmean_st, (float*)dq, (float*)dk, (float*)dv, delta_ws, ds_ws, (hipStream_t)stream);
+        return acr_check_launch(who);
+    }
+    acr_attn_bwd_f32_sres(geom(d), (const float*)q, (const float*)k, (const float*)v, (const float*)o, (const float*)d_o, lse2,
+                          scores, gmean, gmean_sb, gmean_st, (float*)dq, (float*)dk, (float*)dv, delta_ws, (hipStream_t)stream);
+    return acr_check_launch(who);
+}
+
 extern "C" int acr_attn_bwd_scores(const acr_attn_desc* d, const void* q, const void* k, const void* v, const void* o,
                                    const void* d_o, const float* lse2, const float* scores, const float* gmean, int64_t gmean_sb,
                                    int64_t gmean_st, void* dq, void* dk, void* dv, float* delta_ws, void* stream) {
-    int rc = check_desc(d, "acr_attn_bwd_scores");
-    if (rc) return rc;
-    if (d->dtype != ACR_F32 && d->dtype != ACR_F32_BF16X3) {
-        acr_set_error("acr_attn_bwd_scores: fp32 tensors only (the bf16 kernels recompute the logits)");
-        return ACR_ERR_UNSUPPORTED;
-    }
-    ACR_CHECK_ARG(q && k && v && o && d_o && lse2 && scores && dq && dk && dv && delta_ws, "acr_attn_bwd_scores: null pointer");
-    ACR_CHECK_ARG(aligned16(q) && aligned16(k) && aligned16(v) && aligned16(o) && aligned16(d_o) && aligned16(scores),
-                  "acr_attn_bwd_scores: inputs must be 16-byte aligned");
-    rc = check_gmean(d, "acr_attn_bwd_scores", gmean, gmean_sb, gmean_st);
-    if (rc) return rc;
-    ACR_CHECK_ARG(!gmean || ((gmean_st & 3) == 0 && (gmean_sb & 3) == 0 && aligned16(gmean)),
-                  "acr_attn_bwd_scores: gmean must be 16-byte aligned with pitch and batch stride multiples of 4 floats");
-    if (d->dtype == ACR_F32_BF16X3) {
-        rc = check_x3(d, "acr_attn_bwd_scores");
-        if (rc) return rc;
-        ACR_CHECK_ARG(aligned16(delta_ws) && aligned16(dq) && aligned16(dk) && aligned16(dv), "acr_attn_bwd_scores: delta_ws / dq / dk / dv must be 16-byte aligned");
-        acr_attn_bwd_f32_x3(geom(d), (const float*)q, (const float*)k, (const float*)v, (const float*)o, (const float*)d_o, lse2, scores,
-                            gmean, gmean_sb, gmean_st, (float*)dq, (float*)dk, (float*)dv, delta_ws, (hipStream_t)stream);
-        return acr_check_launch("acr_attn_bwd_scores");
-    }
-    acr_attn_bwd_f32_sres(geom(d), (const float*)q, (const float*)k, (const float*)v, (const float*)o, (const float*)d_o, lse2,
-                          scores, gmean, gmean_sb, gmean_st, (float*)dq, (float*)dk, (float*)dv, delta_ws, (hipStream_t)stream);
-    return acr_check_launch("acr_attn_bwd_scores");
+    return attn_bwd_scores("acr_attn_bwd_scores", false, d, q, k, v, o, d_o, lse2, scores, gmean, gmean_sb, gmean_st, dq, dk, dv, delta_ws,
+                           nullptr, stream);
+}
+
+extern "C" int64_t acr_attn_bwd_ds_floats(const acr_attn_desc* d) {
+    if (d == nullptr || d->B <= 0 || d->H <= 0 || d->T <= 0 || d->dtype != ACR_F32_BF16X3) return 0;
+    return acr_attn_x3_bwd_ds_floats(geom(d));
+}
+extern "C" int acr_attn_bwd_scores_ds(const acr_attn_desc* d, const void* q, const void* k, const void* v, const void* o,
+                                      const void* d_o, const float* lse2, const float* scores, const float* gmean, int64_t gmean_sb,
+                                      int64_t gmean_st, void* dq, void* dk, void* dv, float* delta_ws, float* ds_ws, void* stream) {
+    return attn_bwd_scores("acr_attn_bwd_scores_ds", true, d, q, k, v, o, d_o, lse2, scores, gmean, gmean_sb, gmean_st, dq, dk, dv, delta_ws,
+                           ds_ws, stream);
 }
 
 extern "C" int acr_attn_probs(const acr_attn_desc* d, const void* q, const void* k, const float* lse2, float* probs,
diff --git a/acr_wsss_amd/csrc/attn_f32_scores.h b/acr_wsss_amd/csrc/attn_f32_scores.h
--- a/acr_wsss_amd/csrc/attn_f32_scores.h
+++ b/acr_wsss_amd/csrc/attn_f32_scores.h
@@ -87,9 +87,9 @@
         ds[reg] = __builtin_amdgcn_exp2f(s4[reg >> 2][reg & 3] - l2q) * (dp[reg] + g4[reg >> 2][reg & 3] * invH - dl);
 }
 
-#define ATTN_KLANE_STREAMS(sres, H, NB, T, b, hd, key0, wave, lane, ssm, gsm, gm, gm_sb, gm_st)                                     \
-    const float* scol = sres + attn_score_block(H, NB, b, hd, 0, min(key0 >> 5, NB - 1));                                           \
-    const int64_t sstep = (int64_t)NB * SB_FLOATS;                                                                                  \
+#define ATTN_KLANE_SCORE_STREAM(col0, step_floats, wave, lane, ssm)                                                                  \
+    const float* scol = col0;                                                                                                       \
+    const int64_t sstep = step_floats;                                                                                              \
     int soff[4];                                                                                                                    \
     _Pragma("unroll") for (int gq = 0; gq < 4; ++gq) soff[gq] = gq * 256 + 4 * (lane ^ (2 * gq + (lane >> 5)));                     \
     float* sw = ssm + wave * 2 * SB_FLOATS;                                                                                         \
@@ -97,7 +97,9 @@
         const float* src = scol + (int64_t)qblk * sstep;                                                                            \
         _Pragma("unroll") for (int gq = 0; gq < 4; ++gq)                                                                            \
             __builtin_amdgcn_global_load_lds((glb_vp)(src + soff[gq]), (lds_vp)(sw + slot * SB_FLOATS + gq * 256), 16, 0, SRES_DMA_AUX); \
-    };                                                                                                                              \
+    }
+#define ATTN_KLANE_STREAMS(sres, H, NB, T, b, hd, key0, wave, lane, ssm, gsm, gm, gm_sb, gm_st)                                     \
+    ATTN_KLANE_SCORE_STREAM(sres + attn_score_block(H, NB, b, hd, 0, min(key0 >> 5, NB - 1)), (int64_t)NB * SB_FLOATS, wave, lane, ssm); \
     const float* gb0 = gm ? gm + (int64_t)b * gm_sb : nullptr;                                                                      \
     float* gw = gsm + wave * SB_FLOATS;                                                                                             \
     const int gcol = min(key0 + 4 * (lane & 7), (int)gm_st - 4);                                                                    \
@@ -108,13 +110,15 @@
             __builtin_amdgcn_global_load_lds((glb_vp)src, (lds_vp)(gw + p * 256), 16, 0, 0);                                        \
         }                                                                                                                           \
     }
-#define ATTN_KLANE_ADDRS(ssm, gsm, wave, r, h)                                                                                      \
+#define ATTN_KLANE_SADDRS(ssm, wave, r, h)                                                                                          \
     uint32_t stb[4];                                                                                                                \
     {                                                                                                                               \
         const int gk = r >> 3, hk = (r >> 2) & 1, ek = r & 3, mm = 2 * gk + hk;                                                     \
         _Pragma("unroll") for (int j = 0; j < 4; ++j)                                                                               \
             stb[j] = lds_addr_of(ssm) + ((wave * 2 * SB_FLOATS) + gk * 256 + 128 * hk + ek + 4 * ((j + 4 * h) ^ mm)) * 4;           \
-    }                                                                                                                               \
+    }
+#define ATTN_KLANE_ADDRS(ssm, gsm, wave, r, h)                                                                                      \
+    ATTN_KLANE_SADDRS(ssm, wave, r, h)                                                                                              \
     const uint32_t gaddr = lds_addr_of(gsm) + (wave * SB_FLOATS + 4 * h * 32 + r) * 4
 #define ATTN_16(M, ...) \
     M(0, __VA_ARGS__); M(1, __VA_ARGS__); M(2, __VA_ARGS__); M(3, __VA_ARGS__); M(4, __VA_ARGS__); M(5, __VA_ARGS__); M(6, __VA_ARGS__); M(7, __VA_ARGS__); \
@@ -137,6 +141,14 @@
     for (int gq = 0; gq < 4; ++gq) {
         const f32x4 t = {s[4 * gq], s[4 * gq + 1], s[4 * gq + 2], s[4 * gq + 3]};
         SRES_STORE(sp + gq * 256, t);
+    }
+}
+__device__ __forceinline__ void attn_store_scores_uniform(float* blk, int lane, const f32x16& s) {
+    const uint32_t voff = (uint32_t)lane * 16u;
+#pragma unroll
+    for (int gq = 0; gq < 4; ++gq) {
+        const f32x4 t = {s[4 * gq], s[4 * gq + 1], s[4 * gq + 2], s[4 * gq + 3]};
+        asm volatile("global_store_dwordx4 %0, %1, %2 offset:%3 nt" ::"v"(voff), "v"(t), "s"(blk), "n"(gq * 1024) : "memory");
     }
 }
 #define ATTN_SOFTMAX_STEP(s, m, l, o0, o1, p)                                                             \
diff --git a/acr_wsss_amd/csrc/attn_f32_sres.hip b/acr_wsss_amd/csrc/attn_f32_sres.hip
--- a/acr_wsss_amd/csrc/attn_f32_sres.hip
+++ b/acr_wsss_amd/csrc/attn_f32_sres.hip
@@ -482,7 +482,7 @@
     else if (bid < 2 * half)
         attn_dq_sres_body(smem, ssm, gsm, bid - half, half, ntail != 0, g, k, v, d_o, lse2, delta, sres, gm, gm_sb, gm_st, dq);
     else if (bid < 2 * half + ntail)
-        attn_dkdv_tail_body<4>(smem, ssm, g, q, v, d_o, lse2, delta, sres, gm, gm_sb, gm_st, dk, dv, acr_xcd_remap(bid - 2 * half, ntail));
+        attn_dkdv_tail_body<4>(smem, ssm, g, q, v, d_o, lse2, delta, sres, gm, gm_sb, gm_st, dk, dv, nullptr, acr_xcd_remap(bid - 2 * half, ntail));
     else
         attn_dq_tail_body<4>(smem, g, k, v, d_o, lse2, delta, sres, gm, gm_sb, gm_st, dq, acr_xcd_remap(bid - 2 * half - ntail, ntail));
 }
diff --git a/acr_wsss_amd/csrc/attn_f32_sres_tails.h b/acr_wsss_amd/csrc/attn_f32_sres_tails.h
--- a/acr_wsss_amd/csrc/attn_f32_sres_tails.h
+++ b/acr_wsss_amd/csrc/attn_f32_sres_tails.h
@@ -161,7 +161,8 @@
                                                     const float* __restrict__ v, const float* __restrict__ d_o,
                                                     const float* __restrict__ lse2, const float* __restrict__ delta,
                                                     const float* __restrict__ sres, const float* __restrict__ gm, int64_t gm_sb,
-                                                    int64_t gm_st, float* __restrict__ dk, float* __restrict__ dv, int id) {
+                                                    int64_t gm_st, float* __restrict__ dk, float* __restrict__ dv,
+                                                    float* __restrict__ dsw, int id) {
     const int NB = (g.T + 31) >> 5;
     const int hd = id % g.H, b = id / g.H;
     const int tid = threadIdx.x, lane = tid & 63;
@@ -230,6 +231,7 @@
                 ds[reg] = pv * (dp[reg] + gv[reg] - d4[e]);
             }
         }
+        if (dsw != nullptr) attn_store_scores_uniform(dsw + (scol - sres) + (int64_t)qt * sstep, lane, ds);
         accop_a_i<0, 0>(dv0, p, sm, lb);
         accop_a_i<0, 1>(dv1, p, sm, lb);
         wave_wait_lds();
diff --git a/acr_wsss_amd/csrc/attn_f32_x3.hip b/acr_wsss_amd/csrc/attn_f32_x3.hip
--- a/acr_wsss_amd/csrc/attn_f32_x3.hip
+++ b/acr_wsss_amd/csrc/attn_f32_x3.hip
@@ -13,6 +13,7 @@
 
 
 __device__ __forceinline__ void x3_wait_vm(int n) { attn_wait_vm<false, 9, 8, 7, 5, 4, 1>(n); }
+__device__ __forceinline__ void x3_wait_vm_dkdv(int n) { attn_wait_vm<false, 13, 9, 7, 5>(n); }
 __device__ __forceinline__ void x3_barrier(int n_younger) {
     x3_wait_vm(n_younger);
     acr_barrier_nofence();
@@ -388,13 +389,14 @@
     }
 }
 
+template <bool DS>
 __device__ __forceinline__ void attn_dkdv_x3_body(char* smem, float* ssm, float* gsm, float* rcm, int bid, int nblk, bool tails,
                                                   const X3Geom& g,
                                                   const bf16_t* __restrict__ qp, const bf16_t* __restrict__ vp,
                                                   const bf16_t* __restrict__ dop, const float* __restrict__ lse2,
                                                   const float* __restrict__ delta, const float* __restrict__ sres,
                                                   const float* __restrict__ gm, int64_t gm_sb, int64_t gm_st, float* __restrict__ dk,
-                                                  float* __restrict__ dv) {
+                                                  float* __restrict__ dv, float* __restrict__ dsw) {
     const int NB = (g.T + 31) >> 5, nkt = tails ? NB / X3_BW : (NB + X3_BW - 1) / X3_BW;
     int id = acr_xcd_remap(bid, nblk);
     const int ktile = id % nkt; id /= nkt;
@@ -432,10 +434,16 @@
     const int doff = x3_dma_off(g.D, pc, lane);
     ATTN_KLANE_ADDRS(ssm, gsm, wave, r, h);
     const uint32_t rcaddr = lds_addr_of(rcw) + 16 * h;
+    float* dcol = DS ? dsw + attn_score_block(g.H, NB, b, hd, 0, min(key0 >> 5, NB - 1)) : nullptr;
     auto step = [&](int q0, auto slot_tag) {
         constexpr int SLOT = decltype(slot_tag)::value;
         constexpr int QOFF = SLOT * X3_SLOT_B, DOOFF = QOFF + X3_TILE_B;
-        x3_barrier((q0 > 0 && live) ? 1 + (gb0 ? 4 : 0) + (q0 + 32 < g.T ? 4 : 0) : 0);
+        if constexpr (DS) {
+            x3_wait_vm_dkdv((q0 > 0 && live) ? 5 + (gb0 ? 4 : 0) + (q0 + 32 < g.T ? 4 : 0) : 0);
+            acr_barrier_nofence();
+        } else {
+            x3_barrier((q0 > 0 && live) ? 1 + (gb0 ? 4 : 0) + (q0 + 32 < g.T ? 4 : 0) : 0);
+        }
         auto dma_next = [&] {
             if (q0 + 64 <= g.T) x3_dma_tile_i(tdst + (SLOT ^ 1) * X3_SLOT_B, tb + (int64_t)(q0 + 32) * g.D, g.plane, doff, pc);
             else if (q0 + 32 < g.T) x3_dma_tile(tdst + (SLOT ^ 1) * X3_SLOT_B, tb, g.plane, g.D, q0 + 32, g.T, pc, lane);
@@ -444,7 +452,7 @@
         if (!live) { dma_next(); return; }
         f32x16 dp = {0};
         x3_rowop<DOOFF>(dp, lb, vf, dma_next);
-        if (q0 > 0) x3_wait_vm(q0 + 32 < g.T ? 7 : 0);
+        if (q0 > 0) { if constexpr (DS) x3_wait_vm_dkdv(q0 + 32 < g.T ? 7 : 0); else x3_wait_vm(q0 + 32 < g.T ? 7 : 0); }
         float s[16], gv[16];
         f32x4 l4[4], d4[4];
         ATTN_16(ATTN_RDS, s, SLOT);
@@ -468,7 +476,10 @@
         bf16x8 z0[3], z1[3];
         split3_bf16_acc<0>(p, z0);
         x3_accop<DOOFF, true>(dv0, dv1, z0, z1, lb,
-                              [&] { split3_bf16_acc<1>(p, z1); },
+                              [&] {
+                                  split3_bf16_acc<1>(p, z1);
+                                  if constexpr (DS) { attn_store_scores(dcol + (int64_t)(q0 >> 5) * sstep + lane * 4, ds); ATTN_FENCE(); }
+                              },
                               [&] { if (q0 + 32 < g.T) dma_rc(q0 + 32); ATTN_FENCE(); },
                               [&] { if (q0 + 32 < g.T) dma_g(q0 + 32); ATTN_FENCE(); });
         split3_bf16_acc<0>(ds, z0);
@@ -513,23 +524,111 @@
     const int half = ((int)gridDim.x - 2 * ntail) >> 1;
     const int bid = (int)blockIdx.x;
     if (bid < half)
-        attn_dkdv_x3_body(smem, ssm, gsm, rcm, bid, half, ntail != 0, g, qp, vp, dop, lse2, delta, sres, gm, gm_sb, gm_st, dk, dv);
+        attn_dkdv_x3_body<false>(smem, ssm, gsm, rcm, bid, half, ntail != 0, g, qp, vp, dop, lse2, delta, sres, gm, gm_sb, gm_st, dk, dv, nullptr);
     else if (bid < 2 * half)
         attn_dq_x3_body(smem, ssm, gsm, bid - half, half, ntail != 0, g, kp, vp, dop, lse2, delta, sres, gm, gm_sb, gm_st, dq);
     else if (bid < 2 * half + ntail)
         attn_dkdv_tail_body<X3_BW>(reinterpret_cast<float*>(lds), reinterpret_cast<float*>(lds) + X3_BW * DT_FLOATS, g32, q32, v32, do32, lse2,
-                                   delta, sres, gm, gm_sb, gm_st, dk, dv, acr_xcd_remap(bid - 2 * half, ntail));
+                                   delta, sres, gm, gm_sb, gm_st, dk, dv, nullptr, acr_xcd_remap(bid - 2 * half, ntail));
     else
         attn_dq_tail_body<X3_BW>(reinterpret_cast<float*>(lds), g32, k32, v32, do32, lse2, delta, sres, gm, gm_sb, gm_st, dq,
                                  acr_xcd_remap(bid - 2 * half - ntail, ntail));
 }
 
+#define X3_QW 4
+__global__ __launch_bounds__(64 * X3_QW, 2) void attn_dq_x3_kernel(X3Geom g, const bf16_t* __restrict__ kp, const float* __restrict__ dsw,
+                                                                  float* __restrict__ dq) {
+    __shared__ __attribute__((aligned(1024))) char smem[2 * X3_TILE_B + X3_QW * 2 * SB_FLOATS * 4];
+    float* ssm = reinterpret_cast<float*>(smem + 2 * X3_TILE_B);
+    const int NB = (g.T + 31) >> 5, nqt = (NB + X3_QW - 1) / X3_QW;
+    int id = acr_xcd_remap(blockIdx.x, gridDim.x);
+    const int qt = id % nqt; id /= nqt;
+    const int hd = id % g.H;
+    const int b = id / g.H;
+    const int tid = threadIdx.x, lane = tid & 63;
+    const int wave = __builtin_amdgcn_readfirstlane(tid >> 6);
+    const int r = lane & 31, h = lane >> 5;
+    const int q0 = (qt * X3_QW + wave) * 32;
+    const bool live = q0 < g.T;
+    const bf16_t* kb = kp + (int64_t)b * g.T * g.D + (int64_t)hd * 64;
+    ATTN_KLANE_SCORE_STREAM(dsw + attn_score_block(g.H, NB, b, hd, min(q0 >> 5, NB - 1), 0), SB_FLOATS, wave, lane, ssm);
+    x3_dma_tile(smem, kb, g.plane, g.D, 0, g.T, wave, lane);
+    if (live) {
+        dma_scores(0, 0);
+        if (32 < g.T) dma_scores(1, 1);
+    }
+    f32x16 dq0 = {0}, dq1 = {0};
+    const X3Lane lb = x3_lane(lane, smem);
+    const int doff = x3_dma_off(g.D, wave, lane);
+    ATTN_KLANE_SADDRS(ssm, wave, r, h);
+    auto step = [&](int k0, auto slot_tag) {
+        constexpr int SLOT = decltype(slot_tag)::value;
+        constexpr int KOFF = SLOT * X3_TILE_B;
+        x3_barrier((k0 > 0 && live && k0 + 32 < g.T) ? 4 : 0);
+        auto dma_next = [&] {
+            if (k0 + 64 <= g.T) x3_dma_tile_i(smem + (SLOT ^ 1) * X3_TILE_B, kb + (int64_t)(k0 + 32) * g.D, g.plane, doff, wave);
+            else if (k0 + 32 < g.T) x3_dma_tile(smem + (SLOT ^ 1) * X3_TILE_B, kb, g.plane, g.D, k0 + 32, g.T, wave, lane);
+            ATTN_FENCE();
+        };
+        if (!live) { dma_next(); return; }
+        float s[16];
+        ATTN_16(ATTN_RDS, s, SLOT);
+        asm volatile("s_waitcnt lgkmcnt(0)" : ATTN_V16(s));
+        f32x16 ds;
+#pragma unroll
+        for (int reg = 0; reg < 16; ++reg) ds[reg] = s[reg];
+        bf16x8 z0[3], z1[3];
+        split3_bf16_acc<0>(ds, z0);
+        x3_accop<KOFF, true>(dq0, dq1, z0, z1, lb,
+                             [&] { split3_bf16_acc<1>(ds, z1); },
+                             dma_next,
+                             [&] { if (k0 + 64 < g.T) dma_scores((k0 >> 5) + 2, SLOT); ATTN_FENCE(); });
+    };
+    for (int k0 = 0; k0 < g.T; k0 += 64) {
+        step(k0, std::integral_constant<int, 0>{});
+        if (k0 + 32 < g.T) step(k0 + 32, std::integral_constant<int, 1>{});
+    }
+    if (!live) return;
+    const int64_t base = (int64_t)b * g.sb + (int64_t)hd * g.sh;
+#pragma unroll
+    for (int reg = 0; reg < 16; ++reg) {
+        const int qq = q0 + acr_krow(reg, h);
+        if (qq < g.T) {
+            float* p = dq + base + (int64_t)qq * g.st;
+            p[r] = dq0[reg] * g.scale;
+            p[32 + r] = dq1[reg] * g.scale;
+        }
+    }
+}
+
+__global__ __launch_bounds__(64 * X3_BW, 2) void attn_dkdv_x3_kernel(X3Geom g, const bf16_t* __restrict__ qp, const bf16_t* __restrict__ vp,
+                                                                    const bf16_t* __restrict__ dop, const float* __restrict__ lse2,
+                                                                    const float* __restrict__ delta, const float* __restrict__ sres,
+                                                                    const float* __restrict__ gm, int64_t gm_sb, int64_t gm_st,
+                                                                    float* __restrict__ dk, float* __restrict__ dv, float* __restrict__ dsw,
+                                                                    const float* __restrict__ q32, const float* __restrict__ v32,
+                                                                    const float* __restrict__ do32, AttnGeom g32, int ntail) {
+    __shared__ __attribute__((aligned(1024))) char lds[2 * X3_SLOT_B + X3_BW * 3 * SB_FLOATS * 4 + X3_BW * 256];
+    char* smem = lds;
+    float* ssm = reinterpret_cast<float*>(lds + 2 * X3_SLOT_B);
+    float* gsm = ssm + X3_BW * 2 * SB_FLOATS;
+    float* rcm = gsm + X3_BW * SB_FLOATS;
+    const int nmain = (int)gridDim.x - ntail;
+    const int bid = (int)blockIdx.x;
+    if (bid < nmain)
+        attn_dkdv_x3_body<true>(smem, ssm, gsm, rcm, bid, nmain, ntail != 0, g, qp, vp, dop, lse2, delta, sres, gm, gm_sb, gm_st, dk, dv, dsw);
+    else
+        attn_dkdv_tail_body<X3_BW>(reinterpret_cast<float*>(lds), reinterpret_cast<float*>(lds) + X3_BW * DT_FLOATS, g32, q32, v32, do32, lse2,
+                                   delta, sres, gm, gm_sb, gm_st, dk, dv, dsw, acr_xcd_remap(bid - nmain, ntail));
+}
+
 int64_t acr_attn_x3_scores_floats(const AttnGeom& g) {
     return attn_score_floats(g.B, g.H, g.T) + 9 * ((int64_t)g.B * g.T * g.H * 64) / 2;
 }
 int64_t acr_attn_x3_bwd_ws_floats(const AttnGeom& g) {
     return (((int64_t)g.B * g.H * g.T + 3) & ~(int64_t)3) + 3 * ((int64_t)g.B * g.T * g.H * 64) / 2;
 }
+int64_t acr_attn_x3_bwd_ds_floats(const AttnGeom& g) { return attn_score_floats(g.B, g.H, g.T); }
 static X3Geom x3_geom(const AttnGeom& g) {
     X3Geom x;
     x.B = g.B; x.H = g.H; x.T = g.T; x.D = g.H * 64; x.scale = g.scale;
@@ -562,7 +661,7 @@
 
 void acr_attn_bwd_f32_x3(const AttnGeom& g, const float* q, const float* k, const float* v, const float* o, const float* d_o,
                          const float* lse2, const float* scores, const float* gm, int64_t gm_sb, int64_t gm_st, float* dq, float* dk,
-                         float* dv, float* delta_ws, hipStream_t st) {
+                         float* dv, float* delta_ws, float* ds_ws, hipStream_t st) {
     const X3Geom x = x3_geom(g);
     const bf16_t* planes = reinterpret_cast<const bf16_t*>(scores + attn_score_floats(g.B, g.H, g.T));
     bf16_t* dop = reinterpret_cast<bf16_t*>(delta_ws + (((int64_t)g.B * g.H * g.T + 3) & ~(int64_t)3));
@@ -575,9 +674,16 @@
     const int NB = (g.T + 31) / 32;
     const int ntail = attn_split_tail(NB, X3_BW) ? g.B * g.H : 0;
     const int nmain = g.B * g.H * (ntail ? NB / X3_BW : (NB + X3_BW - 1) / X3_BW);
-    hipLaunchKernelGGL(attn_bwd_x3_kernel, dim3(2 * nmain + 2 * ntail), dim3(64 * X3_BW), 0, st, x, planes, planes + 3 * x.plane,
-                       planes + 6 * x.plane, (const bf16_t*)dop, lse2, (const float*)delta_ws, scores, gm, gm_sb, gm_st, dq, dk, dv, q, k, v, d_o, g,
-                       ntail);
+    if (ds_ws == nullptr) {
+        hipLaunchKernelGGL(attn_bwd_x3_kernel, dim3(2 * nmain + 2 * ntail), dim3(64 * X3_BW), 0, st, x, planes, planes + 3 * x.plane,
+                           planes + 6 * x.plane, (const bf16_t*)dop, lse2, (const float*)delta_ws, scores, gm, gm_sb, gm_st, dq, dk, dv, q, k, v, d_o,
+                           g, ntail);
+        return;
+    }
+    hipLaunchKernelGGL(attn_dkdv_x3_kernel, dim3(nmain + ntail), dim3(64 * X3_BW), 0, st, x, planes, planes + 6 * x.plane, (const bf16_t*)dop,
+                       lse2, (const float*)delta_ws, scores, gm, gm_sb, gm_st, dk, dv, ds_ws, q, v, d_o, g, ntail);
+    hipLaunchKernelGGL(attn_dq_x3_kernel, dim3(g.B * g.H * ((NB + X3_QW - 1) / X3_QW)), dim3(64 * X3_QW), 0, st, x, planes + 3 * x.plane,
+                       (const float*)ds_ws, dq);
 }
 
 extern "C" int acr_split3_bf16(const float* x, int64_t rows, int64_t cols, int64_t ld, void* planes, int64_t plane_stride, void* stream) {
diff --git a/acr_wsss_amd/ops.py b/acr_wsss_amd/ops.py
--- a/acr_wsss_amd/ops.py
+++ b/acr_wsss_amd/ops.py
@@ -167,7 +167,11 @@
         qp, kp, vp = _qkv_ptrs(qkv, heads)
         dqp, dkp, dvp = _qkv_ptrs(dqkv, heads)
         tok = _t0("attn_bwd" if g_pm is not None else "attn_bwd_nomean", B, heads, T)
-        if scores is not None:
+        if scores is not None and d.dtype == L.ACR_F32_BF16X3:
+            ds_ws = torch.empty(lib.acr_attn_bwd_ds_floats(d), dtype=torch.float32, device=qkv.device)
+            L.check(lib.acr_attn_bwd_scores_ds(d, qp, kp, vp, L.ptr(o), L.ptr(d_o), L.ptr(lse2), L.ptr(scores), L.ptr(g_pm), gm_sb,
+                                               gm_st, dqp, dkp, dvp, L.ptr(delta), L.ptr(ds_ws), L.stream_ptr()), "acr_attn_bwd_scores_ds")
+        elif scores is not None:
             L.check(lib.acr_attn_bwd_scores(d, qp, kp, vp, L.ptr(o), L.ptr(d_o), L.ptr(lse2), L.ptr(scores), L.ptr(g_pm), gm_sb,
                                             gm_st, dqp, dkp, dvp, L.ptr(delta), L.stream_ptr()), "acr_attn_bwd_scores")
         else:
diff --git a/include/acr_hip.h b/include/acr_hip.h
--- a/include/acr_hip.h
+++ b/include/acr_hip.h
@@ -65,6 +65,11 @@
                         const void* o, const void* d_o, const float* lse2, const float* scores,
                         const float* gmean, int64_t gmean_sb, int64_t gmean_st,
                         void* dq, void* dk, void* dv, float* delta_ws, void* stream);
+int64_t acr_attn_bwd_ds_floats(const acr_attn_desc* desc);
+int acr_attn_bwd_scores_ds(const acr_attn_desc* desc, const void* q, const void* k, const void* v,
+                           const void* o, const void* d_o, const float* lse2, const float* scores,
+                           const float* gmean, int64_t gmean_sb, int64_t gmean_st,
+                           void* dq, void* dk, void* dv, float* delta_ws, float* ds_ws, void* stream);
 
 int acr_attn_probs(const acr_attn_desc* desc, const void* q, const void* k, const float* lse2,
                    float* probs, void* stream);
```
